# viswavi/speech-anonymization

Hardware: AMD Instinct MI355X
Metric: audio frames/sec (node), ConvAE+gender-adv train step (higher is better)
Workload: dtype bf16x3; 1 GPU; ConvAE recon0.1+sex0.9 adversarial train step (L1 recon + NLL), shape M: 32 utt/GPU x 161120 samples (T=1008 frames), Fbank x2 + norm + fwd + bwd + clip + Adam + Noam; batch_per_gpu=32, frames_per_utt=1008, parallelism=dp1

## Files before the change

### include/sa_hip.h

```cpp
#ifndef SA_HIP_H
#define SA_HIP_H
#ifdef __cplusplus
extern "C" {
#endif

#define SA_F32 0
#define SA_BF16 1
#define SA_BF16X3 2
#define SA_BF16X1F 3
#define SA_FP8 4
#define SA_F64 5
#define SA_MAX_TAPS 5
#define SA_COMM_ID_BYTES 128

typedef struct SaTaps {
  int ntaps[2];
  int off[2][SA_MAX_TAPS];
  int widx[2][SA_MAX_TAPS];
} SaTaps;

typedef struct SaConvArgs {
  const void* x;
  const void* wp;
  const float* bias;
  void* y;
  const float* s1; const float* t1;
  const float* s2; const float* t2;
  int swish;
  int relu;
  float* stats;
  int B, Lin, Lout, ntiles;
  int rowmin, nrows, wlo_off;
  SaTaps taps;
  int ep_mode, ep_xp_is_act, ep_bstride;
  const void* ep_x; const void* ep_g2;
  const float* ep_s1; const float* ep_t1; const float* ep_mean; const float* ep_rstd;
  void* a_out;
  const void* nb_x; const float* nb_c1; const float* nb_c2; const float* nb_c3;
  int nb_bstride, nb_relu_mask; float* nb_colsum;
  const float* ep_g2k1; const float* ep_g2k2; const float* ep_g2k3;
  float* pro_stats;
  const float* wscale;
  int tile_rows; int pad2_;
} SaConvArgs;

int sa_conv_gemm(int dtype, int cin, int cout, int sa, int u, const SaConvArgs* a, void* stream);
int sa_abi_sizeof(int which);
int sa_conv_gemm_ntiles(int cin, int cout, int u, int Lout);
int sa_conv_gemm_ntiles_tm(int tile_rows, int u, int Lout);
int sa_conv_gemm_set_tile_rows(int rows);
int sa_conv_gemm_set_impl(int impl);
int sa_conv_gemm_route(int dtype, int cin, int cout, int sa, int u, const SaConvArgs* a);

int sa_pack_weights(int dtype, const float* src, void* dst, int ntaps, int K, int N, int sk, int sn,
                    int st, void* stream);

typedef struct SaPackDesc {
  const float* src; void* dst;
  int dtype, ntaps, K, N, sk, sn, st, pad_;
  float* scale;
} SaPackDesc;
int sa_pack_weights_multi(const SaPackDesc* descs, int n, int blocks_per_image, void* stream);
int sa_pack_scales_multi(const SaPackDesc* descs, int n, void* stream);

typedef struct SaWgradArgs {
  const void* x;
  const void* dy;
  float* slabs;
  const float* s1; const float* t1; const float* s2; const float* t2; int swish;
  int B, Lin, Ldy, Mrows, chunk, nchunk;
  int ntaps; int off[SA_MAX_TAPS]; int ph[SA_MAX_TAPS];
  int x_pre;
  int dy_pre;
} SaWgradArgs;

int sa_wgrad(int dtype, int cin, int cout, int sa, int u, const SaWgradArgs* a, void* stream);
int sa_wgrad_kw(int cin, int cout);
int sa_wgrad_reduce(const float* slabs, float* dst, int nslab, int ntaps, int cin, int cout, int sk,
                    int sn, int st, int accumulate, void* stream);
#define SA_WRED_MAX 8
typedef struct SaWredDesc {
  const float* slabs; float* dst;
  int nslab, ntaps, cin, cout, sk, sn, st, accumulate, vec, pad_;
} SaWredDesc;
typedef struct SaWredMulti { int n, pad_; SaWredDesc d[SA_WRED_MAX]; } SaWredMulti;
int sa_wgrad_reduce_multi(const SaWredMulti* m, void* stream);

int sa_conv1toC(int dtype, const float* x, const float* w, const float* bias, void* y, int B, int L,
                int flip, float* stats, const void* ep_x, const float* ep_s1, const float* ep_t1,
                const float* ep_mean, const float* ep_rstd, void* stream);
int sa_conv1toC_ntiles(int L);
int sa_convCto1(int dtype, const void* x, const float* w, const float* bias, float* y, int B, int L,
                const float* s1, const float* t1, int swish, int flip, void* stream);
int sa_wgrad1C(int dtype, const float* u, const void* v, float* slabs, int B, int L, int chunk,
               int flip, const float* s1, const float* t1, int swish, void* stream);
int sa_wgrad1C_nchunk(int L, int chunk);
int sa_bwd1C(int dtype, const float* u, const void* v, const float* w, void* g, float* stats, float* slabs,
             int B, int L, int chunk, int flip, const float* s1, const float* t1, const float* mean,
             const float* rstd, void* stream);
int sa_sum_slabs(const float* slabs, float* dst, int nslab, int n, int accumulate, void* stream);

typedef struct SaEwArgs {
  const void* g; const void* g2; const void* x; void* out;
  const float* s1; const float* t1;
  const float* mean; const float* rstd;
  const float* c1; const float* c2; const float* c3;
  int actbwd, xp_is_act, relu_mask, bstride;
  float* stats;
  int B, L, ntiles;
} SaEwArgs;

int sa_ew_stats(int dtype, int C, const SaEwArgs* a, void* stream);
int sa_ew_apply(int dtype, int C, const SaEwArgs* a, void* stream);
int sa_ew_ntiles(int L);
int sa_sum_partials(const float* slabs, double* dst, int nbatch, int nslab, int n, void* stream);
int sa_sum_rows_d(const double* src, double* dst, int R, int n, void* stream);
int sa_fin_in_fwd(const double* sums, int B, int C, int n, const float* gamma, const float* beta,
                  float eps, float* mean, float* rstd, float* scale, float* shift, void* stream);
int sa_fin_bn_fwd(const double* sums, int R, int C, double count, const float* gamma, const float* beta,
                  float eps, float momentum, float* run_mean, float* run_var, float* mean,
                  float* rstd, float* scale, float* shift, const double* count_dev, void* stream);
int sa_fin_bn_eval(int C, const float* gamma, const float* beta, float eps, const float* run_mean,
                   const float* run_var, float* mean, float* rstd, float* scale, float* shift,
                   void* stream);
int sa_fin_norm_bwd(const double* sums, const double* lsums, int R, int groups, int C, double n,
                    const float* gamma, const float* mean, const float* rstd, float sign, float* c1,
                    float* c2, float* c3, float* dgamma, float* dbeta, const double* n_dev,
                    void* stream);
int sa_fin_bias(const double* sums, int B, int C, int ncomp, float* db, void* stream);

#define SA_FLATS_MAX 4
typedef struct SaFlat { float* p; long long n; } SaFlat;
typedef struct SaFlats { int n, pad_; SaFlat f[SA_FLATS_MAX]; } SaFlats;
int sa_clip_grads(const SaFlats* f, float max_norm, float eps, double* partials, float* total_norm, void* stream);
#define SA_BIAS_MAX 8
typedef struct SaBiasDesc {
  const float* part; double* rows; float* db;
  int nbatch, nslab, C, ncomp;
} SaBiasDesc;
typedef struct SaBiasMulti { int n, pad_; SaBiasDesc d[SA_BIAS_MAX]; } SaBiasMulti;
int sa_bias_multi(const SaBiasMulti* m, void* stream);

int sa_pool_fwd(int dtype, const void* r, const float* scale, const float* shift, float* part, int B,
                int L, int nseg, void* stream);
int sa_pool_nseg(int B);
int sa_pool_gather(const float* part, int B, int nseg, int L, double* sums, void* stream);
int sa_pool_fin(const double* sums, int B, int n, const float* noise, float eps, float* pooled,
                float* mean, float* stdraw, void* stream);
int sa_pool_bwd(int dtype, const void* r, const float* scale, const float* shift,
                const float* dpooled, const float* mean, const float* stdraw, void* g, int B, int L,
                const float* bn_mean, const float* bn_rstd, float* stats, void* stream);
int sa_dense(const float* X, int lda, const float* ps, const float* pt, const float* W, int sbk,
             int sbn, const float* bias, float* Y, int ldy, int M, int N, int K, int relu,
             void* stream);
int sa_colsums(const float* X, const float* H, const float* hmean, const float* hrstd, int M, int N,
               double* sums, float* out0, float* out1, void* stream);
int sa_bn2d_bwd(const float* G, const float* H, const double* sums, double count, const float* gamma,
                const float* mean, const float* rstd, int relu_mask, int M, int N, float* dH,
                const double* count_dev, void* stream);
int sa_dense_wgrad(const float* dY, const float* X, const float* ps, const float* pt, int M, int N,
                   int K, float* dW, void* stream);
int sa_log_softmax(const float* X, float* Y, int M, int N, void* stream);
int sa_log_softmax_bwd(const float* dY, const float* Y, float* dX, int M, int N, void* stream);
int sa_loss_workspace_bytes(void);
int sa_recon_loss(const float* a, const float* b, long long n, int kind, float* grad, float* loss,
                  void* workspace, void* stream);
int sa_cls_losses(const float* logp, const long long* label, int B, int NC, float* out, float* dnll,
                  float* dconf, void* stream);
int sa_cosine_loss(const float* x1, const float* x2, int B, int S, int D, float* rowloss,
                   float* loss, float* dx1, void* stream);

int sa_head_fwd(const float* pooled, const float* w1, const float* b1, const float* g1, const float* be1,
                float* rm1, float* rv1, const float* w2, const float* b2, const float* g2, const float* be2,
                float* rm2, float* rv2, const float* w3, const float* b3, float* h1, float* f1, float* h2,
                float* f2, float* logp, int M, float eps, float momentum, void* stream);
int sa_head_bwd(const float* dlogp, const float* logp, const float* pooled, const float* h1, const float* f1,
                const float* h2, const float* f2, const float* w1, const float* g1, const float* w2,
                const float* g2, const float* w3, float* dw1, float* db1, float* dg1, float* dbe1, float* dw2,
                float* db2, float* dg2, float* dbe2, float* dw3, float* db3, float* dpooled, int M, void* stream);
int sa_head_max_rows(void);

int sa_tdnn_fwd(const float* x, const void* wp, const float* bias, const float* bn_s, const float* bn_t,
                float* y, int B, int T, int Cin, int Cout, int Npad, int K, int dil, float slope,
                unsigned char* mask, void* stream);
int sa_time_pool(const float* x, const float* lens, const float* noise, int B, int T, int C, float eps,
                 float* out, void* stream);
int sa_leaky_affine(const float* x, const float* s, const float* t, float slope, int M, int C, float* y,
                    void* stream);
int sa_tdnn_bwd_input(const float* dy, const unsigned char* mask, const float* bn_s, const void* wp,
                      float* dxe, int B, int T, int Cy, int Cred, int Cin, int Npad, int K, int dil,
                      float slope, void* stream);
int sa_tdnn_fold(const float* dxe, float* dx, int B, int T, int C, int pad, void* stream);
int sa_time_pool_bwd(const float* x, const float* lens, const float* g, const float* pooled, int B,
                     int T, int C, float eps, float* dx, void* stream);
int sa_leaky_affine_bwd(const float* dy, const float* x, const float* s, float slope, int M, int C,
                        float* dx, void* stream);

int sa_xv_tdnn_fwd_train(const float* x, const float* s_in, const float* t_in, const void* wp, const float* bias,
                         float* z, float* part, int B, int T, int Cin, int Cout, int Npad, int K, int dil,
                         float slope, void* stream);
int sa_xv_tdnn_ntiles(int T);
int sa_xv_colsums(const float* G, const float* H, const float* hmean, const float* hrstd, const float* c1,
                  const float* c2, const float* c3, float slope, float* out, int M, int N, int rows_per,
                  double* part, void* stream);
int sa_xv_tdnn_wgrad(const float* dpre, const float* x, const float* s_in, const float* t_in, float* part, int B,
                     int T, int Cin, int Cout, int K, int dil, int nsplit, int rows_per, void* stream);
int sa_xv_wgrad_reduce(const float* part, int nsplit, int K, int Cout, int Cin, float* dW, void* stream);
int sa_xv_tdnn_dgrad(const float* dpre, const void* wp, float* dxe, int B, int T, int Cy, int Cred, int Cin,
                     int Npad, int K, int dil, void* stream);
int sa_xv_pool_affine(const float* pz, const float* s, const float* t, const float* noise, int B, int C,
                      float eps, float* pooled, void* stream);
int sa_xv_pool_affine_bwd(const float* g, const float* s, int B, int C, float* gz, void* stream);

int sa_fc_tiles(int T);
int sa_fc_groups(int B, int T);
int sa_fc_nparam(void);
int sa_fc_nhead(void);
int sa_fc_max_rows(void);
int sa_fc_enc_fwd(const float* feats, const void* const* wb, float* h1, float* h2, float* z, double* bnpart,
                  int B, int T, void* stream);
int sa_fc_bn_fin(const double* bnpart, int npart, const float* gamma, const float* beta, float* run_mean,
                 float* run_var, float* bnf, int B, int T, int train, float eps, float momentum, void* stream);
int sa_fc_mid_fwd(const float* z, const float* bnf, const void* const* wb, float* a1, float* u, float* d1,
                  float* d2, float* recon, double* poolpart, int B, int T, void* stream);
int sa_fc_recon_fwd(const float* feats, const void* const* wb, float* recon, int B, int T, void* stream);
int sa_fc_head_fwd(const double* poolpart, const float* noise, const void* const* hw, float* pooled, float* pst,
                   float* h1, float* f1, float* h2, float* h3, float* f2, float* logp, int B, int T, int train,
                   float eps, float momentum, void* stream);
int sa_fc_head_bwd(const float* dlogp, const float* logp, const float* pooled, const float* h1,
                   const float* h2, const float* h3, const void* const* hw, float* dhead,
                   float* dpooled, int B, int train, float eps, void* stream);
int sa_fc_mid_bwd(const float* d_recon, const float* dpooled, const float* pst, const float* z, const float* bnf,
                  const float* a1, const float* u, const float* d1, const float* d2, const void* const* wb,
                  float* dzn, float* dzdec, float* wpart, double* bnbpart, int B, int T, void* stream);
int sa_fc_bn_bwd_fin(const double* bnbpart, int npart, const float* gamma, const float* bnf, float* coef,
                     float* dgamma, float* dbeta, int B, int T, int train, void* stream);
int sa_fc_enc_bwd(const float* feats, const float* h1, const float* h2, const float* z, const float* dzn,
                  const float* dzdec, const float* coef, const void* const* wb, float* wpart, int B, int T,
                  void* stream);
int sa_fc_wreduce(const float* wpart, int G, float* grads, void* stream);

int sa_cluster_mi(const float* X, const long long* y, const long long* idx, int iters, int n, int D,
                  int ncls, int k, float* mi, void* stream);

int sa_fbank(const float* wav, int B, int N, const float* window, const void* dft,
             const void* mel, float* feats, float* tilemax, void* stream);
int sa_fbank_table_elems(int which);
int sa_fbank_ntiles(int T);
int sa_fbank_scratch_bytes(int B);
int sa_fbank_normalize(const float* feats, const float* tilemax, int B, int T, int Tp,
                       const float* lens, float top_db, int batch_max, int update, int epoch,
                       int update_until_epoch, float* state, float* scratch, float* out,
                       void* stream);
int sa_fbank_normalize_pair(const float* feats, const float* tilemax, int B, int T, int Tp,
                            const float* lens, float top_db, int batch_max, int update, int epoch,
                            int update_until_epoch, float* state, float* scratch, float* snap,
                            float* out1, float* out2, void* stream);

int sa_wav_augment_tile(void);
int sa_wav_augment_max_chunks(void);
int sa_wav_abs_sums(const float* wav, const float* noise, int B, int L, double* sums, void* stream);
int sa_noise_scales(const double* sums, const float* lens, const float* snr, int B, int L, float* scales,
                    void* stream);
int sa_wav_augment(const float* wav, const float* noise, const float* scales, const void* plan, int B, int L, int R,
                   int Lp, int S_in, int S_out, int W, int first_min, int first_max, float* out, void* stream);

int sa_specaug_warp_sums(const float* x, const void* plan, int B, int T, int F, float* out, double* part,
                         void* stream);
int sa_specaug_finalize(const double* part, const void* plan, int B, int T, int F, float* vals, void* stream);
int sa_specaug_fill(const void* plan, const float* vals, int B, int T, int F, float* out, void* stream);

int sa_gl_tile(void);
int sa_mel_to_mag(const float* x, const float* mean, const float* stdv, const float* M, int B, int T, int Tf,
                  float* S, void* stream);
int sa_gl_istft(const void* C, const float* window, const float* twiddle, int B, int T, float* y, void* stream);
int sa_gl_project(const float* y, const float* S, const void* Tprev, float momentum_ratio, const float* window,
                  const float* twiddle, int B, int T, void* C_new, void* R, void* stream);

int sa_yin_dim(int which);
int sa_yin_f0(const float* wav, int B, int N, float threshold, float* f0, float* dprime, void* stream);
int sa_pitch_ratio(const float* f0, const float* lens, int B, int T, int N, float target, float r_min, float r_max,
                   int min_voiced, float* ratio, float* mean, int* voiced, void* stream);
int sa_pitch_stretch_mag(const void* R, const float* ratio, int B, int T, int Tout, float* S, void* stream);
int sa_pitch_resample(const float* y, const float* ratio, const int* n_valid, int B, int Nin, int Nout, float* out,
                      void* stream);

int sa_env_dim(int which);
int sa_env_warp(const float* S, const float* q, int B, int T, int n_c, float floor_rel, float max_gain_ln,
                float* out, float* env, void* stream);

int sa_mcadams_dim(int which);
int sa_mcadams(const float* wav, const float* alpha, const int* n_valid, int B, int N, int level, float* out,
               void* ws, int* status, float* gain, void* stream);

int sa_stoi_dim(int which);
int sa_stoi(const float* ref, const float* deg, const int* n_valid, int B, int N, const double* taps,
            float* stoi, float* estoi, int* frames, int* segments, void* ws, void* stream);

int sa_pv_dim(int which);
long long sa_pv_workspace_bytes(int B, int Tout);
int sa_pv_synth(const void* R, const float* S, const float* ratio, int B, int T, int Tout, void* C, double* phase,
                void* ws, void* stream);

int sa_contour_dim(int which);
int sa_pitch_contour(const float* f0, const float* lens, int B, int T, int N, float target, float gamma, int smooth,
                     float r_min, float r_max, int min_voiced, int* rho_q, long long* Q, int* Tq, float* mean,
                     int* voiced, void* stream);
int sa_pv_synth_map(const void* R, const float* M, const int* rho_q, const long long* Q, int B, int T, int Tout,
                    void* C, double* phase, void* ws, void* stream);
int sa_env_warp_frames(const float* S, const float* q, int B, int T, int n_c, float floor_rel, float max_gain_ln,
                       float* out, float* env, void* stream);
int sa_pitch_resample_map(const float* y, const int* rho_q, const long long* Q, const int* n_valid, int B, int Nin,
                          int Nout, int T, float* out, void* stream);

int sa_f0v_dim(int which);
int sa_f0_candidates(const float* dprime, int B, int T, int* cand_tau, int* cand_q, void* stream);
int sa_f0_viterbi(const float* dprime, const int* cand_tau, const int* cand_q, const float* lens, const int* log_q,
                  int B, int T, int N, float voicing_cost, float switch_cost, float jump_cost, float lag_bias,
                  unsigned char* psi, int* path, float* f0, void* stream);

int sa_f0cmp_dim(int which);
int sa_f0_compare(const float* f0_ref, const float* f0_deg, const int* frames, int B, int T, int max_lag,
                  int min_common, float* rho, int* lag, int* common, float* shift_st, float* dev_st, float* voicing,
                  void* stream);

int sa_mcd_dim(int which);
int sa_mcd(const float* mel_ref, const float* mel_deg, const int* n_ref, const int* n_deg, int B, int T_ref, int T_deg,
           int n_mels, int order, int band, void* ws, float* mcd, float* mcd_sync, int* frames, void* stream);

int sa_psola_dim(int which);
long long sa_psola_workspace_bytes(int B, int N);
int sa_psola_marks(const float* wav, const float* f0, const int* n_valid, int B, int N, int T, int* marks, int* count,
                   void* stream);
int sa_psola_plan(const int* marks, const int* count, const float* f0, const int* rho_q, const int* n_valid, int B,
                  int N, int T, void* ws, int* syn_pos, int* syn_src, int* syn_count, void* stream);
int sa_psola_ola(const float* wav, const int* marks, const int* count, const int* syn_pos, const int* syn_src,
                 const int* syn_count, const int* n_valid, int B, int N, float* out, void* stream);

int sa_formant_dim(int which);
int sa_formant_tracks(const float* wav, const int* n_valid, int B, int N, float* freq, float* bw, int* status,
                      void* stream);
int sa_formant_compare(const float* F_ref, const float* F_deg, const int* st_ref, const int* st_deg,
                       const float* f0_ref, const float* f0_deg, const int* frames, int B, int T, int min_common,
                       float* med, float* ratio, float* shift, int* common, void* stream);

int sa_add_layernorm_fwd(const void* x, const void* r, const void* gamma, const void* beta, void* y, void* s_out,
                         float* stat, int rows, int d, float eps, void* stream);
int sa_layernorm_bwd(const void* dy, const void* s, const float* stat, const void* gamma, void* ds, int rows,
                     int d, void* stream);
int sa_ln_leaky_fwd(const void* x, const void* gamma, const void* beta, void* y, float* stat, int rows, int d,
                    float eps, float slope, void* stream);
int sa_ln_leaky_bwd(const void* dy, const void* x, const float* stat, const void* gamma, const void* beta, void* dx,
                    int rows, int d, float slope, void* stream);
int sa_asr_block0_fwd(const void* x, const void* w, const void* bias, const void* gamma, const void* beta, void* y,
                      float* stat, int B, int T, int F, int C, float eps, float slope, void* stream);
int sa_asr_block0_bwd(const void* dy, const void* x, const void* w, const void* bias, const void* gamma,
                      const void* beta, const float* stat, float* part, void* dx, int B, int T, int F, int C,
                      float slope, void* stream);
int sa_reflect_pad_fwd(const void* x, void* y, int B, int T, int F, int C, void* stream);
int sa_reflect_pad_bwd(const void* dy, void* dx, int B, int T, int F, int C, void* stream);

int sa_comm_unique_id(void* id128);
int sa_comm_init(int rank, int world, const void* id128, int device);
int sa_comm_world(void);
int sa_comm_allreduce(void* buf, long long n, int dtype, int avg, void* producer_stream);
int sa_comm_allreduce_inline(void* buf, long long n, int dtype, int avg, void* stream);
int sa_comm_join(void* consumer_stream);
int sa_comm_ncalls(void);
int sa_comm_destroy(void);

#ifdef __cplusplus
}
#endif
#endif
```

### speech-anonymization_amd/_lib.py

```python
import ctypes as C
import os

import torch

_HERE = os.path.dirname(os.path.abspath(__file__))
LIB_PATH = os.environ.get("SA_HIP_LIB") or os.path.join(_HERE, "libsa_hip.so")

F32, BF16, BF16X3, BF16X1F, FP8, F64 = 0, 1, 2, 3, 4, 5
MAX_TAPS = 5

c_fp = C.POINTER(C.c_float)
vp = C.c_void_p


class SaTaps(C.Structure):
    _fields_ = [("ntaps", C.c_int * 2), ("off", (C.c_int * MAX_TAPS) * 2),
                ("widx", (C.c_int * MAX_TAPS) * 2)]


class SaConvArgs(C.Structure):
    _fields_ = [("x", vp), ("wp", vp), ("bias", vp), ("y", vp),
                ("s1", vp), ("t1", vp), ("s2", vp), ("t2", vp),
                ("swish", C.c_int), ("relu", C.c_int), ("stats", vp),
                ("B", C.c_int), ("Lin", C.c_int), ("Lout", C.c_int), ("ntiles", C.c_int),
                ("rowmin", C.c_int), ("nrows", C.c_int), ("wlo_off", C.c_int), ("taps", SaTaps),
                ("ep_mode", C.c_int), ("ep_xp_is_act", C.c_int), ("ep_bstride", C.c_int),
                ("ep_x", vp), ("ep_g2", vp), ("ep_s1", vp), ("ep_t1", vp), ("ep_mean", vp), ("ep_rstd", vp),
                ("a_out", vp),
                ("nb_x", vp), ("nb_c1", vp), ("nb_c2", vp), ("nb_c3", vp),
                ("nb_bstride", C.c_int), ("nb_relu_mask", C.c_int), ("nb_colsum", vp),
                ("ep_g2k1", vp), ("ep_g2k2", vp), ("ep_g2k3", vp), ("pro_stats", vp), ("wscale", vp),
                ("tile_rows", C.c_int), ("pad2_", C.c_int)]


class SaPackDesc(C.Structure):
    _fields_ = [("src", vp), ("dst", vp), ("dtype", C.c_int), ("ntaps", C.c_int), ("K", C.c_int),
                ("N", C.c_int), ("sk", C.c_int), ("sn", C.c_int), ("st", C.c_int), ("pad_", C.c_int),
                ("scale", vp)]


class SaWgradArgs(C.Structure):
    _fields_ = [("x", vp), ("dy", vp), ("slabs", vp),
                ("s1", vp), ("t1", vp), ("s2", vp), ("t2", vp), ("swish", C.c_int),
                ("B", C.c_int), ("Lin", C.c_int), ("Ldy", C.c_int), ("Mrows", C.c_int),
                ("chunk", C.c_int), ("nchunk", C.c_int),
                ("ntaps", C.c_int), ("off", C.c_int * MAX_TAPS), ("ph", C.c_int * MAX_TAPS),
                ("x_pre", C.c_int), ("dy_pre", C.c_int)]


class SaEwArgs(C.Structure):
    _fields_ = [("g", vp), ("g2", vp), ("x", vp), ("out", vp),
                ("s1", vp), ("t1", vp), ("mean", vp), ("rstd", vp),
                ("c1", vp), ("c2", vp), ("c3", vp),
                ("actbwd", C.c_int), ("xp_is_act", C.c_int), ("relu_mask", C.c_int),
                ("bstride", C.c_int), ("stats", vp),
                ("B", C.c_int), ("L", C.c_int), ("ntiles", C.c_int)]


BIAS_MAX = 8


class SaBiasDesc(C.Structure):
    _fields_ = [("part", vp), ("rows", vp), ("db", vp),
                ("nbatch", C.c_int), ("nslab", C.c_int), ("C", C.c_int), ("ncomp", C.c_int)]


class SaBiasMulti(C.Structure):
    _fields_ = [("n", C.c_int), ("pad_", C.c_int), ("d", SaBiasDesc * BIAS_MAX)]


WRED_MAX = 8
FLATS_MAX = 4


class SaFlat(C.Structure):
    _fields_ = [("p", vp), ("n", C.c_longlong)]


class SaFlats(C.Structure):
    _fields_ = [("n", C.c_int), ("pad_", C.c_int), ("f", SaFlat * FLATS_MAX)]



class SaWredDesc(C.Structure):
    _fields_ = [("slabs", vp), ("dst", vp)] + [(k, C.c_int) for k in ("nslab", "ntaps", "cin", "cout", "sk", "sn", "st",
                                                                      "accumulate", "vec", "pad_")]


class SaWredMulti(C.Structure):
    _fields_ = [("n", C.c_int), ("pad_", C.c_int), ("d", SaWredDesc * WRED_MAX)]


SYMBOLS = [
    "sa_conv_gemm", "sa_abi_sizeof", "sa_conv_gemm_ntiles", "sa_conv_gemm_ntiles_tm", "sa_conv_gemm_set_tile_rows",
    "sa_conv_gemm_set_impl", "sa_conv_gemm_route", "sa_pack_weights", "sa_pack_weights_multi", "sa_pack_scales_multi", "sa_wgrad", "sa_wgrad_kw", "sa_wgrad_reduce",
    "sa_conv1toC", "sa_conv1toC_ntiles", "sa_convCto1", "sa_wgrad1C", "sa_wgrad1C_nchunk", "sa_bwd1C",
    "sa_sum_slabs", "sa_ew_stats", "sa_ew_apply", "sa_ew_ntiles",
    "sa_sum_partials", "sa_sum_rows_d", "sa_fin_in_fwd", "sa_fin_bn_fwd", "sa_fin_bn_eval", "sa_fin_norm_bwd", "sa_fin_bias",
    "sa_pool_fwd", "sa_pool_nseg", "sa_pool_gather", "sa_pool_fin", "sa_pool_bwd", "sa_dense", "sa_colsums",
    "sa_bn2d_bwd", "sa_dense_wgrad", "sa_log_softmax", "sa_log_softmax_bwd",
    "sa_loss_workspace_bytes", "sa_recon_loss", "sa_cls_losses", "sa_cosine_loss",
    "sa_tdnn_fwd", "sa_time_pool", "sa_leaky_affine", "sa_tdnn_bwd_input", "sa_tdnn_fold", "sa_time_pool_bwd",
    "sa_leaky_affine_bwd", "sa_cluster_mi", "sa_fbank", "sa_fbank_table_elems", "sa_fbank_ntiles", "sa_fbank_scratch_bytes", "sa_fbank_normalize", "sa_fbank_normalize_pair",
    "sa_comm_unique_id", "sa_comm_init", "sa_comm_world", "sa_comm_allreduce", "sa_comm_allreduce_inline", "sa_comm_join", "sa_comm_ncalls",
    "sa_comm_destroy", "sa_head_fwd", "sa_head_bwd", "sa_head_max_rows",
    "sa_add_layernorm_fwd", "sa_layernorm_bwd", "sa_reflect_pad_fwd", "sa_reflect_pad_bwd", "sa_ln_leaky_fwd", "sa_ln_leaky_bwd", "sa_bias_multi", "sa_asr_block0_fwd", "sa_asr_block0_bwd", "sa_wgrad_reduce_multi", "sa_clip_grads",
    "sa_xv_tdnn_fwd_train", "sa_xv_tdnn_ntiles", "sa_xv_colsums", "sa_xv_tdnn_wgrad", "sa_xv_wgrad_reduce",
    "sa_xv_tdnn_dgrad", "sa_xv_pool_affine", "sa_xv_pool_affine_bwd",
    "sa_fc_tiles", "sa_fc_groups", "sa_fc_nparam", "sa_fc_nhead", "sa_fc_max_rows", "sa_fc_enc_fwd", "sa_fc_bn_fin",
    "sa_fc_mid_fwd", "sa_fc_head_fwd", "sa_fc_head_bwd", "sa_fc_mid_bwd", "sa_fc_bn_bwd_fin", "sa_fc_enc_bwd",
    "sa_fc_wreduce", "sa_fc_recon_fwd",
    "sa_wav_augment_tile", "sa_wav_augment_max_chunks", "sa_wav_abs_sums", "sa_noise_scales", "sa_wav_augment",
    "sa_specaug_warp_sums", "sa_specaug_finalize", "sa_specaug_fill",
    "sa_gl_tile", "sa_mel_to_mag", "sa_gl_istft", "sa_gl_project",
    "sa_yin_dim", "sa_yin_f0", "sa_pitch_ratio", "sa_pitch_stretch_mag", "sa_pitch_resample",
    "sa_env_dim", "sa_env_warp",
    "sa_mcadams_dim", "sa_mcadams",
    "sa_stoi_dim", "sa_stoi",
    "sa_pv_dim", "sa_pv_synth",
    "sa_contour_dim", "sa_pitch_contour", "sa_pv_synth_map", "sa_env_warp_frames", "sa_pitch_resample_map",
    "sa_f0v_dim", "sa_f0_candidates", "sa_f0_viterbi",
    "sa_f0cmp_dim", "sa_f0_compare",
    "sa_mcd_dim", "sa_mcd",
    "sa_psola_dim", "sa_psola_marks", "sa_psola_plan", "sa_psola_ola",
    "sa_formant_dim", "sa_formant_tracks", "sa_formant_compare",
]

_lib = None


class SaHipError(RuntimeError):
    pass


def load():
    global _lib
    if _lib is None:
        if not os.path.exists(LIB_PATH):
            raise SaHipError(
                f"{LIB_PATH} not found: build it with `python -c 'import __graft_entry__ as g; "
                "g.build()'` (hipcc --offload-arch=gfx950). There is no CPU fallback.")
        _lib = C.CDLL(LIB_PATH)
        for s in SYMBOLS:
            getattr(_lib, s).restype = C.c_int
        _lib.sa_pv_workspace_bytes.restype = C.c_longlong
        _lib.sa_psola_workspace_bytes.restype = C.c_longlong
        for i, rec in enumerate((SaConvArgs, SaWgradArgs, SaEwArgs, SaPackDesc, SaTaps, SaBiasMulti, SaWredMulti, SaFlats)):
            if _lib.sa_abi_sizeof(i) != C.sizeof(rec):
                raise SaHipError(f"{rec.__name__}: binding has {C.sizeof(rec)} bytes, {LIB_PATH} "
                                 f"{_lib.sa_abi_sizeof(i)} -- rebuild the library (stale build?)")
    return _lib


def stream():
    return C.c_void_p(torch._C._cuda_getCurrentRawStream(torch._C._cuda_getDevice()))


def ptr(t):
    if t is None:
        return None
    assert t.is_cuda and t.is_contiguous(), "HIP kernels take contiguous device tensors"
    return C.c_void_p(t.data_ptr())


def check(rc, what):
    if rc != 0:
        raise SaHipError(f"{what} failed with code {rc}")


def dt_code(dtype):
    if dtype == torch.float32:
        return F32
    if dtype == torch.bfloat16:
        return BF16
    raise SaHipError(f"unsupported activation dtype {dtype}")


_taps_cache = {}


def make_taps(phases):
    key = tuple(tuple(p) for p in phases)
    t = _taps_cache.get(key)
    if t is not None:
        return t
    t = _taps_cache[key] = SaTaps()
    for ph, lst in enumerate(phases):
        t.ntaps[ph] = len(lst)
        for i, (off, wi) in enumerate(lst):
            t.off[ph][i] = off
            t.widx[ph][i] = wi
    return t
```

### speech-anonymization_amd/brain.py

```python
import enum
import os
import types

import torch

from . import distributed as sdist


class Stage(enum.Enum):
    TRAIN = 1
    VALID = 2
    TEST = 3


class EpochCounter:

    def __init__(self, limit):
        self.current, self.limit = 0, int(limit)

    def __iter__(self):
        return self

    def __next__(self):
        if self.current < self.limit:
            self.current += 1
            return self.current
        raise StopIteration


class NoamScheduler:

    def __init__(self, lr_initial, n_warmup_steps, model_size=None):
        self.lr_initial, self.n_warmup_steps = lr_initial, n_warmup_steps
        self.current_lr, self.n_steps = lr_initial, 0
        self.normalize = n_warmup_steps ** 0.5 if model_size is None else model_size ** (-0.5)

    def __call__(self, opt):
        self.n_steps += 1
        current_lr = getattr(opt, "_sa_host_lr", None)
        if current_lr is None:
            current_lr = opt.param_groups[0]["lr"]
        lr = self.lr_initial * self.normalize * min(self.n_steps ** (-0.5),
                                                    self.n_steps * self.n_warmup_steps ** (-1.5))
        for g in opt.param_groups:
            if torch.is_tensor(g["lr"]):
                g["lr"].fill_(lr)
            else:
                g["lr"] = lr
        opt._sa_host_lr = lr
        self.current_lr = current_lr
        return current_lr, lr

    def state_dict(self):
        return {"losses": [], "n_steps": self.n_steps}

    def load_state_dict(self, sd):
        self.n_steps = sd["n_steps"]


class Batch:

    def __init__(self, wavs, lens, gender, tokens_bos=None, ids=None):
        self.sig = (wavs, lens)
        self.gender = gender
        self.tokens_bos = (tokens_bos if tokens_bos is not None
                           else torch.ones(wavs.shape[0], 1, dtype=torch.long), lens)
        self.id = ids

    def to(self, device):
        w, l = self.sig
        tb, tl = self.tokens_bos
        out = Batch.__new__(Batch)
        out.sig = (w.to(device, non_blocking=True), l.to(device, non_blocking=True))
        out.gender = self.gender.to(device, non_blocking=True)
        out.tokens_bos = (tb.to(device, non_blocking=True), tl.to(device, non_blocking=True))
        out.id = self.id
        return out


def settle_python_heap():
    import gc
    gc.collect()
    gc.freeze()


class Brain:
    GC_FREEZE_STEP = 8

    def __init__(self, modules=None, opt_class=None, hparams=None, run_opts=None, checkpointer=None):
        run_opts = dict(run_opts or {})
        self.device = torch.device(run_opts.get("device", "cuda:0" if torch.cuda.is_available() else "cpu"))
        if self.device.type == "cuda":
            torch.cuda.set_device(self.device)
        self.max_grad_norm = float(run_opts.get("max_grad_norm", 5.0))
        self.nonfinite_patience = int(run_opts.get("nonfinite_patience", 3))
        self.lazy_finite_check = bool(run_opts.get("lazy_finite_check", True))
        self.hip_graph = bool(run_opts.get("hip_graph", False)) and self.device.type == "cuda"
        self.gc_freeze = bool(run_opts.get("gc_freeze", True))
        self.fused_clip = bool(run_opts.get("fused_clip", os.environ.get("SA_FUSED_CLIP", "1") == "1"))
        self.front_end_once = bool(run_opts.get("front_end_once", os.environ.get("SA_FRONT_END_ONCE", "1") == "1"))
        self.distributed_launch = bool(run_opts.get("distributed_launch", sdist.is_distributed()))
        self.modules = torch.nn.ModuleDict(modules or {})
        self.dp_batch_sizes = run_opts.get("dp_batch_sizes", "equal")
        self.opt_class = opt_class
        self.hparams = types.SimpleNamespace(**(hparams or {}))
        self.checkpointer = checkpointer
        self.step, self.nonfinite_count, self.optimizer = 0, 0, None
        self.avg_train_loss = 0.0

    def compute_forward(self, batch, stage):
        raise NotImplementedError

    def compute_objectives(self, predictions, batch, stage):
        raise NotImplementedError

    def on_stage_start(self, stage, epoch=None):
        pass

    def on_stage_end(self, stage, stage_loss, epoch=None):
        pass

    def on_fit_start(self):
        self.modules.to(self.device)
        for m in self.modules.values():
            if hasattr(m, "dp_batch_sizes"):
                m.dp_batch_sizes = self.dp_batch_sizes
        self.init_optimizers()
        if self.checkpointer is not None:
            if self.optimizer is not None:
                self.checkpointer.add_recoverable("optimizer", self.optimizer)
            self.resumed_from = self.checkpointer.recover_if_possible(device=self.device, brain=self)

    def init_optimizers(self):
        if self.opt_class is not None and self.optimizer is None:
            params = list(self.modules.parameters())
            base = getattr(self.opt_class, "func", self.opt_class)
            given = getattr(self.opt_class, "keywords", None) or {}
            if base is torch.optim.Adam and "fused" not in given and params and all(p.is_cuda for p in params):
                try:
                    if self.hip_graph:
                        self.optimizer = self.opt_class(params, fused=True, capturable=True)
                        for g in self.optimizer.param_groups:
                            self.optimizer._sa_host_lr = float(g["lr"])
                            g["lr"] = torch.tensor(float(g["lr"]), dtype=torch.float32, device=self.device)
                    else:
                        self.optimizer = self.opt_class(params, fused=True)
                    return
                except (TypeError, RuntimeError):
                    self.hip_graph = False
            self.optimizer = self.opt_class(params)

    def check_gradients(self, loss):
        bad = self._count_nonfinite(loss)
        if bad:
            self.nonfinite_count += bad
            if self.nonfinite_count > self.nonfinite_patience:
                raise ValueError("Loss is not finite and patience is exhausted.")
            if not (self.lazy_finite_check and loss.is_cuda):
                return False
        params = getattr(self, "_clip_params", None)
        if params is None:
            params = self._clip_params = list(self.modules.parameters())
        flats = self._grad_flats(params) if self.fused_clip else None
        if flats:
            from . import ops
            ops.clip_flats(flats, self.max_grad_norm)
        else:
            torch.nn.utils.clip_grad_norm_(params, self.max_grad_norm)
        return True

    def _grad_flats(self, params):
        model = self.modules["ConvAE"] if "ConvAE" in self.modules else None
        flats = getattr(model, "_last_flats", None) if model is not None else None
        if not flats:
            return None
        spans = [(f.data_ptr(), f.data_ptr() + 4 * f.numel(), f.numel()) for f in flats]
        seen = [0] * len(flats)
        for p in params:
            g = p.grad
            if g is None:
                continue
            if g.dtype != torch.float32 or not g.is_contiguous():
                return None
            a = g.data_ptr()
            for i, (lo, hi, _) in enumerate(spans):
                if lo <= a < hi:
                    seen[i] += g.numel()
                    break
            else:
                return None
        if any(n != span[2] for n, span in zip(seen, spans)):
            return None
        return flats

    def _count_nonfinite(self, loss):
        if not (self.lazy_finite_check and loss.is_cuda):
            return 0 if bool(torch.isfinite(loss)) else 1
        st = getattr(self, "_finite_state", None)
        if st is None:
            st = self._finite_state = dict(dev=torch.zeros((), dtype=torch.int32, device=loss.device),
                                           host=torch.zeros((), dtype=torch.int32).pin_memory(),
                                           event=torch.cuda.Event(), seen=0, pending=False)
        new = self._poll_nonfinite()
        st["dev"].add_((~torch.isfinite(loss.detach())).to(torch.int32))
        st["host"].copy_(st["dev"], non_blocking=True)
        if not torch.cuda.is_current_stream_capturing():
            st["event"].record()
            st["pending"] = True
        return new

    def _poll_nonfinite(self, wait=False):
        st = getattr(self, "_finite_state", None)
        if st is None or not st["pending"]:
            return 0
        if wait:
            st["event"].synchronize()
        elif not st["event"].query():
            return 0
        st["pending"] = False
        total = int(st["host"])
        new, st["seen"] = total - st["seen"], total
        return max(new, 0)

    def fit_batch(self, batch):
        outputs = self.compute_forward(batch, Stage.TRAIN)
        loss = self.compute_objectives(outputs, batch, Stage.TRAIN)
        loss.backward()
        if self.check_gradients(loss):
            self.optimizer.step()
        self.optimizer.zero_grad()
        return loss.detach()

    def evaluate_batch(self, batch, stage):
        out = self.compute_forward(batch, stage=stage)
        return self.compute_objectives(out, batch, stage=stage).detach()

    def update_average(self, loss, avg_loss):
        if not loss.is_cuda:
            if torch.isfinite(loss):
                avg_loss -= avg_loss / self.step
                avg_loss += float(loss) / self.step
            return avg_loss
        if not torch.is_tensor(avg_loss):
            avg_loss = torch.full((), float(avg_loss), device=loss.device, dtype=torch.float32)
        new = avg_loss + (loss.detach().float() - avg_loss) / self.step
        return torch.where(torch.isfinite(loss), new, avg_loss)

    def fit(self, epoch_counter, train_set, valid_set=None, progressbar=False, **_):
        self.on_fit_start()
        for epoch in epoch_counter:
            self.on_stage_start(Stage.TRAIN, epoch)
            self.modules.train()
            self.nonfinite_count = 0
            self.avg_train_loss = 0.0
            self.step = 0
            for batch in train_set:
                self.step += 1
                loss = self.fit_batch(batch)
                self.avg_train_loss = self.update_average(loss, self.avg_train_loss)
                if self.gc_freeze and self.step == self.GC_FREEZE_STEP and not self.__dict__.get("_gc_frozen"):
                    settle_python_heap()
                    self._gc_frozen = True
            self.nonfinite_count += self._poll_nonfinite(wait=True)
            if self.nonfinite_count > self.nonfinite_patience:
                raise ValueError("Loss is not finite and patience is exhausted.")
            self.avg_train_loss = float(self.avg_train_loss)
            self.on_stage_end(Stage.TRAIN, self.avg_train_loss, epoch)
            if valid_set is not None:
                self.on_stage_start(Stage.VALID, epoch)
                self.modules.eval()
                avg, n = 0.0, 0
                with torch.no_grad():
                    for batch in valid_set:
                        n += 1
                        avg += (float(self.evaluate_batch(batch, Stage.VALID)) - avg) / n
                self.on_stage_end(Stage.VALID, avg, epoch)

    def on_evaluate_start(self, max_key=None, min_key=None):
        pass

    def evaluate(self, test_set, max_key=None, min_key=None, **_):
        self.on_evaluate_start(max_key=max_key, min_key=min_key)
        self.on_stage_start(Stage.TEST, None)
        self.modules.eval()
        avg, n = 0.0, 0
        with torch.no_grad():
            for batch in test_set:
                n += 1
                avg += (float(self.evaluate_batch(batch, Stage.TEST)) - avg) / n
        self.on_stage_end(Stage.TEST, avg, None)
        return avg


class SexAnonymizationTraining(Brain):

    @staticmethod
    def _sig_key(wavs, wav_lens):
        return tuple((t.data_ptr(), tuple(t.shape), t.dtype, t._version) for t in (wavs, wav_lens))

    def features(self, wavs, wav_lens):
        stash, self._target_stash = self.__dict__.get("_target_stash"), None
        if stash is not None and stash[0] == self._sig_key(wavs, wav_lens):
            return stash[1]
        feats = self.hparams.compute_features(wavs)
        current_epoch = self.hparams.epoch_counter.current
        pad = 36 if self.hparams.model_type != "fcae" else None
        return self.modules.normalize(feats, wav_lens, epoch=current_epoch, pad_multiple=pad)

    def _features_pair(self, wavs, wav_lens):
        feats = self.hparams.compute_features(wavs)
        pad = 36 if self.hparams.model_type != "fcae" else None
        inp, target = self.modules.normalize.forward_pair(feats, wav_lens, epoch=self.hparams.epoch_counter.current,
                                                          pad_multiple=pad)
        self._target_stash = (self._sig_key(wavs, wav_lens), target)
        return inp

    def compute_forward(self, batch, stage):
        batch = batch.to(self.device)
        wavs, wav_lens = batch.sig
        if (stage == Stage.TRAIN and self.__dict__.get("_in_fit_batch") and self.front_end_once
                and hasattr(self.modules.normalize, "forward_pair")):
            feats = self._features_pair(wavs, wav_lens)
        else:
            feats = self.features(wavs, wav_lens)
        aug = self.__dict__.get("_specaug")
        if aug is not None and stage == Stage.TRAIN:
            self._specaug_shapes[tuple(wavs.shape)] = tuple(feats.shape)
            feats = aug.apply(feats) if self.__dict__.get("_specaug_drawn") else aug(feats)
        return self.modules.ConvAE(feats)

    def spec_augment(self):
        if not getattr(self.hparams, "spec_augment", False):
            return None
        from . import specaug
        aug = getattr(self.hparams, "augmentation", None)
        return aug if isinstance(aug, specaug.SpecAugment) else None

    def compute_objectives(self, predictions, batch, stage):
        reconstructed_speech, sex_logits = predictions
        batch = batch.to(self.device)
        sex_label = batch.gender
        wavs, wav_lens = batch.sig
        feats = self.features(wavs, wav_lens)
        hp = self.hparams
        utility_loss = 0.0
        asr_brain = getattr(self, "asr_brain", None)
        if stage == Stage.TRAIN and hp.utility_loss_weight > 0 and asr_brain is not None:
            from . import asr
            tokens_bos, _ = batch.tokens_bos
            utility_loss = asr.utility_loss(asr_brain, hp.loss_utility, feats, reconstructed_speech,
                                            wav_lens, tokens_bos, batch)
        B = reconstructed_speech.shape[0]
        recon_loss = hp.loss_reconstruction(reconstructed_speech.view(B, -1), feats.view(B, -1))
        sex_loss = hp.loss_sex_classification(sex_logits, sex_label)
        if hp.model_type == "endtoend":
            if hp.recon_loss_weight == 0.0 and hp.utility_loss_weight == 0.0:
                loss = hp.sex_loss_weight * sex_loss
            else:
                confusion_loss = hp.loss_confusion(sex_logits, None)
                loss = (hp.recon_loss_weight * recon_loss - hp.sex_loss_weight * sex_loss
                        + hp.utility_loss_weight * utility_loss
                        - hp.confusion_loss_weight * confusion_loss)
        else:
            loss = (hp.recon_loss_weight * recon_loss + hp.sex_loss_weight * sex_loss
                    + hp.utility_loss_weight * utility_loss)
        self.last_losses = dict(recon=recon_loss.detach(), sex=sex_loss.detach())
        if stage != Stage.TRAIN:
            n = torch.tensor(sex_label.shape[0], device=sex_logits.device).unsqueeze(0)
            self.sex_classification_acc.append(sex_logits.unsqueeze(0), sex_label.unsqueeze(0), n)
            ext = getattr(self, "external_classifier", None)
            if ext is not None:
                with torch.no_grad():
                    lo, _, _ = ext.classify_batch_feats(feats)
                    lr, _, _ = ext.classify_batch_feats(reconstructed_speech.detach())
                self.sex_classification_acc_extern_orig.append(lo.unsqueeze(0), sex_label.unsqueeze(0), n)
                self.sex_classification_acc_extern.append(lr.unsqueeze(0), sex_label.unsqueeze(0), n)
            if asr_brain is not None:
                from . import ops
                tokens_bos, _ = batch.tokens_bos
                with torch.no_grad():
                    recon_enc, _ = asr_brain.get_predictions(reconstructed_speech.detach(), wav_lens, tokens_bos,
                                                             batch, eval=True, do_ctc=False)
                    orig_enc, _ = asr_brain.get_predictions(feats, wav_lens, tokens_bos, batch, eval=True,
                                                            do_ctc=False)
                    nb = recon_enc.shape[0]
                    self.utility_similarity_aggregator.append(
                        ops.cosine_rows(recon_enc.reshape(nb, -1), orig_enc.reshape(nb, -1)))
        return loss

    def apply_epoch_schedule(self):
        hp = self.hparams
        if not getattr(hp, "epoch_parity_schedule", False):
            return
        joint = hp.epoch_counter.current % 2 == 0
        if joint:
            hp.recon_loss_weight, hp.sex_loss_weight = 0.0, 0.8
            hp.utility_loss_weight, hp.confusion_loss_weight = 0.2, 0.0
        else:
            hp.recon_loss_weight, hp.sex_loss_weight, hp.utility_loss_weight = 0.0, 0.5, 0.0
        for name, param in self.modules.ConvAE.named_parameters():
            param.requires_grad = ("sex_classifier" not in name) if joint else ("sex_classifier" in name)

    def _zero_grads_of_frozen(self):
        st = self.optimizer.state
        for group in self.optimizer.param_groups:
            for p in group["params"]:
                if p.grad is None and not p.requires_grad and p in st and len(st[p]):
                    z = getattr(self, "_zero_grad_cache", None)
                    if z is None:
                        z = self._zero_grad_cache = {}
                    g = z.get(p)
                    if g is None:
                        g = z[p] = torch.zeros_like(p)
                    p.grad = g

    GRAPH_WARMUP = 3

    def _graph_key(self, batch):
        hp = self.hparams
        wavs, lens = batch.sig
        nrm = self.modules["normalize"] if "normalize" in self.modules else None
        upd = nrm is not None and hp.epoch_counter.current < getattr(nrm, "update_until_epoch", 0)
        st = self.optimizer.state if self.optimizer is not None else {}
        params = list(self.modules.ConvAE.parameters())
        tok = batch.tokens_bos[0]
        return (tuple(wavs.shape), str(wavs.dtype), hp.model_type, float(hp.recon_loss_weight),
                float(hp.sex_loss_weight), float(hp.utility_loss_weight),
                float(getattr(hp, "confusion_loss_weight", 0.0)), bool(upd),
                tuple(p.requires_grad for p in params),
                tuple(bool(st.get(p)) for p in params if not p.requires_grad),
                tuple(tok.shape), getattr(self, "asr_brain", None) is not None,
                self.front_end_once, bool(not upd and getattr(nrm, "_count_positive", False)),
                self.__dict__.get("_specaug") is not None)

    def _step_core(self, batch):
        predictions = self.compute_forward(batch, Stage.TRAIN)
        loss = self.compute_objectives(predictions, batch, Stage.TRAIN)
        loss.backward()
        if getattr(self.hparams, "epoch_parity_schedule", False):
            self._zero_grads_of_frozen()
        self.check_gradients(loss)
        self.optimizer.step()
        return loss.detach()

    def _fit_batch_graph(self, batch):
        batch = batch.to(self.device)
        key = self._graph_key(batch)
        graphs = self.__dict__.setdefault("_graphs", {})
        ent = graphs.get(key)
        if ent is None:
            ent = graphs[key] = {"seen": 0}
        if "graph" not in ent:
            ent["seen"] += 1
            if ent["seen"] <= self.GRAPH_WARMUP:
                self.optimizer.zero_grad(set_to_none=True)
                loss = self._step_core(batch)
                self.optimizer.zero_grad()
                self.hparams.noam_annealing(self.optimizer)
                return loss
            wavs, lens = batch.sig
            ent["wav"], ent["lens"] = wavs.clone(), lens.clone()
            ent["gender"] = batch.gender.clone()
            tok, tok_lens = batch.tokens_bos
            ent["tok"], ent["tok_lens"] = tok.clone(), tok_lens.clone()
            ent["batch"] = Batch(ent["wav"], ent["lens"], ent["gender"], tokens_bos=ent["tok"], ids=batch.id)
            ent["batch"].tokens_bos = (ent["tok"], ent["tok_lens"])
            torch.cuda.synchronize()
            self.nonfinite_count += self._poll_nonfinite(wait=True)
            g = torch.cuda.CUDAGraph()
            self.optimizer.zero_grad(set_to_none=True)
            aug = self.__dict__.get("_specaug")
            if aug is not None:
                ent["specaug"] = self._specaug_shapes[tuple(wavs.shape)]
                aug.draw(*ent["specaug"], device=self.device)
                self._specaug_drawn = True
            try:
                with torch.cuda.graph(g):
                    ent["loss"] = self._step_core(ent["batch"])
            finally:
                self._specaug_drawn = False
            ent["graph"] = g
        elif "specaug" in ent:
            self._specaug.draw(*ent["specaug"], device=self.device)
        wavs, lens = batch.sig
        ent["wav"].copy_(wavs, non_blocking=True)
        ent["lens"].copy_(lens, non_blocking=True)
        ent["gender"].copy_(batch.gender, non_blocking=True)
        ent["tok"].copy_(batch.tokens_bos[0], non_blocking=True)
        ent["tok_lens"].copy_(batch.tokens_bos[1], non_blocking=True)
        ent["batch"].id = batch.id
        bad = self._poll_nonfinite()
        if bad:
            self.nonfinite_count += bad
            if self.nonfinite_count > self.nonfinite_patience:
                raise ValueError("Loss is not finite and patience is exhausted.")
        ent["graph"].replay()
        st = getattr(self, "_finite_state", None)
        if st is not None:
            st["event"].record()
            st["pending"] = True
        self.hparams.noam_annealing(self.optimizer)
        return ent["loss"]

    def fit_batch(self, batch):
        self._target_stash, self._in_fit_batch = None, True
        try:
            return self._fit_batch(batch)
        finally:
            self._target_stash, self._in_fit_batch = None, False

    def _fit_batch(self, batch):
        self.apply_epoch_schedule()
        if (self.hip_graph and self.hparams.gradient_accumulation == 1 and sdist.capturable()
                and self.optimizer is not None):
            return self._fit_batch_graph(batch)
        if self.front_end_once:
            batch = batch.to(self.device)
        predictions = self.compute_forward(batch, Stage.TRAIN)
        loss = self.compute_objectives(predictions, batch, Stage.TRAIN)
        (loss / self.hparams.gradient_accumulation).backward()
        if self.step % self.hparams.gradient_accumulation == 0:
            if getattr(self.hparams, "epoch_parity_schedule", False):
                self._zero_grads_of_frozen()
            self.check_gradients(loss)
            self.optimizer.step()
            self.optimizer.zero_grad()
            self.hparams.noam_annealing(self.optimizer)
        return loss.detach()

    def evaluate_batch(self, batch, stage):
        with torch.no_grad():
            predictions = self.compute_forward(batch, stage=stage)
            loss = self.compute_objectives(predictions, batch, stage=stage)
        return loss.detach()

    def load_external_classifier(self):
        ext = getattr(self.hparams, "external_classifier", None)
        if ext is not None:
            ext.eval()
            ext.to(self.device)
        return ext

    def on_stage_start(self, stage, epoch=None):
        from .metrics import AccuracyStats, SimilarityMetricsStats
        self.external_classifier = self.load_external_classifier()
        if stage == Stage.TRAIN:
            self._specaug = self.spec_augment()
            if self._specaug is not None:
                self.__dict__.setdefault("_specaug_shapes", {})
                self._specaug.reseed(epoch, sdist.rank())
        if stage != Stage.TRAIN:
            self.sex_classification_acc = AccuracyStats()
            self.sex_classification_acc_extern = AccuracyStats()
            self.sex_classification_acc_extern_orig = AccuracyStats()
            self.utility_similarity_aggregator = SimilarityMetricsStats()

    def on_evaluate_start(self, max_key=None, min_key=None):
        if self.checkpointer is None:
            return
        ckpts = self.checkpointer.find_checkpoints(max_key=max_key, min_key=min_key)
        if not ckpts:
            return
        sd = self.checkpointer.average_checkpoints(ckpts, recoverable_name="model", device=self.device)
        model = getattr(self.hparams, "model", None)
        if model is not None:
            model.load_state_dict(sd, strict=False)
            model.eval()

    def on_stage_end(self, stage, stage_loss, epoch=None):
        stats = {"loss": stage_loss}
        if stage == Stage.TRAIN:
            self.train_stats = stats
            return
        stats["ACC"] = self.sex_classification_acc.summarize()
        if self.external_classifier is not None:
            stats["ACC_external"] = self.sex_classification_acc_extern.summarize()
            stats["ACC_external_orig"] = self.sex_classification_acc_extern_orig.summarize()
        if self.utility_similarity_aggregator.denom:
            stats["Utility_Retention"] = float(self.utility_similarity_aggregator.summarize())
        self.valid_stats = stats
        logger = getattr(self.hparams, "train_logger", None)
        if stage == Stage.VALID and sdist.if_main_process() and logger is not None:
            na = self.hparams.noam_annealing
            logger.log_stats(stats_meta={"epoch": epoch, "lr": na.current_lr, "steps": na.n_steps,
                                         "optimizer": self.optimizer.__class__.__name__},
                             train_stats=self.train_stats, valid_stats=stats)
        if stage == Stage.VALID and sdist.if_main_process() and self.checkpointer is not None:
            keys = {k: stats[k] for k in ("ACC_external", "Utility_Retention") if k in stats}
            self.checkpointer.save_and_keep_only(self, epoch, dict(stats, **keys),
                                                 max_keys=[k for k in ("Utility_Retention",) if k in stats],
                                                 min_keys=[k for k in ("ACC_external",) if k in stats],
                                                 num_to_keep=5)


class FileTrainLogger:

    def __init__(self, save_file):
        self.save_file = save_file

    @staticmethod
    def _fmt(d):
        out = []
        for k, v in d.items():
            if isinstance(v, float) and 1.0 < v < 100.0:
                v = f"{v:.2f}"
            elif isinstance(v, float):
                v = f"{v:.2e}"
            out.append(f"{k}: {v}")
        return ", ".join(out)

    def log_stats(self, stats_meta, train_stats=None, valid_stats=None, test_stats=None):
        s = self._fmt(stats_meta)
        for name, st in (("train", train_stats), ("valid", valid_stats), ("test", test_stats)):
            if st is not None:
                s += " - " + self._fmt({f"{name} {k}": v for k, v in st.items()})
        os.makedirs(os.path.dirname(os.path.abspath(self.save_file)), exist_ok=True)
        with open(self.save_file, "a") as f:
            f.write(s + "\n")
```

### speech-anonymization_amd/convae.py

```python
import functools
import os

import torch
import torch.nn as nn

from . import distributed as sdist
from . import ops
from . import _lib as L
from ._lib import SaHipError


class _ParamOnly(nn.Module):

    def forward(self, x):
        raise SaHipError("parameter container only; use ConvAutoencoder.forward")


class GLU(_ParamOnly):
    pass


class StatisticsPooling(_ParamOnly):
    pass


class TDNNSexClassifier(nn.Module):
    def __init__(self, num_classes=2):
        super().__init__()
        self.tdnn = nn.Sequential(
            nn.Conv1d(128, 128, kernel_size=5, dilation=1), nn.ReLU(), nn.BatchNorm1d(128),
            nn.Conv1d(128, 128, kernel_size=3, dilation=2), nn.ReLU(), nn.BatchNorm1d(128),
            nn.Conv1d(128, 128, kernel_size=3, dilation=3), nn.ReLU(), nn.BatchNorm1d(128),
        )
        self.norm = nn.BatchNorm1d(128)
        self.stats_pooling = StatisticsPooling()
        self.classify = nn.Sequential(
            nn.Linear(256, 128), nn.ReLU(), nn.BatchNorm1d(128),
            nn.Linear(128, 64), nn.ReLU(), nn.BatchNorm1d(64),
            nn.Linear(64, num_classes),
        )

    def forward(self, x):
        raise SaHipError("parameter container only; use ConvAutoencoder.forward")


class ConvAutoencoder(nn.Module):
    def __init__(self, precision="bf16x3", pooling_noise=True, sync_bn=True, dtype=None,
                 cache_wgrad_operand=True):
        super().__init__()
        if dtype is not None:
            precision = {torch.float32: "f32", torch.bfloat16: "bf16"}[dtype]
        if precision not in ops.PRECISIONS:
            raise SaHipError(f"unknown precision {precision!r}")
        self.precision = precision
        self.encoder = nn.Sequential(
            nn.Conv1d(1, 32, 15, 1, 7), GLU(),
            nn.Conv1d(32, 64, 5, 2, 2), nn.InstanceNorm1d(64, affine=True), GLU(),
            nn.Conv1d(64, 64, 5, 1, 2), nn.InstanceNorm1d(64, affine=True), GLU(),
            nn.Conv1d(64, 128, 5, 2, 2), nn.InstanceNorm1d(128, affine=True), GLU(),
            nn.Conv1d(128, 128, 5, 1, 2), nn.InstanceNorm1d(128, affine=True), GLU(),
        )
        self.decoder = nn.Sequential(
            nn.Conv1d(128, 128, 5, 1, 2),
            nn.ConvTranspose1d(128, 64, 5, 2, 2, output_padding=1),
            nn.InstanceNorm1d(64, affine=True), GLU(),
            nn.Conv1d(64, 64, 5, 1, 2),
            nn.ConvTranspose1d(64, 32, 5, 2, 2, output_padding=1),
            nn.InstanceNorm1d(32, affine=True), GLU(),
            nn.Conv1d(32, 1, 15, 1, 7),
        )
        self.sex_classifier = TDNNSexClassifier(2)
        self.lay = ops.conv_layers(self, ("encoder", "sex_classifier.tdnn", "decoder"))
        self.pack_plan = [(ly.key, ly.kinds[i]) for i in (0, 1)
                          for ly in sorted(self.lay.values(), key=lambda ly: ly.transposed)]
        self.act_dtype, self.kcode = ops.PRECISIONS[precision]
        self.dgrad_kcode = ops.DGRAD_CODE[precision]
        self.cache_wgrad_operand = cache_wgrad_operand
        self.pooling_noise = pooling_noise
        self.sync_bn = sync_bn
        self.fused_head = os.environ.get("SA_FUSED_HEAD", "1") == "1"
        self.fused_bwd1c = os.environ.get("SA_FUSED_BWD1C", "1") == "1"
        self.dp_batch_sizes = None

    def forward(self, feats):
        names, params = self._named_params()
        return _ConvAEFn.apply(self, names, feats, *params)

    def _named_params(self):
        c = self.__dict__.get("_np_cache")
        if c is None or any(o[n] is not p for o, n, p in c[2]):
            names, params, owners = [], [], []
            for mname, mod in self.named_modules():
                for pname, p in mod._parameters.items():
                    if p is not None:
                        names.append(f"{mname}.{pname}" if mname else pname)
                        params.append(p)
                        owners.append((mod._parameters, pname, p))
            c = self.__dict__["_np_cache"] = (tuple(names), tuple(params), owners)
        return c[0], c[1]

    @torch.no_grad()
    def reconstruct(self, feats):
        if not torch.is_tensor(feats) or feats.dim() != 3:
            raise SaHipError("ConvAutoencoder expects feats [B, T, 80]")
        x0, B, T, Ltot = _input_rows(feats)
        P = dict(zip(*self._named_params()))
        cg, inorm = _launchers(self, P, _packed(self, P), B)
        y, _, _ = _encoder_launches(self, P, cg, inorm, x0, Ltot, False)
        return _decoder_launches(self, P, cg, inorm, y[5], Ltot)[-1].view(B, T, 80)

    def _side_stream(self, device):
        if getattr(self, "_side", None) is None and device.type == "cuda":
            self._side = torch.cuda.Stream(device=device)
        return getattr(self, "_side", None)

    def _bn_syncs(self):
        return self.sync_bn and sdist.dp_active()

    def _bn_allreduce(self, sums):
        if self._bn_syncs():
            sdist.all_reduce_now(sums)
            return sdist.world_size()
        return 1

    def _bn_global_counts(self, counts, device):
        if not self._bn_syncs():
            return None
        key = (tuple(counts), str(device))
        cache = self.__dict__.setdefault("_count_cache", {})
        local = cache.get(key)
        if local is None:
            if len(cache) > 64:
                cache.clear()
            local = cache[key] = torch.tensor(counts, dtype=torch.float64).to(device)
        g = local.clone()
        sdist.all_reduce_now(g)
        return g

    def _bn_rows(self):
        return not self._bn_syncs()

    def _bn_global(self, local_sums):
        if not self._bn_syncs():
            return local_sums, 1
        g = local_sums.clone()
        return g, self._bn_allreduce(g)

    def _head_plan(self, B):
        if not self._bn_syncs() or self.dp_batch_sizes is None:
            return None
        W, r = sdist.world_size(), sdist.rank()
        sizes = [B] * W if isinstance(self.dp_batch_sizes, str) else [int(b) for b in self.dp_batch_sizes]
        if self.dp_batch_sizes != "equal" and isinstance(self.dp_batch_sizes, str):
            raise SaHipError(f"dp_batch_sizes: 'equal', a list of per-rank batch sizes or None, not {self.dp_batch_sizes!r}")
        if len(sizes) != W or sizes[r] != B:
            raise SaHipError(f"dp_batch_sizes {sizes} does not describe rank {r} of {W} holding {B} utterances")
        return sum(sizes[:r]), sum(sizes), W

    @staticmethod
    def _gather_rows(x, plan):
        off, Bg, _ = plan
        g = torch.zeros(Bg, x.shape[1], device=x.device, dtype=x.dtype)
        g[off:off + x.shape[0]].copy_(x)
        sdist.all_reduce_now(g)
        return g


class _W:
    __slots__ = ("img", "code")

    def __init__(self, img, code):
        self.img, self.code = img, code


def _kcode(model, kind):
    return model.dgrad_kcode if kind.endswith("dgrad") else model.kcode


def _packed(model, P):
    items = [((k, kind), P[k], kind, _kcode(model, kind)) for k, kind in model.pack_plan]
    key = tuple(w.data_ptr() for _, w, _, _ in items) + tuple(c for _, _, _, c in items)
    pk = getattr(model, "_pack_cache", None)
    if pk is None or pk[0] != key:
        pk = (key, ops.PackedWeights(items, model.act_dtype))
        model._pack_cache = pk
    pk[1].refresh()
    return {tag: _W(img, code) for tag, (img, code) in pk[1].images.items()}


def _conv(x, w, *args, **kw):
    return ops.conv_gemm(x, w.img, *args, code=w.code, **kw)


class _PendingApply:
    __slots__ = ("g", "y", "c", "per_c", "relu", "bias_key", "wgrads")

    def __init__(self, g, y, c, per_c, relu, bias_key):
        self.g, self.y, self.c, self.per_c, self.relu, self.bias_key = g, y, c, per_c, relu, bias_key
        self.wgrads = []


def _noise(model, B, device):
    return ops.pooling_noise(model.pooling_noise, B, 128, device)


def _input_rows(feats):
    B, T, Fd = feats.shape
    Ltot = T * Fd
    if Fd != 80 or Ltot % 4:
        raise SaHipError("ConvAutoencoder expects feats [B, T, 80] with T*80 divisible by 4")
    if not feats.is_cuda:
        raise SaHipError("ConvAutoencoder runs on the GPU only (no CPU fallback)")
    return feats.detach().reshape(B, Ltot).contiguous().float(), B, T, Ltot


def _in_ep(y, nrm, g2=None):
    mean, rstd, scale, shift = nrm
    d = dict(mode=1, x=y, g2=g2, s1=scale, t1=shift, mean=mean, rstd=rstd)
    if isinstance(g2, _PendingApply):
        d.update(g2=g2.g, g2k=g2.c)
    return d


def _launchers(model, P, W, B, A=None):
    def cg(ly, x, **kw):
        if A is not None and P[ly.key].requires_grad:
            A[ly.key] = kw["a_out"] = torch.empty(x.shape, dtype=torch.bfloat16, device=x.device)
        return _conv(x, W[ly.key, ly.kinds[0]], P[ly.bias], *ly.fwd(x.shape[1]), **kw)

    def inorm(stats, n, prefix, C):
        sums = ops.sum_partials(stats, B)
        return ops.fin_in_fwd(sums, B, C, n, P[prefix + ".weight"], P[prefix + ".bias"])
    return cg, inorm


def _encoder_launches(model, P, cg, inorm, x0, Ltot, want_pro_stats):
    L2, L4, lay = Ltot // 2, Ltot // 4, model.lay
    y0 = ops.conv1toC(x0, P["encoder.0.weight"], P["encoder.0.bias"], model.act_dtype)
    y1, st = cg(lay["encoder.2"], y0, swish=True, want_stats=True)
    n1 = inorm(st, L2, "encoder.3", 64)
    y2, st = cg(lay["encoder.5"], y1, s1=n1[2], t1=n1[3], swish=True, want_stats=True)
    n2 = inorm(st, L2, "encoder.6", 64)
    y3, st = cg(lay["encoder.8"], y2, s1=n2[2], t1=n2[3], swish=True, want_stats=True)
    n3 = inorm(st, L4, "encoder.9", 128)
    y4, st = cg(lay["encoder.11"], y3, s1=n3[2], t1=n3[3], swish=True, want_stats=True)
    n4 = inorm(st, L4, "encoder.12", 128)
    y5 = cg(lay["decoder.0"], y4, s1=n4[2], t1=n4[3], swish=True, want_pro_stats=want_pro_stats)
    a4_stats = None
    if want_pro_stats:
        y5, a4_stats = y5
    return [y0, y1, y2, y3, y4, y5], [n1, n2, n3, n4], a4_stats


def _decoder_launches(model, P, cg, inorm, y5, Ltot):
    L2, lay = Ltot // 2, model.lay
    y6, st = cg(lay["decoder.1"], y5, want_stats=True)
    n6 = inorm(st, L2, "decoder.2", 64)
    y7 = cg(lay["decoder.4"], y6, s1=n6[2], t1=n6[3], swish=True)
    y8, st = cg(lay["decoder.5"], y7, want_stats=True)
    n8 = inorm(st, Ltot, "decoder.6", 32)
    recon = ops.convCto1(y8, P["decoder.8.weight"], P["decoder.8.bias"], n8[2], n8[3], True)
    return y6, n6, y7, y8, n8, recon


class _ConvAEFn(torch.autograd.Function):
    @staticmethod
    def forward(ctx, model, names, feats, *params):
        ctx.set_materialize_grads(False)
        P = dict(zip(names, params))
        train = model.training
        x0, B, T, Ltot = _input_rows(feats)
        L2, L4 = Ltot // 2, Ltot // 4
        S = {}
        W, lay = _packed(model, P), model.lay
        A = {}
        cache_a = (train and model.cache_wgrad_operand and any(ctx.needs_input_grad)
                   and ops.WGRAD_CODE[model.precision] in (L.BF16X1F, L.BF16) and model.kcode != L.FP8)

        cg, inorm = _launchers(model, P, W, B, A if cache_a else None)

        def bn_stats(stats, count, mod, prefix, C, ci):
            sums = ops.sum_partials(stats, 1, rows=model._bn_rows()) if train else None
            return bnorm(sums, count, mod, prefix, C, ci)

        def bnorm(sums, count, mod, prefix, C, ci, local=False):
            if not train:
                return ops.fin_bn_eval(C, P[prefix + ".weight"], P[prefix + ".bias"],
                                       mod.running_mean, mod.running_var)
            if not local:
                model._bn_allreduce(sums)
            out = ops.fin_bn_fwd(sums, C, count, P[prefix + ".weight"], P[prefix + ".bias"],
                                 mod.running_mean, mod.running_var, count_dev=None if local else cdev(ci))
            tracked.append(mod.num_batches_tracked)
            return out

        tracked = []
        enc, dec, cls = model.encoder, model.decoder, model.sex_classifier
        La, Lb, Lc = L4 - 4, L4 - 8, L4 - 14
        gc = model._bn_global_counts([B * L4, B * La, B * Lb, B * Lc, B, B], feats.device) if train else None
        cdev = lambda i: None if gc is None else gc[i:i + 1]
        (y0, y1, y2, y3, y4, y5), (n1, n2, n3, n4), a4_stats = _encoder_launches(model, P, cg, inorm, x0, Ltot, train)
        bn_n = bn_stats(a4_stats if train else None, B * L4, cls.norm, "sex_classifier.norm", 128, 0)
        r0, st = cg(lay["sex_classifier.tdnn.0"], y4, s1=n4[2], t1=n4[3], swish=True, s2=bn_n[2], t2=bn_n[3],
                    relu=True, want_stats=True)
        bn0 = bn_stats(st, B * La, cls.tdnn[2], "sex_classifier.tdnn.2", 128, 1)
        r1, st = cg(lay["sex_classifier.tdnn.3"], r0, s2=bn0[2], t2=bn0[3], relu=True, want_stats=True)
        bn1 = bn_stats(st, B * Lb, cls.tdnn[5], "sex_classifier.tdnn.5", 128, 2)
        r2, st = cg(lay["sex_classifier.tdnn.6"], r1, s2=bn1[2], t2=bn1[3], relu=True, want_stats=True)
        bn2 = bn_stats(st, B * Lc, cls.tdnn[8], "sex_classifier.tdnn.8", 128, 3)
        pooled, pmean, psd = ops.pool_fwd(r2, bn2[2], bn2[3], noise=_noise(model, B, feats.device))
        def head_fwd(X, n, local=False):
            H1 = ops.dense(X, P["sex_classifier.classify.0.weight"], P["sex_classifier.classify.0.bias"],
                           128, 256, relu=True)
            f1 = bnorm(ops.colsums(H1) if train else None, n, cls.classify[2], "sex_classifier.classify.2", 128, 4, local)
            H2 = ops.dense(H1, P["sex_classifier.classify.3.weight"], P["sex_classifier.classify.3.bias"],
                           64, 128, ps=f1[2], pt=f1[3], relu=True)
            f2 = bnorm(ops.colsums(H2) if train else None, n, cls.classify[5], "sex_classifier.classify.5", 64, 5, local)
            logits = ops.dense(H2, P["sex_classifier.classify.6.weight"], P["sex_classifier.classify.6.bias"],
                               2, 64, ps=f2[2], pt=f2[3])
            return H1, f1, H2, f2, ops.log_softmax(logits)

        plan = model._head_plan(B) if train else None
        head_in, Bh = (model._gather_rows(pooled, plan), plan[1]) if plan else (pooled, B)
        fused_head = (train and model.fused_head and (plan is not None or not model._bn_syncs())
                      and Bh <= ops.head_max_rows())
        clsP = {k[len("sex_classifier.classify."):]: v for k, v in P.items() if k.startswith("sex_classifier.classify.")}
        if fused_head:
            H1, f1, H2, f2, logp = ops.head_fwd(head_in, clsP, cls.classify[2], cls.classify[5])
            tracked += [cls.classify[2].num_batches_tracked, cls.classify[5].num_batches_tracked]
        else:
            H1, f1, H2, f2, logp = head_fwd(head_in, Bh, plan is not None)
        logp_all = logp
        if plan:
            logp = logp_all[plan[0]:plan[0] + B]
        y6, n6, y7, y8, n8, recon = _decoder_launches(model, P, cg, inorm, y5, Ltot)

        if tracked:
            torch._foreach_add_(tracked, 1)
        S.update(x0=x0, y=[y0, y1, y2, y3, y4, y5, y6, y7, y8], r=[r0, r1, r2],
                 n=[None, n1, n2, n3, n4, None, n6, None, n8], bn=[bn_n, bn0, bn1, bn2], f=[f1, f2],
                 pooled=head_in, pmean=pmean, psd=psd, H1=H1, H2=H2, logp=logp_all, head_plan=plan,
                 dims=(B, T, Ltot, L2, L4, La, Lb, Lc), train=train, W=W, A=A, gc=gc, fused_head=fused_head)
        ctx.S, ctx.model, ctx.names, ctx.params = S, model, names, params
        ctx.need_input_grad = feats.requires_grad
        return recon.view(B, T, 80), logp

    @staticmethod
    def backward(ctx, d_recon, d_logp):
        S, model, names = ctx.S, ctx.model, ctx.names
        if S is None:
            raise SaHipError("ConvAutoencoder backward called twice (saved tensors were released)")
        P = dict(zip(names, ctx.params))
        dt = model.act_dtype
        B, T, Ltot, L2, L4, La, Lb, Lc = S["dims"]
        if not S["train"]:
            raise SaHipError("backward through eval-mode BatchNorm is not implemented")
        y0, y1, y2, y3, y4, y5, y6, y7, y8 = S["y"]
        r0, r1, r2 = S["r"]
        n1, n2, n3, n4, n6, n8 = S["n"][1], S["n"][2], S["n"][3], S["n"][4], S["n"][6], S["n"][8]
        bn_n, bn0, bn1, bn2 = S["bn"]
        f1, f2 = S["f"]
        dev = y0.device
        G = {k: None for k in names}
        need = {k: p.requires_grad for k, p in P.items()}
        need_stage = {st: any(v for k, v in need.items() if k.startswith(st))
                      for st in sdist.StageBuckets.STAGES}
        run_encoder = need_stage["encoder"] or ctx.need_input_grad
        run_decoder = need_stage["decoder"] or run_encoder
        model._last_flats = None
        buckets = sdist.StageBuckets(list(P.items()), dev, model._side_stream(dev))
        newg = buckets.view

        def setg(key, val):
            G[key] = newg(key).copy_(val.reshape(P[key].shape))
        W, A, lay = S["W"], S["A"], model.lay
        gc = S["gc"]
        cdev = lambda i: None if gc is None else gc[i:i + 1]
        pending_wred = []
        wg = functools.partial(ops.wgrad, code=ops.WGRAD_CODE[model.precision], defer=pending_wred)
        fuse = bool(A) and model.dgrad_kcode in (L.BF16X3, L.BF16)

        def cg(ly, gin, **kw):
            p, dy = gin, gin.g if isinstance(gin, _PendingApply) else gin
            w, args = W[ly.key, ly.kinds[1]], (None,) + ly.dgrad(ly.lin(dy.shape[1]))
            if dy is gin:
                return _conv(dy, w, *args, **kw)
            dyc = torch.empty(p.g.shape, dtype=torch.bfloat16, device=p.g.device) if p.wgrads else None
            want_cs = p.bias_key is not None and need[p.bias_key]
            out = _conv(p.g, w, *args, a_out=dyc, nb=dict(x=p.y, c1=p.c[0], c2=p.c[1], c3=p.c[2],
                                                           per_c=p.per_c, relu_mask=p.relu,
                                                           want_colsum=want_cs), **kw)
            if want_cs:
                cs = out[-1]
                out = out[:-1] if len(out) > 2 else out[0]
                nb_, _, cc_ = cs.shape
                G[p.bias_key] = newg(p.bias_key)
                pending_bias.append((cs, nb_, cc_, 1, G[p.bias_key]))
            for f in p.wgrads:
                f(dyc)
            p.wgrads = []
            return out

        def bias_from(stats, key, C):
            if need[key]:
                G[key] = newg(key)
                pending_bias.append((stats, B, C, 2, G[key]))

        pending_bias = []

        def flush_pending():
            if pending_bias:
                ops.bias_multi(pending_bias)
                pending_bias.clear()
            if pending_wred:
                ops.wgrad_reduce_multi(pending_wred)
                pending_wred.clear()

        def in_finish(g, st, y, nrm, C, Ln, prefix, bias_key):
            mean, rstd = nrm[0], nrm[1]
            dg, db = newg(prefix + ".weight"), newg(prefix + ".bias")
            sums = ops.sum_partials(st, B)
            c1, c2, c3 = ops.fin_norm_bwd(sums, sums, B * C, C, Ln, P[prefix + ".weight"], mean, rstd,
                                          dgamma=dg, dbeta=db)
            G[prefix + ".weight"], G[prefix + ".bias"] = dg, db
            if fuse:
                return _PendingApply(g, y, (c1, c2, c3), False, False, bias_key)
            st2 = ops.ew("apply", g, y, C, out=g, c1=c1, c2=c2, c3=c3)
            bias_from(st2, bias_key, C)
            return g

        def bn_ep(r, bn, xp=None):
            d = dict(mode=2, x=r, mean=bn[0], rstd=bn[1], per_c=True)
            if xp:
                d.update(s1=xp[0], t1=xp[1], xp_is_act=True)
            return d

        def bn_finish(g, st, r, bn, Ln, prefix, bias_key, ci, xp=None):
            mean, rstd = bn[0], bn[1]
            kw = dict(s1=xp[0], t1=xp[1], xp_is_act=True) if xp else {}
            dg, db = newg(prefix + ".weight"), newg(prefix + ".bias")
            lsums = ops.sum_partials(st, 1, rows=model._bn_rows())
            gsums, _ = model._bn_global(lsums)
            c1, c2, c3 = ops.fin_norm_bwd(gsums, lsums, 128, 128, float(B * Ln), P[prefix + ".weight"],
                                          mean, rstd, sign=-1.0 if xp else 1.0, dgamma=dg, dbeta=db,
                                          n_dev=cdev(ci))
            G[prefix + ".weight"], G[prefix + ".bias"] = dg, db
            if fuse:
                return _PendingApply(g, r, (c1, c2, c3), True, not xp, bias_key)
            st2 = ops.ew("apply", g, r, 128, out=g, c1=c1, c2=c2, c3=c3, relu_mask=not xp, per_c=True,
                         want_stats=bias_key is not None, **kw)
            if bias_key:
                bias_from(st2, bias_key, 128)
            return g

        def conv_wgrad(ly, x, dy, **pro):
            key = ly.key
            if not need[key]:
                return
            if isinstance(dy, _PendingApply):
                dy.wgrads.append(lambda dyc: conv_wgrad(ly, x, dyc, dy_pre=True))
                return
            if key in A:
                x, pro = A[key], dict(x_pre=True, dy_pre=bool(pro.get("dy_pre")))
            *geo, strides = ly.wgrad(x.shape[1])
            G[key] = wg(x, dy, *geo, newg(key), strides, **pro)

        recon_unused = d_recon is None
        if recon_unused:
            for k in need:
                if k.startswith("decoder"):
                    need[k] = False
            need_stage["decoder"] = False
        if d_logp is None:
            d_logp = torch.zeros(B, 2, device=dev)

        def finish(d_feats=None):
            flush_pending()
            buckets.join()
            ctx.S = None
            model._last_flats = [buckets.flat[st] for st in sdist.StageBuckets.STAGES if need_stage[st]]
            grads = tuple(G[k] if need[k] else None for k in names)
            G.clear()
            buckets.views.clear()
            return (None, None, d_feats) + grads

        def head_bwd():
            c = "sex_classifier.classify."
            plan = S.get("head_plan")
            dlp, Bh = d_logp.contiguous().float(), B
            if plan:
                dlp, Bh = model._gather_rows(dlp, plan), plan[1]
            dP = head_bwd_rows(c, dlp, Bh, plan is not None)
            if plan:
                hg = [G[k] for k in names if k.startswith(c) and k in G]
                if plan[2] > 1 and hg:
                    torch._foreach_mul_(hg, 1.0 / plan[2])
                dP = dP[plan[0]:plan[0] + B]
            return dP

        def head_bwd_rows(c, dlp, n, local):
            if S.get("fused_head"):
                short = ("0.weight", "0.bias", "2.weight", "2.bias", "3.weight", "3.bias", "5.weight", "5.bias",
                         "6.weight", "6.bias")
                views = {}
                for k in short:
                    if need[c + k]:
                        views[k] = G[c + k] = newg(c + k)
                clsP = {k: P[c + k] for k in short}
                return ops.head_bwd(dlp, S["logp"], S["pooled"], S["H1"], f1, S["H2"], f2, clsP, views)
            glob = (lambda l: l) if local else (lambda l: model._bn_global(l)[0])
            cd = (lambda i: None) if local else cdev
            dLG = ops.log_softmax_bwd(dlp, S["logp"])
            H1, H2 = S["H1"], S["H2"]
            G[c + "6.weight"] = ops.dense_wgrad(dLG, H2, newg(c + "6.weight"), ps=f2[2], pt=f2[3])
            G[c + "6.bias"] = newg(c + "6.bias"); ops.colsums(dLG, out0=G[c + "6.bias"])
            dN2 = ops.dense(dLG, P[c + "6.weight"], None, 64, 2, transpose_w=True)
            G[c + "5.weight"], G[c + "5.bias"] = newg(c + "5.weight"), newg(c + "5.bias")
            l2 = ops.colsums(dN2, H2, f2[0], f2[1], out0=G[c + "5.bias"], out1=G[c + "5.weight"])
            dH2 = ops.bn2d_bwd(dN2, H2, glob(l2), n, P[c + "5.weight"], f2[0], f2[1], True, count_dev=cd(5))
            G[c + "3.weight"] = ops.dense_wgrad(dH2, H1, newg(c + "3.weight"), ps=f1[2], pt=f1[3])
            G[c + "3.bias"] = newg(c + "3.bias"); ops.colsums(dH2, out0=G[c + "3.bias"])
            dN1 = ops.dense(dH2, P[c + "3.weight"], None, 128, 64, transpose_w=True)
            G[c + "2.weight"], G[c + "2.bias"] = newg(c + "2.weight"), newg(c + "2.bias")
            l1 = ops.colsums(dN1, H1, f1[0], f1[1], out0=G[c + "2.bias"], out1=G[c + "2.weight"])
            dH1 = ops.bn2d_bwd(dN1, H1, glob(l1), n, P[c + "2.weight"], f1[0], f1[1], True, count_dev=cd(4))
            G[c + "0.weight"] = ops.dense_wgrad(dH1, S["pooled"], newg(c + "0.weight"))
            G[c + "0.bias"] = newg(c + "0.bias"); ops.colsums(dH1, out0=G[c + "0.bias"])
            return ops.dense(dH1, P[c + "0.weight"], None, 256, 128, transpose_w=True)

        def tdnn_bwd(dP):
            t = "sex_classifier.tdnn."
            g, st = ops.pool_bwd(r2, bn2[2], bn2[3], dP, S["pmean"], S["psd"], bn=(bn2[0], bn2[1]))
            g = bn_finish(g, st, r2, bn2, Lc, t + "8", t + "6.bias", 3)
            conv_wgrad(lay[t + "6"], r1, g, s2=bn1[2], t2=bn1[3])
            g, st = cg(lay[t + "6"], g, want_stats=True, ep=bn_ep(r1, bn1))
            g = bn_finish(g, st, r1, bn1, Lb, t + "5", t + "3.bias", 2)
            conv_wgrad(lay[t + "3"], r0, g, s2=bn0[2], t2=bn0[3])
            g, st = cg(lay[t + "3"], g, want_stats=True, ep=bn_ep(r0, bn0))
            g = bn_finish(g, st, r0, bn0, La, t + "2", t + "0.bias", 1)
            conv_wgrad(lay[t + "0"], y4, g, s1=n4[2], t1=n4[3], swish=True, s2=bn_n[2], t2=bn_n[3])
            xp4 = (n4[2], n4[3])
            g, st = cg(lay[t + "0"], g, want_stats=True, ep=bn_ep(y4, bn_n, xp4))
            da = bn_finish(g, st, y4, bn_n, L4, "sex_classifier.norm", None, 0, xp=xp4)
            flush_pending()
            if need_stage["sex_classifier"]:
                buckets.reduce_stage("sex_classifier")
            return da

        def decoder_bwd():
            d_rec = torch.zeros(B, T, 80, device=dev) if recon_unused else d_recon
            g_rec = d_rec.reshape(B, Ltot).contiguous().float()
            if need["decoder.8.bias"]:
                setg("decoder.8.bias", ops.sum_partials(g_rec.view(4 * B, Ltot // 4), 1, n=Ltot // 4).sum())
            if need["decoder.8.weight"] and model.fused_bwd1c:
                g, st, G["decoder.8.weight"] = ops.bwd1C(g_rec, y8, P["decoder.8.weight"], newg("decoder.8.weight"),
                                                         n8[2], n8[3], n8[0], n8[1])
            else:
                if need["decoder.8.weight"]:
                    G["decoder.8.weight"] = ops.wgrad1C(g_rec, y8, newg("decoder.8.weight"), flip=True,
                                                        s1=n8[2], t1=n8[3], swish=True)
                g, st = ops.conv1toC(g_rec, P["decoder.8.weight"], None, dt, flip=True, want_stats=True,
                                     ep=dict(x=y8, s1=n8[2], t1=n8[3], mean=n8[0], rstd=n8[1]))
            g = in_finish(g, st, y8, n8, 32, Ltot, "decoder.6", "decoder.5.bias")
            conv_wgrad(lay["decoder.5"], y7, g)
            g, st = cg(lay["decoder.5"], g, want_stats=True)
            bias_from(st, "decoder.4.bias", 64)
            conv_wgrad(lay["decoder.4"], y6, g, s1=n6[2], t1=n6[3], swish=True)
            g, st = cg(lay["decoder.4"], g, want_stats=True, ep=_in_ep(y6, n6))
            g = in_finish(g, st, y6, n6, 64, L2, "decoder.2", "decoder.1.bias")
            conv_wgrad(lay["decoder.1"], y5, g)
            g, st = cg(lay["decoder.1"], g, want_stats=True)
            bias_from(st, "decoder.0.bias", 128)
            conv_wgrad(lay["decoder.0"], y4, g, s1=n4[2], t1=n4[3], swish=True)
            flush_pending()
            if need_stage["decoder"]:
                buckets.reduce_stage("decoder")
            return g

        da4_cls = tdnn_bwd(head_bwd())
        if not run_decoder:
            return finish()
        g = decoder_bwd()
        if not run_encoder:
            return finish()

        g, st = cg(lay["decoder.0"], g, want_stats=True, ep=_in_ep(y4, n4, g2=da4_cls))
        for conv, norm, y, nrm, x, nx in (("encoder.11", "encoder.12", y4, n4, y3, n3),
                                          ("encoder.8", "encoder.9", y3, n3, y2, n2),
                                          ("encoder.5", "encoder.6", y2, n2, y1, n1),
                                          ("encoder.2", "encoder.3", y1, n1, y0, None)):
            ly = lay[conv]
            g = in_finish(g, st, y, nrm, ly.cout, y.shape[1], norm, ly.bias)
            conv_wgrad(ly, x, g, swish=True, **(dict(s1=nx[2], t1=nx[3]) if nx else {}))
            g, st = cg(ly, g, want_stats=True, ep=_in_ep(x, nx) if nx else dict(mode=1, x=x))
        bias_from(st, "encoder.0.bias", 32)
        if need["encoder.0.weight"]:
            G["encoder.0.weight"] = ops.wgrad1C(S["x0"], g, newg("encoder.0.weight"))
        d_feats = None
        if ctx.need_input_grad:
            d_feats = ops.convCto1(g, P["encoder.0.weight"], None, flip=True).view(B, T, 80)
        flush_pending()
        if need_stage["encoder"]:
            buckets.reduce_stage("encoder")
        return finish(d_feats)
```

### speech-anonymization_amd/csrc/sa_head.hip

```cpp
#include "sa_common.h"

template <typename T>
__global__ __launch_bounds__(256) void sa_pool_fwd_kernel(const T* __restrict__ r,
                                                          const float* __restrict__ sc,
                                                          const float* __restrict__ sh,
                                                          float* __restrict__ part, int L,
                                                          int nseg) {
  constexpr int C = 128, VEC = Tr<T>::VEC, CH = C / VEC, RPB = 256 / CH, NG = 128 / RPB;
  __shared__ float tile[RPB][C][2];
  const int tid = threadIdx.x, b = blockIdx.y, grp = blockIdx.x % NG, seg = blockIdx.x / NG;
  const int c = tid % CH, rl = tid / CH, lm = grp * RPB + rl;
  float s[VEC], t[VEC], sum[VEC], sq[VEC];
#pragma unroll
  for (int j = 0; j < VEC; ++j) { s[j] = sc[c * VEC + j]; t[j] = sh[c * VEC + j]; sum[j] = 0.f; sq[j] = 0.f; }
  const int nk = (L + 127) / 128, per = (nk + nseg - 1) / nseg;
  const int kbeg = seg * per, kend = (kbeg + per < nk) ? kbeg + per : nk;
  const T* rb = r + (size_t)b * L * C + c * VEC;
  for (int k0 = kbeg; k0 < kend; k0 += 4) {
    uint4 raw[4];
#pragma unroll
    for (int i = 0; i < 4; ++i) {
      const int l = lm + 128 * (k0 + i);
      raw[i] = make_uint4(0, 0, 0, 0);
      if (k0 + i < kend && l < L) raw[i] = *reinterpret_cast<const uint4*>(rb + (size_t)l * C);
    }
#pragma unroll
    for (int i = 0; i < 4; ++i) {
      const int l = lm + 128 * (k0 + i);
      if (k0 + i < kend && l < L) {
        float f[VEC];
        Tr<T>::unpack(raw[i], f);
#pragma unroll
        for (int j = 0; j < VEC; ++j) {
          const float v = fmaf(f[j], s[j], t[j]);
          sum[j] += v; sq[j] = fmaf(v, v, sq[j]);
        }
      }
    }
  }
#pragma unroll
  for (int j = 0; j < VEC; ++j) { tile[rl][c * VEC + j][0] = sum[j]; tile[rl][c * VEC + j][1] = sq[j]; }
  __syncthreads();
  float* dst = part + ((size_t)b * nseg + seg) * C * 128 * 2;
  for (int e = tid; e < RPB * C * 2; e += 256) {
    const int cc = e / (RPB * 2), w = e % (RPB * 2);
    dst[((size_t)cc * 128 + grp * RPB) * 2 + w] = tile[w >> 1][cc][w & 1];
  }
}

__global__ __launch_bounds__(1024) void sa_pool_gather_kernel(const float* __restrict__ part, int nseg,
                                                              int L, double* __restrict__ sums) {
  __shared__ double grp[7][128][2];
  const int tid = threadIdx.x, b = blockIdx.x, j = tid & 127, h = tid >> 7, Lm = L % 128;
  double s = 0.0, q = 0.0;
  for (int seg = 0; seg < nseg; ++seg) {
    const float2* p = reinterpret_cast<const float2*>(part) + ((size_t)b * nseg + seg) * 128 * 128;
#pragma unroll 16
    for (int c = h * 16; c < h * 16 + 16; ++c) {
      const float2 v = p[(size_t)c * 128 + ((j - c * Lm) & 127)];
      s += v.x; q += v.y;
    }
  }
  if (h > 0) { grp[h - 1][j][0] = s; grp[h - 1][j][1] = q; }
  __syncthreads();
  if (h == 0) {
#pragma unroll
    for (int g = 0; g < 7; ++g) { s += grp[g][j][0]; q += grp[g][j][1]; }
    sums[((size_t)b * 128 + j) * 2 + 0] = s;
    sums[((size_t)b * 128 + j) * 2 + 1] = q;
  }
}

extern "C" int sa_pool_nseg(int B) {
  int n = 2048 / (B * 16);
  return n < 1 ? 1 : (n > 8 ? 8 : n);
}

extern "C" int sa_pool_fwd(int dtype, const void* r, const float* scale, const float* shift,
                           float* part, int B, int L, int nseg, void* stream) {
  if (!r || !scale || !shift || !part || B <= 0 || L <= 1 || nseg < 1) return -22;
  hipStream_t st = reinterpret_cast<hipStream_t>(stream);
  if (dtype == SA_BF16)
    hipLaunchKernelGGL(sa_pool_fwd_kernel<bf16_t>, dim3(8 * nseg, B), dim3(256), 0, st,
                       reinterpret_cast<const bf16_t*>(r), scale, shift, part, L, nseg);
  else
    hipLaunchKernelGGL(sa_pool_fwd_kernel<float>, dim3(16 * nseg, B), dim3(256), 0, st,
                       reinterpret_cast<const float*>(r), scale, shift, part, L, nseg);
  hipError_t e = hipGetLastError();
  return e == hipSuccess ? 0 : -(int)e;
}

extern "C" int sa_pool_gather(const float* part, int B, int nseg, int L, double* sums, void* stream) {
  if (!part || !sums || B <= 0 || nseg < 1) return -22;
  hipLaunchKernelGGL(sa_pool_gather_kernel, dim3(B), dim3(1024), 0,
                     reinterpret_cast<hipStream_t>(stream), part, nseg, L, sums);
  hipError_t e = hipGetLastError();
  return e == hipSuccess ? 0 : -(int)e;
}

__global__ void sa_pool_fin_kernel(const double* __restrict__ sums, int B, int n,
                                   const float* __restrict__ noise, float eps, float* pooled,
                                   float* mean, float* stdraw) {
  const int i = blockIdx.x * blockDim.x + threadIdx.x;
  if (i >= B * 128) return;
  const int b = i / 128, j = i % 128;
  const double S = sums[2 * i], Q = sums[2 * i + 1];
  const double m = S / n;
  double var = (Q - S * m) / (n - 1);
  if (var < 0.0) var = 0.0;
  const float sd = (float)sqrt(var);
  mean[i] = (float)m; stdraw[i] = sd;
  float mo = (float)m;
  if (noise) mo += eps * ((1.0f - 9.0f) * noise[i] + 9.0f);
  pooled[(size_t)b * 256 + j] = mo;
  pooled[(size_t)b * 256 + 128 + j] = sd + eps;
}

extern "C" int sa_pool_fin(const double* sums, int B, int n, const float* noise, float eps,
                           float* pooled, float* mean, float* stdraw, void* stream) {
  if (!sums || !pooled || !mean || !stdraw || n < 2) return -22;
  hipLaunchKernelGGL(sa_pool_fin_kernel, dim3(sa_div_up(B * 128, 256)), dim3(256), 0,
                     reinterpret_cast<hipStream_t>(stream), sums, B, n, noise, eps, pooled, mean,
                     stdraw);
  hipError_t e = hipGetLastError();
  return e == hipSuccess ? 0 : -(int)e;
}

template <typename T>
__global__ __launch_bounds__(256) void sa_pool_bwd_kernel(const T* __restrict__ r,
                                                          const float* __restrict__ sc,
                                                          const float* __restrict__ sh,
                                                          const float* __restrict__ dpooled,
                                                          const float* __restrict__ mean,
                                                          const float* __restrict__ stdraw,
                                                          T* __restrict__ g, int L,
                                                          const float* __restrict__ bn_mean,
                                                          const float* __restrict__ bn_rstd,
                                                          float* __restrict__ stats) {
  constexpr int C = 128, VEC = Tr<T>::VEC, CH = C / VEC, RPP = 256 / CH;
  __shared__ float ka[128], kb[128];
  __shared__ float red[RPP][C][2];
  const int tid = threadIdx.x, b = blockIdx.y, l0 = blockIdx.x * SA_WAVE * 4;
  if (tid < 128) {
    const float dm = dpooled[(size_t)b * 256 + tid], ds = dpooled[(size_t)b * 256 + 128 + tid];
    const float sd = stdraw[(size_t)b * 128 + tid], m = mean[(size_t)b * 128 + tid];
    const float inv = sd > 0.0f ? 1.0f / ((float)(L - 1) * sd) : 0.0f;
    kb[tid] = ds * inv;
    ka[tid] = dm / (float)L - ds * inv * m;
  }
  __syncthreads();
  const int c = tid % CH, r0 = tid / CH;
  float s[VEC], t[VEC];
  int jb[VEC];
#pragma unroll
  for (int j = 0; j < VEC; ++j) {
    s[j] = sc[c * VEC + j]; t[j] = sh[c * VEC + j];
    jb[j] = (int)(((long long)(c * VEC + j) * L) % 128);
  }
  float bm[VEC], br[VEC], s1[VEC], s2[VEC];
#pragma unroll
  for (int j = 0; j < VEC; ++j) {
    bm[j] = stats ? bn_mean[c * VEC + j] : 0.0f;
    br[j] = stats ? bn_rstd[c * VEC + j] : 0.0f;
    s1[j] = 0.0f; s2[j] = 0.0f;
  }
  for (int rr = r0; rr < 256; rr += RPP) {
    const int l = l0 + rr;
    if (l >= L) break;
    float f[VEC], x[VEC];
    Tr<T>::unpack(*reinterpret_cast<const uint4*>(r + ((size_t)b * L + l) * C + c * VEC), x);
#pragma unroll
    for (int j = 0; j < VEC; ++j) {
      const int col = (jb[j] + l) % 128;
      f[j] = fmaf(kb[col], fmaf(x[j], s[j], t[j]), ka[col]);
    }
    const uint4 u = Tr<T>::pack(f);
    *reinterpret_cast<uint4*>(g + ((size_t)b * L + l) * C + c * VEC) = u;
    if (stats) {
      Tr<T>::unpack(u, f);
#pragma unroll
      for (int j = 0; j < VEC; ++j) {
        s1[j] += f[j];
        s2[j] = fmaf(f[j], (x[j] - bm[j]) * br[j], s2[j]);
      }
    }
  }
  if (stats) {
#pragma unroll
    for (int j = 0; j < VEC; ++j) { red[r0][c * VEC + j][0] = s1[j]; red[r0][c * VEC + j][1] = s2[j]; }
    __syncthreads();
    if (tid < C) {
      float a0 = 0.0f, a1 = 0.0f;
#pragma unroll
      for (int q = 0; q < RPP; ++q) { a0 += red[q][tid][0]; a1 += red[q][tid][1]; }
      float* dst = stats + (((size_t)b * gridDim.x + blockIdx.x) * C + tid) * 2;
      dst[0] = a0; dst[1] = a1;
    }
  }
}

extern "C" int sa_pool_bwd(int dtype, const void* r, const float* scale, const float* shift,
                           const float* dpooled, const float* mean, const float* stdraw, void* g,
                           int B, int L, const float* bn_mean, const float* bn_rstd, float* stats,
                           void* stream) {
  if (!r || !scale || !shift || !dpooled || !mean || !stdraw || !g || L < 2) return -22;
  if (stats && (!bn_mean || !bn_rstd)) return -22;
  hipStream_t st = reinterpret_cast<hipStream_t>(stream);
  dim3 grid(sa_div_up(L, 256), B);
  if (dtype == SA_BF16)
    hipLaunchKernelGGL(sa_pool_bwd_kernel<bf16_t>, grid, dim3(256), 0, st,
                       reinterpret_cast<const bf16_t*>(r), scale, shift, dpooled, mean, stdraw,
                       reinterpret_cast<bf16_t*>(g), L, bn_mean, bn_rstd, stats);
  else
    hipLaunchKernelGGL(sa_pool_bwd_kernel<float>, grid, dim3(256), 0, st,
                       reinterpret_cast<const float*>(r), scale, shift, dpooled, mean, stdraw,
                       reinterpret_cast<float*>(g), L, bn_mean, bn_rstd, stats);
  hipError_t e = hipGetLastError();
  return e == hipSuccess ? 0 : -(int)e;
}

__global__ __launch_bounds__(256) void sa_dense_kernel(const float* __restrict__ X, int lda,
                                                       const float* __restrict__ ps,
                                                       const float* __restrict__ pt,
                                                       const float* __restrict__ W, int sbk, int sbn,
                                                       const float* __restrict__ bias, float* __restrict__ Y,
                                                       int ldy, int M, int N, int K, int relu) {
  __shared__ float part[4][16][64];
  const int lane = threadIdx.x & 63, wave = threadIdx.x >> 6, n0 = blockIdx.x * 32, m0 = blockIdx.y * 32;
  const int m = m0 + (lane & 31), n = n0 + (lane & 31), kh = lane >> 5;
  f32x16 acc;
#pragma unroll
  for (int i = 0; i < 16; ++i) acc[i] = 0.0f;
  for (int k0 = wave * 16; k0 < K; k0 += 64) {
    float av[8], bv[8];
#pragma unroll
    for (int u = 0; u < 8; ++u) {
      const int k = k0 + 2 * u + kh;
      av[u] = 0.0f; bv[u] = 0.0f;
      if (k < K) {
        if (m < M) {
          av[u] = X[(size_t)m * lda + k];
          if (ps) av[u] = fmaf(av[u], ps[k], pt[k]);
        }
        if (n < N) bv[u] = W[(size_t)k * sbk + (size_t)n * sbn];
      }
    }
#pragma unroll
    for (int u = 0; u < 8; ++u)
      if (k0 + 2 * u < K) acc = __builtin_amdgcn_mfma_f32_32x32x2f32(av[u], bv[u], acc, 0, 0, 0);
  }
#pragma unroll
  for (int i = 0; i < 16; ++i) part[wave][i][lane] = acc[i];
  __syncthreads();
  if (wave == 0 && n < N) {
    const float bb = bias ? bias[n] : 0.0f;
#pragma unroll
    for (int i = 0; i < 16; ++i) {
      const int mr = m0 + sa_acc_row(i, lane);
      if (mr < M) {
        float v = ((part[0][i][lane] + part[1][i][lane]) + part[2][i][lane]) + part[3][i][lane] + bb;
        if (relu) v = fmaxf(v, 0.0f);
        Y[(size_t)mr * ldy + n] = v;
      }
    }
  }
}

extern "C" int sa_dense(const float* X, int lda, const float* ps, const float* pt, const float* W,
                        int sbk, int sbn, const float* bias, float* Y, int ldy, int M, int N, int K,
                        int relu, void* stream) {
  if (!X || !W || !Y || M <= 0 || N <= 0 || K <= 0) return -22;
  dim3 grid(sa_div_up(N, 32), sa_div_up(M, 32));
  hipLaunchKernelGGL(sa_dense_kernel, grid, dim3(256), 0, reinterpret_cast<hipStream_t>(stream), X,
                     lda, ps, pt, W, sbk, sbn, bias, Y, ldy, M, N, K, relu);
  hipError_t e = hipGetLastError();
  return e == hipSuccess ? 0 : -(int)e;
}

__global__ void sa_colsums_kernel(const float* __restrict__ X, const float* __restrict__ H,
                                  const float* __restrict__ hm, const float* __restrict__ hr,
                                  int M, int N, double* sums, float* __restrict__ out0,
                                  float* __restrict__ out1) {
  const int n = blockIdx.x * blockDim.x + threadIdx.x;
  if (n >= N) return;
  double s = 0.0, q = 0.0;
#pragma unroll 8
  for (int m = 0; m < M; ++m) {
    const float x = X[(size_t)m * N + n];
    float h = H ? H[(size_t)m * N + n] : x;
    if (hm) h = (h - hm[n]) * hr[n];
    s += x; q += (double)x * h;
  }
  sums[2 * n] = s; sums[2 * n + 1] = q;
  if (out0) out0[n] = (float)s;
  if (out1) out1[n] = (float)q;
}

extern "C" int sa_colsums(const float* X, const float* H, const float* hmean, const float* hrstd,
                          int M, int N, double* sums, float* out0, float* out1, void* stream) {
  if (!X || !sums) return -22;
  hipLaunchKernelGGL(sa_colsums_kernel, dim3(sa_div_up(N, 64)), dim3(64), 0,
                     reinterpret_cast<hipStream_t>(stream), X, H, hmean, hrstd, M, N, sums, out0,
                     out1);
  hipError_t e = hipGetLastError();
  return e == hipSuccess ? 0 : -(int)e;
}

__global__ void sa_bn2d_bwd_kernel(const float* __restrict__ G, const float* __restrict__ H,
                                   const double* __restrict__ sums, double count,
                                   const float* __restrict__ gamma, const float* __restrict__ mean,
                                   const float* __restrict__ rstd, int relu_mask, int M, int N,
                                   float* dH, const double* __restrict__ count_dev) {
  const int i = blockIdx.x * blockDim.x + threadIdx.x;
  if (i >= M * N) return;
  if (count_dev) count = *count_dev;
  const int n = i % N;
  const float hh = (H[i] - mean[n]) * rstd[n];
  float v = gamma[n] * rstd[n] * (G[i] - (float)(sums[2 * n] / count) - hh * (float)(sums[2 * n + 1] / count));
  if (relu_mask && !(H[i] > 0.0f)) v = 0.0f;
  dH[i] = v;
}

extern "C" int sa_bn2d_bwd(const float* G, const float* H, const double* sums, double count,
                           const float* gamma, const float* mean, const float* rstd, int relu_mask,
                           int M, int N, float* dH, const double* count_dev, void* stream) {
  if (!G || !H || !sums || !gamma || !mean || !rstd || !dH) return -22;
  hipLaunchKernelGGL(sa_bn2d_bwd_kernel, dim3(sa_div_up(M * N, 256)), dim3(256), 0,
                     reinterpret_cast<hipStream_t>(stream), G, H, sums, count, gamma, mean, rstd,
                     relu_mask, M, N, dH, count_dev);
  hipError_t e = hipGetLastError();
  return e == hipSuccess ? 0 : -(int)e;
}

__global__ void sa_dense_wgrad_kernel(const float* __restrict__ dY, const float* __restrict__ X,
                                      const float* __restrict__ ps, const float* __restrict__ pt,
                                      int M, int N, int K, float* dW) {
  const int i = blockIdx.x * blockDim.x + threadIdx.x;
  if (i >= N * K) return;
  const int n = i / K, k = i % K;
  float s = 0.0f;
#pragma unroll 8
  for (int m = 0; m < M; ++m) {
    float x = X[(size_t)m * K + k];
    if (ps) x = fmaf(x, ps[k], pt[k]);
    s = fmaf(dY[(size_t)m * N + n], x, s);
  }
  dW[i] = s;
}

extern "C" int sa_dense_wgrad(const float* dY, const float* X, const float* ps, const float* pt,
                              int M, int N, int K, float* dW, void* stream) {
  if (!dY || !X || !dW) return -22;
  hipLaunchKernelGGL(sa_dense_wgrad_kernel, dim3(sa_div_up(N * K, 256)), dim3(256), 0,
                     reinterpret_cast<hipStream_t>(stream), dY, X, ps, pt, M, N, K, dW);
  hipError_t e = hipGetLastError();
  return e == hipSuccess ? 0 : -(int)e;
}

__global__ void sa_log_softmax_kernel(const float* __restrict__ X, float* __restrict__ Y, int M, int N) {
  const int m = blockIdx.x * blockDim.x + threadIdx.x;
  if (m >= M) return;
  float mx = -INFINITY;
  for (int n = 0; n < N; ++n) mx = fmaxf(mx, X[(size_t)m * N + n]);
  float s = 0.0f;
  for (int n = 0; n < N; ++n) s += expf(X[(size_t)m * N + n] - mx);
  const float lse = mx + logf(s);
  for (int n = 0; n < N; ++n) Y[(size_t)m * N + n] = X[(size_t)m * N + n] - lse;
}
__global__ void sa_log_softmax_bwd_kernel(const float* __restrict__ dY, const float* __restrict__ Y,
                                          float* __restrict__ dX, int M, int N) {
  const int m = blockIdx.x * blockDim.x + threadIdx.x;
  if (m >= M) return;
  float s = 0.0f;
  for (int n = 0; n < N; ++n) s += dY[(size_t)m * N + n];
  for (int n = 0; n < N; ++n) dX[(size_t)m * N + n] = dY[(size_t)m * N + n] - expf(Y[(size_t)m * N + n]) * s;
}
extern "C" int sa_log_softmax(const float* X, float* Y, int M, int N, void* stream) {
  if (!X || !Y) return -22;
  hipLaunchKernelGGL(sa_log_softmax_kernel, dim3(sa_div_up(M, 64)), dim3(64), 0,
                     reinterpret_cast<hipStream_t>(stream), X, Y, M, N);
  hipError_t e = hipGetLastError();
  return e == hipSuccess ? 0 : -(int)e;
}
extern "C" int sa_log_softmax_bwd(const float* dY, const float* Y, float* dX, int M, int N, void* stream) {
  if (!dY || !Y || !dX) return -22;
  hipLaunchKernelGGL(sa_log_softmax_bwd_kernel, dim3(sa_div_up(M, 64)), dim3(64), 0,
                     reinterpret_cast<hipStream_t>(stream), dY, Y, dX, M, N);
  hipError_t e = hipGetLastError();
  return e == hipSuccess ? 0 : -(int)e;
}

__global__ __launch_bounds__(256) void sa_recon_loss_kernel(const float* __restrict__ a,
                                                            const float* __restrict__ b, size_t n,
                                                            int kind, float* __restrict__ grad,
                                                            double* __restrict__ part) {
  __shared__ double wsum[4];
  const float inv = 1.0f / (float)n;
  double s = 0.0;
  const size_t n4 = n / 4;
  for (size_t i = (size_t)blockIdx.x * blockDim.x + threadIdx.x; i < n4; i += (size_t)gridDim.x * blockDim.x) {
    const float4 x = reinterpret_cast<const float4*>(a)[i], y = reinterpret_cast<const float4*>(b)[i];
    float d[4] = {x.x - y.x, x.y - y.y, x.z - y.z, x.w - y.w}, g[4];
#pragma unroll
    for (int j = 0; j < 4; ++j) {
      if (kind == 0) { s += fabsf(d[j]); g[j] = d[j] > 0.f ? inv : (d[j] < 0.f ? -inv : 0.f); }
      else { s += (double)d[j] * d[j]; g[j] = 2.0f * d[j] * inv; }
    }
    if (grad) reinterpret_cast<float4*>(grad)[i] = make_float4(g[0], g[1], g[2], g[3]);
  }
  if (blockIdx.x == 0 && threadIdx.x == 0)
    for (size_t i = n4 * 4; i < n; ++i) {
      const float d = a[i] - b[i];
      if (kind == 0) { s += fabsf(d); if (grad) grad[i] = d > 0.f ? inv : (d < 0.f ? -inv : 0.f); }
      else { s += (double)d * d; if (grad) grad[i] = 2.0f * d * inv; }
    }
  s = sa_wave_sum_d(s);
  if ((threadIdx.x & 63) == 0) wsum[threadIdx.x >> 6] = s;
  __syncthreads();
  if (threadIdx.x == 0) part[blockIdx.x] = wsum[0] + wsum[1] + wsum[2] + wsum[3];
}
__global__ void sa_recon_loss_fin_kernel(const double* part, int nb, double n, float* loss) {
  __shared__ double lane_sum[64];
  double s = 0.0;
#pragma unroll 8
  for (int i = threadIdx.x; i < nb; i += 64) s += part[i];
  lane_sum[threadIdx.x] = s;
  __syncthreads();
  if (threadIdx.x == 0) {
    double t = 0.0;
    for (int i = 0; i < 64; ++i) t += lane_sum[i];
    loss[0] = (float)(t / n);
  }
}
#define SA_LOSS_BLOCKS 512
extern "C" int sa_loss_workspace_bytes() { return SA_LOSS_BLOCKS * (int)sizeof(double); }
extern "C" int sa_recon_loss(const float* a, const float* b, long long n, int kind, float* grad,
                             float* loss, void* workspace, void* stream) {
  if (!a || !b || !loss || !workspace || n <= 0) return -22;
  if ((reinterpret_cast<uintptr_t>(a) | reinterpret_cast<uintptr_t>(b) |
       reinterpret_cast<uintptr_t>(grad)) & 15) return -22;
  hipStream_t st = reinterpret_cast<hipStream_t>(stream);
  int nb = (int)((n / 4 + 255) / 256);
  if (nb < 1) nb = 1;
  if (nb > SA_LOSS_BLOCKS) nb = SA_LOSS_BLOCKS;
  hipLaunchKernelGGL(sa_recon_loss_kernel, dim3(nb), dim3(256), 0, st, a, b, (size_t)n, kind, grad,
                     reinterpret_cast<double*>(workspace));
  hipLaunchKernelGGL(sa_recon_loss_fin_kernel, dim3(1), dim3(64), 0, st,
                     reinterpret_cast<const double*>(workspace), nb, (double)n, loss);
  hipError_t e = hipGetLastError();
  return e == hipSuccess ? 0 : -(int)e;
}

__global__ __launch_bounds__(64) void sa_cls_losses_kernel(const float* __restrict__ logp,
                                                           const long long* __restrict__ label, int B, int NC,
                                                           float* out, float* dnll, float* dconf) {
  __shared__ double pn[64], pc[64];
  const int t = threadIdx.x;
  double nll = 0.0, conf = 0.0;
  for (int e = t; e < B * NC; e += 64) {
    const int b = e / NC, c = e % NC;
    const float lp = logp[e];
    const float d = lp - (-0.6931f);
    conf += (double)d * d;
    if (dconf) dconf[e] = 2.0f * d / (float)(B * NC);
    const bool hit = (long long)c == label[b];
    if (hit) nll -= lp;
    if (dnll) dnll[e] = hit ? -1.0f / (float)B : 0.0f;
  }
  pn[t] = nll; pc[t] = conf;
  __syncthreads();
  if (t == 0) {
    double a = 0.0, q = 0.0;
    for (int i = 0; i < 64; ++i) { a += pn[i]; q += pc[i]; }
    out[0] = (float)(a / B);
    out[1] = (float)(q / (B * NC));
  }
}
extern "C" int sa_cls_losses(const float* logp, const long long* label, int B, int NC, float* out,
                             float* dnll, float* dconf, void* stream) {
  if (!logp || !label || !out) return -22;
  hipLaunchKernelGGL(sa_cls_losses_kernel, dim3(1), dim3(64), 0,
                     reinterpret_cast<hipStream_t>(stream), logp, label, B, NC, out, dnll, dconf);
  hipError_t e = hipGetLastError();
  return e == hipSuccess ? 0 : -(int)e;
}

__global__ __launch_bounds__(256) void sa_cosine_rows_kernel(const float* __restrict__ x1,
                                                             const float* __restrict__ x2,
                                                             int rows, int D, int S, float eps,
                                                             float* __restrict__ rowloss,
                                                             float* __restrict__ dx1) {
  const int row = blockIdx.x * 4 + (threadIdx.x >> 6), lane = threadIdx.x & 63;
  if (row >= rows) return;
  const float* a = x1 + (size_t)row * D;
  const float* b = x2 + (size_t)row * D;
  float dot = 0.f, na = 0.f, nb = 0.f;
  for (int i = lane; i < D; i += 64) { dot = fmaf(a[i], b[i], dot); na = fmaf(a[i], a[i], na); nb = fmaf(b[i], b[i], nb); }
  dot = sa_wave_sum(dot); na = sa_wave_sum(na); nb = sa_wave_sum(nb);
  const float den2 = fmaxf(na * nb, eps * eps);
  const float cs = dot / sqrtf(den2);
  if (lane == 0) rowloss[row] = 1.0f - cs;
  if (dx1) {
    const bool clamped = na * nb < eps * eps;
    const float inv = 1.0f / sqrtf(den2), k = -1.0f / (float)S;
    for (int i = lane; i < D; i += 64) {
      float g = b[i] * inv;
      if (!clamped) g -= cs * a[i] / na;
      dx1[(size_t)row * D + i] = k * g;
    }
  }
}
__global__ void sa_cosine_fin_kernel(const float* rowloss, int rows, int S, float* loss) {
  double s = 0.0;
  for (int i = 0; i < rows; ++i) s += rowloss[i];
  loss[0] = (float)(s / S);
}
extern "C" int sa_cosine_loss(const float* x1, const float* x2, int B, int S, int D, float* rowloss,
                              float* loss, float* dx1, void* stream) {
  if (!x1 || !x2 || !rowloss || !loss || B <= 0 || S <= 0 || D <= 0) return -22;
  hipStream_t st = reinterpret_cast<hipStream_t>(stream);
  const int rows = B * S;
  hipLaunchKernelGGL(sa_cosine_rows_kernel, dim3(sa_div_up(rows, 4)), dim3(256), 0, st, x1, x2, rows,
                     D, S, 1e-6f, rowloss, dx1);
  hipLaunchKernelGGL(sa_cosine_fin_kernel, dim3(1), dim3(1), 0, st, rowloss, rows, S, loss);
  hipError_t e = hipGetLastError();
  return e == hipSuccess ? 0 : -(int)e;
}
```

### speech-anonymization_amd/csrc/sa_head_fused.hip

```cpp
#include "sa_common.h"

#define SA_HEAD_MAXB 64

namespace {

constexpr int K0 = 256, N1 = 128, N2 = 64, NC = 2;

__device__ __forceinline__ void head_bn_fwd(const float* H, int M, int N, int n, const float* gamma, const float* beta,
                                            float eps, float momentum, float* run_mean, float* run_var,
                                            float* f , float* s_lds, float* t_lds) {
  double S = 0.0, Q = 0.0;
  for (int m = 0; m < M; ++m) { const float x = H[m * N + n]; S += x; Q += (double)x * x; }
  const double cnt = (double)M, mu = S / cnt;
  double var = Q / cnt - mu * mu;
  if (var < 0.0) var = 0.0;
  const float r = (float)(1.0 / sqrt(var + (double)eps));
  const float sc = gamma[n] * r, sh = beta[n] - (float)mu * sc;
  f[n] = (float)mu; f[N + n] = r; f[2 * N + n] = sc; f[3 * N + n] = sh;
  s_lds[n] = sc; t_lds[n] = sh;
  if (run_mean) {
    const double unb = cnt > 1.0 ? var * cnt / (cnt - 1.0) : var;
    run_mean[n] = (1.0f - momentum) * run_mean[n] + momentum * (float)mu;
    run_var[n] = (1.0f - momentum) * run_var[n] + momentum * (float)unb;
  }
}

}

struct SaHeadFwdArgs {
  const float* pooled;
  const float *w1, *b1, *g1, *be1; float *rm1, *rv1;
  const float *w2, *b2, *g2, *be2; float *rm2, *rv2;
  const float *w3, *b3;
  float *h1, *f1, *h2, *f2, *logp;
  int M; float eps, momentum;
};

constexpr int PITCH = 132;
template <int KC>
__device__ __forceinline__ void head_mfma_tile(f32x16& acc, const float* At, const float* Wt, int lane) {
  const float* ap = At + (lane & 31) * PITCH + (lane >> 5) * (KC / 2);
  const float* wp = Wt + (lane & 31) * PITCH + (lane >> 5) * (KC / 2);
#pragma unroll 4
  for (int j = 0; j < KC / 8; ++j) {
    const float4 av = *reinterpret_cast<const float4*>(ap + 4 * j), bv = *reinterpret_cast<const float4*>(wp + 4 * j);
    acc = __builtin_amdgcn_mfma_f32_32x32x2f32(av.x, bv.x, acc, 0, 0, 0);
    acc = __builtin_amdgcn_mfma_f32_32x32x2f32(av.y, bv.y, acc, 0, 0, 0);
    acc = __builtin_amdgcn_mfma_f32_32x32x2f32(av.z, bv.z, acc, 0, 0, 0);
    acc = __builtin_amdgcn_mfma_f32_32x32x2f32(av.w, bv.w, acc, 0, 0, 0);
  }
}

template <int KC, class XF>
__device__ __forceinline__ void head_stage(float* tile, const float* src, int ld, int k0, int rows, int nvalid, int tid,
                                           XF xf) {
  for (int i = tid; i < rows * (KC / 4); i += 256) {
    const int r = i / (KC / 4), q = i % (KC / 4);
    float4 v = make_float4(0.0f, 0.0f, 0.0f, 0.0f);
    if (r < nvalid) v = xf(*reinterpret_cast<const float4*>(src + (size_t)r * ld + k0 + 4 * q), k0 + 4 * q);
    *reinterpret_cast<float4*>(tile + r * PITCH + 4 * q) = v;
  }
}

__global__ __launch_bounds__(256) void sa_head_fwd_kernel(SaHeadFwdArgs a) {
  extern __shared__ __attribute__((aligned(16))) unsigned char smem[];
  const int M = a.M, tid = threadIdx.x, lane = tid & 63, wave = tid >> 6;
  const int MT = (M + 31) / 32;
  float* At = reinterpret_cast<float*>(smem);
  float* Wt = At + 64 * PITCH;
  float* H1 = Wt + 128 * PITCH;
  float* H2 = H1 + M * N1;
  float* s1 = H2 + M * N2; float* t1 = s1 + N1; float* s2 = t1 + N1; float* t2 = s2 + N2;
  float* lg = t2 + N2;
  auto ident = [](float4 v, int) { return v; };
  {
    f32x16 acc[2];
#pragma unroll
    for (int mt = 0; mt < 2; ++mt)
#pragma unroll
      for (int i = 0; i < 16; ++i) acc[mt][i] = 0.0f;
    for (int c = 0; c < 2; ++c) {
      head_stage<128>(At, a.pooled, K0, c * 128, 32 * MT, M, tid, ident);
      head_stage<128>(Wt, a.w1, K0, c * 128, N1, N1, tid, ident);
      __syncthreads();
      head_mfma_tile<128>(acc[0], At, Wt + wave * 32 * PITCH, lane);
      if (MT > 1) head_mfma_tile<128>(acc[1], At + 32 * PITCH, Wt + wave * 32 * PITCH, lane);
      __syncthreads();
    }
    const int n = wave * 32 + (lane & 31);
    const float bb = a.b1[n];
    for (int mt = 0; mt < MT; ++mt)
#pragma unroll
      for (int i = 0; i < 16; ++i) {
        const int m = mt * 32 + sa_acc_row(i, lane);
        if (m < M) { const float v = fmaxf(acc[mt][i] + bb, 0.0f); H1[m * N1 + n] = v; a.h1[(size_t)m * N1 + n] = v; }
      }
  }
  __syncthreads();
  if (tid < N1) head_bn_fwd(H1, M, N1, tid, a.g1, a.be1, a.eps, a.momentum, a.rm1, a.rv1, a.f1, s1, t1);
  __syncthreads();
  {
    head_stage<128>(At, H1, N1, 0, 32 * MT, M, tid, [&](float4 v, int k) {
      return make_float4(fmaf(v.x, s1[k], t1[k]), fmaf(v.y, s1[k + 1], t1[k + 1]), fmaf(v.z, s1[k + 2], t1[k + 2]),
                         fmaf(v.w, s1[k + 3], t1[k + 3]));
    });
    head_stage<128>(Wt, a.w2, N1, 0, N2, N2, tid, ident);
    __syncthreads();
    const int nt = wave & 1, mt = wave >> 1;
    if (mt < MT) {
      f32x16 acc;
#pragma unroll
      for (int i = 0; i < 16; ++i) acc[i] = 0.0f;
      head_mfma_tile<128>(acc, At + mt * 32 * PITCH, Wt + nt * 32 * PITCH, lane);
      const int n = nt * 32 + (lane & 31);
      const float bb = a.b2[n];
#pragma unroll
      for (int i = 0; i < 16; ++i) {
        const int m = mt * 32 + sa_acc_row(i, lane);
        if (m < M) { const float v = fmaxf(acc[i] + bb, 0.0f); H2[m * N2 + n] = v; a.h2[(size_t)m * N2 + n] = v; }
      }
    }
  }
  __syncthreads();
  if (tid < N2) head_bn_fwd(H2, M, N2, tid, a.g2, a.be2, a.eps, a.momentum, a.rm2, a.rv2, a.f2, s2, t2);
  __syncthreads();
  if (tid < M * NC) {
    const int m = tid / NC, c = tid % NC;
    float acc = 0.0f;
    for (int k = 0; k < N2; ++k) acc = fmaf(fmaf(H2[m * N2 + k], s2[k], t2[k]), a.w3[c * N2 + k], acc);
    lg[tid] = acc + a.b3[c];
  }
  __syncthreads();
  if (tid < M * NC) {
    const int m = tid / NC;
    const float x0 = lg[m * NC], x1 = lg[m * NC + 1], mx = fmaxf(x0, x1);
    const float lse = mx + logf(expf(x0 - mx) + expf(x1 - mx));
    a.logp[tid] = lg[tid] - lse;
  }
}

extern "C" int sa_head_fwd(const float* pooled, const float* w1, const float* b1, const float* g1, const float* be1,
                           float* rm1, float* rv1, const float* w2, const float* b2, const float* g2,
                           const float* be2, float* rm2, float* rv2, const float* w3, const float* b3,
                           float* h1, float* f1, float* h2, float* f2, float* logp, int M, float eps,
                           float momentum, void* stream) {
  if (!pooled || !w1 || !b1 || !g1 || !be1 || !w2 || !b2 || !g2 || !be2 || !w3 || !b3 || !h1 || !f1 || !h2 || !f2 ||
      !logp || M < 1 || M > SA_HEAD_MAXB)
    return -22;
  SaHeadFwdArgs a{pooled, w1, b1, g1, be1, rm1, rv1, w2, b2, g2, be2, rm2, rv2, w3, b3, h1, f1, h2, f2, logp, M, eps, momentum};
  const size_t lds = ((size_t)(64 + 128) * PITCH + (size_t)M * (N1 + N2 + NC) + 2 * (N1 + N2)) * sizeof(float);
  static bool attr_set = false;
  if (!attr_set) {
    hipError_t e = hipFuncSetAttribute(reinterpret_cast<const void*>(sa_head_fwd_kernel),
                                       hipFuncAttributeMaxDynamicSharedMemorySize, 160 * 1024);
    if (e != hipSuccess) return -(int)e;
    attr_set = true;
  }
  hipLaunchKernelGGL(sa_head_fwd_kernel, dim3(1), dim3(256), lds, reinterpret_cast<hipStream_t>(stream), a);
  hipError_t e = hipGetLastError();
  return e == hipSuccess ? 0 : -(int)e;
}

struct SaHeadBwdArgs {
  const float *dlogp, *logp, *pooled, *h1, *f1, *h2, *f2;
  const float *w1, *g1, *w2, *g2, *w3;
  float *dw1, *db1, *dg1, *dbe1, *dw2, *db2, *dg2, *dbe2, *dw3, *db3, *dpooled;
  int M;
};

__device__ __forceinline__ void head_bn_bwd(float* dN, const float* H, int M, int N, int n, const float* f,
                                            const float* gamma, float* dgamma, float* dbeta) {
  const float mean = f[n], rstd = f[N + n];
  double S1 = 0.0, S2 = 0.0;
  for (int m = 0; m < M; ++m) {
    const float g = dN[m * N + n], hh = (H[m * N + n] - mean) * rstd;
    S1 += g; S2 += (double)g * hh;
  }
  if (dbeta) dbeta[n] = (float)S1;
  if (dgamma) dgamma[n] = (float)S2;
  const float a1 = (float)(S1 / (double)M), a2 = (float)(S2 / (double)M), c = gamma[n] * rstd;
  for (int m = 0; m < M; ++m) {
    const float h = H[m * N + n], hh = (h - mean) * rstd;
    float v = c * (dN[m * N + n] - a1 - hh * a2);
    if (!(h > 0.0f)) v = 0.0f;
    dN[m * N + n] = v;
  }
}

__global__ __launch_bounds__(1024) void sa_head_bwd_kernel(SaHeadBwdArgs a) {
  extern __shared__ __attribute__((aligned(16))) unsigned char smem[];
  const int M = a.M, tid = threadIdx.x;
  const float* X = a.pooled;
  float* H1 = reinterpret_cast<float*>(smem);
  float* H2 = H1 + M * N1;
  float* D1 = H2 + M * N2;
  float* D2 = D1 + M * N1;
  float* DL = D2 + M * N2;
  for (int i = tid; i < M * N1 / 4; i += 1024) reinterpret_cast<float4*>(H1)[i] = reinterpret_cast<const float4*>(a.h1)[i];
  for (int i = tid; i < M * N2 / 4; i += 1024) reinterpret_cast<float4*>(H2)[i] = reinterpret_cast<const float4*>(a.h2)[i];
  if (tid < M) {
    const float d0 = a.dlogp[tid * NC], d1 = a.dlogp[tid * NC + 1], s = d0 + d1;
    DL[tid * NC] = d0 - expf(a.logp[tid * NC]) * s;
    DL[tid * NC + 1] = d1 - expf(a.logp[tid * NC + 1]) * s;
  }
  __syncthreads();
  const float* s2 = a.f2 + 2 * N2; const float* t2 = a.f2 + 3 * N2;
  const float* s1 = a.f1 + 2 * N1; const float* t1 = a.f1 + 3 * N1;
  if (tid < NC * N2) {
    const int c = tid / N2, k = tid % N2;
    float acc = 0.0f;
    for (int m = 0; m < M; ++m) acc = fmaf(DL[m * NC + c], fmaf(H2[m * N2 + k], s2[k], t2[k]), acc);
    if (a.dw3) a.dw3[tid] = acc;
  } else if (tid < NC * N2 + NC) {
    const int c = tid - NC * N2;
    float acc = 0.0f;
    for (int m = 0; m < M; ++m) acc += DL[m * NC + c];
    if (a.db3) a.db3[c] = acc;
  }
  for (int i = tid; i < M * N2; i += 1024) {
    const int m = i / N2, k = i % N2;
    D2[i] = fmaf(DL[m * NC], a.w3[k], DL[m * NC + 1] * a.w3[N2 + k]);
  }
  __syncthreads();
  if (tid < N2) head_bn_bwd(D2, H2, M, N2, tid, a.f2, a.g2, a.dg2, a.dbe2);
  __syncthreads();
  for (int i = tid; i < N2 * N1; i += 1024) {
    const int n = i / N1, k = i % N1;
    float acc = 0.0f;
    const float sk = s1[k], tk = t1[k];
    for (int m = 0; m < M; ++m) acc = fmaf(D2[m * N2 + n], fmaf(H1[m * N1 + k], sk, tk), acc);
    if (a.dw2) a.dw2[i] = acc;
  }
  if (tid < N2 && a.db2) {
    float acc = 0.0f;
    for (int m = 0; m < M; ++m) acc += D2[m * N2 + tid];
    a.db2[tid] = acc;
  }
  for (int i = tid; i < M * N1; i += 1024) {
    const int m = i / N1, k = i % N1;
    float acc = 0.0f;
#pragma unroll 8
    for (int n = 0; n < N2; ++n) acc = fmaf(D2[m * N2 + n], a.w2[n * N1 + k], acc);
    D1[i] = acc;
  }
  __syncthreads();
  if (tid < N1) head_bn_bwd(D1, H1, M, N1, tid, a.f1, a.g1, a.dg1, a.dbe1);
  __syncthreads();
  {
    const int kq = tid & 63, ng = tid >> 6;
    float acc[8][4];
#pragma unroll
    for (int r = 0; r < 8; ++r) { acc[r][0] = acc[r][1] = acc[r][2] = acc[r][3] = 0.0f; }
    for (int m = 0; m < M; ++m) {
      const float4 x = *reinterpret_cast<const float4*>(X + m * K0 + 4 * kq);
      const float4 d0 = *reinterpret_cast<const float4*>(D1 + m * N1 + 8 * ng);
      const float4 d1 = *reinterpret_cast<const float4*>(D1 + m * N1 + 8 * ng + 4);
      const float dv[8] = {d0.x, d0.y, d0.z, d0.w, d1.x, d1.y, d1.z, d1.w};
#pragma unroll
      for (int r = 0; r < 8; ++r) {
        acc[r][0] = fmaf(dv[r], x.x, acc[r][0]); acc[r][1] = fmaf(dv[r], x.y, acc[r][1]);
        acc[r][2] = fmaf(dv[r], x.z, acc[r][2]); acc[r][3] = fmaf(dv[r], x.w, acc[r][3]);
      }
    }
    if (a.dw1) {
#pragma unroll
      for (int r = 0; r < 8; ++r)
        *reinterpret_cast<float4*>(a.dw1 + (size_t)(8 * ng + r) * K0 + 4 * kq) = make_float4(acc[r][0], acc[r][1], acc[r][2], acc[r][3]);
    }
  }
  if (tid < N1 && a.db1) {
    float acc = 0.0f;
    for (int m = 0; m < M; ++m) acc += D1[m * N1 + tid];
    a.db1[tid] = acc;
  }
  if (a.dpooled) {
    const int kq = tid & 63, m0 = tid >> 6;
    float acc[4][4];
#pragma unroll
    for (int r = 0; r < 4; ++r) { acc[r][0] = acc[r][1] = acc[r][2] = acc[r][3] = 0.0f; }
#pragma unroll 2
    for (int n = 0; n < N1; ++n) {
      const float4 w = *reinterpret_cast<const float4*>(a.w1 + (size_t)n * K0 + 4 * kq);
#pragma unroll
      for (int r = 0; r < 4; ++r) {
        const int m = m0 + 16 * r;
        const float d = m < M ? D1[m * N1 + n] : 0.0f;
        acc[r][0] = fmaf(d, w.x, acc[r][0]); acc[r][1] = fmaf(d, w.y, acc[r][1]);
        acc[r][2] = fmaf(d, w.z, acc[r][2]); acc[r][3] = fmaf(d, w.w, acc[r][3]);
      }
    }
#pragma unroll
    for (int r = 0; r < 4; ++r) {
      const int m = m0 + 16 * r;
      if (m < M) *reinterpret_cast<float4*>(a.dpooled + (size_t)m * K0 + 4 * kq) = make_float4(acc[r][0], acc[r][1], acc[r][2], acc[r][3]);
    }
  }
}

extern "C" int sa_head_bwd(const float* dlogp, const float* logp, const float* pooled, const float* h1,
                           const float* f1, const float* h2, const float* f2, const float* w1, const float* g1,
                           const float* w2, const float* g2, const float* w3, float* dw1, float* db1, float* dg1,
                           float* dbe1, float* dw2, float* db2, float* dg2, float* dbe2, float* dw3, float* db3,
                           float* dpooled, int M, void* stream) {
  if (!dlogp || !logp || !pooled || !h1 || !f1 || !h2 || !f2 || !w1 || !g1 || !w2 || !g2 || !w3 || M < 1 ||
      M > SA_HEAD_MAXB)
    return -22;
  SaHeadBwdArgs a{dlogp, logp, pooled, h1, f1, h2, f2, w1, g1, w2, g2, w3,
                  dw1, db1, dg1, dbe1, dw2, db2, dg2, dbe2, dw3, db3, dpooled, M};
  const size_t lds = (size_t)M * (2 * N1 + 2 * N2 + NC) * sizeof(float);
  static bool attr_set = false;
  if (!attr_set) {
    hipError_t e = hipFuncSetAttribute(reinterpret_cast<const void*>(sa_head_bwd_kernel),
                                       hipFuncAttributeMaxDynamicSharedMemorySize, 160 * 1024);
    if (e != hipSuccess) return -(int)e;
    attr_set = true;
  }
  hipLaunchKernelGGL(sa_head_bwd_kernel, dim3(1), dim3(1024), lds, reinterpret_cast<hipStream_t>(stream), a);
  hipError_t e = hipGetLastError();
  return e == hipSuccess ? 0 : -(int)e;
}

extern "C" int sa_head_max_rows(void) { return SA_HEAD_MAXB; }
```

### speech-anonymization_amd/ops.py

```python
import collections
import ctypes as C
import functools
import sys

import torch

from . import _lib as L

UP2 = [[(1, 0), (0, 2), (-1, 4)], [(1, 1), (0, 3)]]


def taps_conv(K, dil, pad):
    return [[(k * dil - pad, k) for k in range(K)]]


def taps_conv_dgrad_s1(K, dil, pad):
    return [[(pad - k * dil, k) for k in range(K)]]


def taps_convT_dgrad(K=5, pad=2):
    return [[(k - pad, k) for k in range(K)]]


CONVT_WG_TAPS = [(1, 0), (1, 1), (0, 0), (0, 1), (-1, 0)]
# ... 148 lines not shown
        self.table = raw.to(dev)
        self.n = len(items)
        self.key = tuple(w.data_ptr() for _, w, _, _ in items)

    def refresh(self):
        if getattr(self, "fp8", False):
            L.check(L.load().sa_pack_scales_multi(_f(self.table), self.n, L.stream()), "sa_pack_scales_multi")
        L.check(L.load().sa_pack_weights_multi(_f(self.table), self.n, 64, L.stream()),
                "sa_pack_weights_multi")


@functools.lru_cache(maxsize=None)
def _conv_geometry(cin, cout, u, Lout):
    return L.load().sa_conv_gemm_ntiles(cin, cout, u, Lout)


def conv_impl(pingpong=False, tile_rows=0, ws=True):
    if pingpong:
        raise L.SaHipError("the ping-pong conv kernel was removed (it tied the one-tile kernel forward and lost "
                           "on the fused data gradients: DESIGN.md section 4); use ws=True or ws=False")
    lib = L.load()
    L.check(lib.sa_conv_gemm_set_impl(2 if ws else 0), "sa_conv_gemm_set_impl")
    L.check(lib.sa_conv_gemm_set_tile_rows(int(tile_rows)), "sa_conv_gemm_set_tile_rows")
    _conv_geometry.cache_clear()


def conv_gemm(x, wp, bias, cin, cout, sa, u, phases, Lout, s1=None, t1=None, s2=None, t2=None,
              swish=False, relu=False, want_stats=False, out=None, code=None, ep=None, a_out=None,
              nb=None, want_pro_stats=False):
    lib = L.load()
    B, Lin, _ = x.shape
    assert x.shape[2] == cin
    y = out if out is not None else torch.empty(B, Lout, cout, dtype=x.dtype, device=x.device)
    kc = L.dt_code(x.dtype) if code is None else code
    nt = _conv_geometry(cin, cout, u, Lout)
    stats = torch.empty(B, nt, cout, 2, dtype=torch.float32, device=x.device) if want_stats else None
    a = L.SaConvArgs()
    a.x, a.wp, a.bias, a.y = _f(x), _f(wp), _f(bias), _f(y)
    a.s1, a.t1, a.s2, a.t2 = _f(s1), _f(t1), _f(s2), _f(t2)
    a.swish, a.relu, a.stats = int(swish), int(relu), _f(stats)
    a.B, a.Lin, a.Lout = B, Lin, Lout
    a.taps = L.make_taps(phases)
    if kc == L.FP8:
        a.wscale = C.c_void_p(wp.data_ptr() + wp.numel() - 4)
    if a_out is not None:
        assert a_out.dtype == torch.bfloat16 and a_out.shape == x.shape
        a.a_out = _f(a_out)
    pro_stats = None
    if want_pro_stats:
        pro_stats = torch.empty(B, nt, cin, 2, dtype=torch.float32, device=x.device)
        a.pro_stats = _f(pro_stats)
    colsum = None
    if nb:
        assert nb["x"].shape == x.shape and nb["x"].dtype == x.dtype
        a.nb_x, a.nb_c1, a.nb_c2, a.nb_c3 = _f(nb["x"]), _f(nb["c1"]), _f(nb["c2"]), _f(nb["c3"])
        a.nb_bstride, a.nb_relu_mask = (0 if nb.get("per_c") else cin), int(bool(nb.get("relu_mask")))
        if nb.get("want_colsum"):
            colsum = torch.empty(B, nt, cin, dtype=torch.float32, device=x.device)
            a.nb_colsum = _f(colsum)
    if ep:
        a.ep_mode, a.ep_xp_is_act = int(ep["mode"]), int(bool(ep.get("xp_is_act")))
        a.ep_bstride = 0 if ep.get("per_c") else cout
        a.ep_x, a.ep_g2 = _f(ep["x"]), _f(ep.get("g2"))
        a.ep_s1, a.ep_t1 = _f(ep.get("s1")), _f(ep.get("t1"))
        a.ep_mean, a.ep_rstd = _f(ep.get("mean")), _f(ep.get("rstd"))
        if ep.get("g2k") is not None:
            a.ep_g2k1, a.ep_g2k2, a.ep_g2k3 = (_f(t) for t in ep["g2k"])
    e0 = PROFILE.start(f"conv_gemm({cin},{cout},{sa},{u})") if PROFILE.key else None
    L.check(lib.sa_conv_gemm(kc, cin, cout, sa, u, C.byref(a), L.stream()),
            f"sa_conv_gemm({cin},{cout},{sa},{u})")
    if e0 is not None:
        ntap = sum(len(p) for p in phases)
        esz = x.element_size()
        extra = (a_out.numel() * 2 if a_out is not None else 0)
        if ep:
            extra += y.numel() * esz * (2 if ep.get("g2") is not None else 1)
        if nb:
            extra += x.numel() * esz
        io = (x.numel() + y.numel()) * esz
        route = lib.sa_conv_gemm_route(kc, cin, cout, sa, u, C.byref(a))
        tname = {L.F32: "float", L.BF16: "bf16_t", L.BF16X3: "bf16x3_t", L.BF16X1F: "bf16x1f_t", L.FP8: "fp8_t"}[kc]
        ws_mode = (5 if s2 is not None else 0) if s1 is None else 3 if want_pro_stats else 4 if s2 is not None else 1
        kind = (f"sa_conv_wsd_kernel ({tname}, {cin}->{cout}; 5 instances)" if route == 3 else
                f"sa_conv_ws_kernel<{ws_mode},{ntap}> ({tname}, {cin}->{cout})" if route == 2 else
                f"sa_conv_gemm_kernel<{tname},{cin},{cout},{sa},{u}{',nb prologue' if nb else ''}>")
        PROFILE.stop(e0, io + ntap * cin * cout * esz + extra,
                     2 * B * (-(-Lout // u)) * ntap * cin * cout,
                     alg_bytes=io + (y.numel() * esz if ep else 0), kind=kind)
    out_t = (y, stats) if want_stats else (y,)
    if nb and nb.get("want_colsum"):
        out_t = out_t + (colsum,)
    if want_pro_stats:
        out_t = out_t + (pro_stats,)
    return out_t if len(out_t) > 1 else y


WGRAD_TARGET_WGS = {True: 256, False: 512}


def wgrad(x, dy, cin, cout, sa, u, taps, Mrows, dst, dst_strides, s1=None, t1=None, s2=None,
          t2=None, swish=False, accumulate=False, target_wgs=None, code=None, x_pre=False,
          dy_pre=False, defer=None):
    lib = L.load()
    B, Lin, _ = x.shape
    Ldy = dy.shape[1]
    if x_pre:
        assert x.dtype == torch.bfloat16 and code in (L.BF16X1F, L.BF16)
    nt = len(taps)
    kw = lib.sa_wgrad_kw(cin, cout)
    if target_wgs is None:
        target_wgs = WGRAD_TARGET_WGS[(cin // 32) * (cout // 32) >= 8]
    chunk = max(64, -(-Mrows * B // target_wgs))
    chunk = -(-chunk // 64) * 64
    nchunk = -(-Mrows // chunk)
    slabs = torch.empty(B * nchunk * kw * nt * cin * cout, dtype=torch.float32, device=x.device)
    a = L.SaWgradArgs()
    a.x, a.dy, a.slabs = _f(x), _f(dy), _f(slabs)
    a.s1, a.t1, a.s2, a.t2, a.swish = _f(s1), _f(t1), _f(s2), _f(t2), int(swish)
    a.B, a.Lin, a.Ldy, a.Mrows, a.chunk, a.nchunk, a.ntaps = B, Lin, Ldy, Mrows, chunk, nchunk, nt
    for i, (off, ph) in enumerate(taps):
        a.off[i], a.ph[i] = off, ph
    a.x_pre, a.dy_pre = int(x_pre), int(dy_pre)
    if dy_pre:
        assert x_pre and dy.dtype == torch.bfloat16
    L.check(lib.sa_wgrad((L.BF16X1F if dy_pre else L.dt_code(dy.dtype)) if code is None else code, cin, cout, sa, u,
                         C.byref(a), L.stream()),
            f"sa_wgrad({cin},{cout},{sa},{u})")
    sk, sn, st = dst_strides
    if defer is not None:
        defer.append((slabs, dst, B * nchunk * kw, nt, cin, cout, sk, sn, st, int(accumulate)))
        return dst
    L.check(lib.sa_wgrad_reduce(_f(slabs), _f(dst), B * nchunk * kw, nt, cin, cout, sk, sn, st,
                                int(accumulate), L.stream()), "sa_wgrad_reduce")
    return dst


def wgrad_reduce_multi(items):
    lib = L.load()
    for i0 in range(0, len(items), L.WRED_MAX):
        m = L.SaWredMulti()
        chunk = items[i0:i0 + L.WRED_MAX]
        m.n = len(chunk)
        for d, (slabs, dst, nslab, nt, cin, cout, sk, sn, st, acc) in zip(m.d, chunk):
            d.slabs, d.dst = slabs.data_ptr(), dst.data_ptr()
            d.nslab, d.ntaps, d.cin, d.cout, d.sk, d.sn, d.st, d.accumulate = nslab, nt, cin, cout, sk, sn, st, acc
        L.check(lib.sa_wgrad_reduce_multi(C.byref(m), L.stream()), "sa_wgrad_reduce_multi")


def conv1toC(x, w, bias, dtype, flip=False, want_stats=False, ep=None):
    lib = L.load()
    B, Ln = x.shape
    y = torch.empty(B, Ln, 32, dtype=dtype, device=x.device)
    nt = lib.sa_conv1toC_ntiles(Ln)
    stats = torch.empty(B, nt, 32, 2, dtype=torch.float32, device=x.device) if want_stats else None
    e = ep or {}
    L.check(lib.sa_conv1toC(L.dt_code(dtype), _f(x), _f(w), _f(bias), _f(y), B, Ln, int(flip),
                            _f(stats), _f(e.get("x")), _f(e.get("s1")), _f(e.get("t1")),
                            _f(e.get("mean")), _f(e.get("rstd")), L.stream()), "sa_conv1toC")
    return (y, stats) if want_stats else y


def convCto1(x, w, bias, s1=None, t1=None, swish=False, flip=False):
    lib = L.load()
    B, Ln, _ = x.shape
    y = torch.empty(B, Ln, dtype=torch.float32, device=x.device)
    L.check(lib.sa_convCto1(L.dt_code(x.dtype), _f(x), _f(w), _f(bias), _f(y), B, Ln, _f(s1), _f(t1),
                            int(swish), int(flip), L.stream()), "sa_convCto1")
    return y


def wgrad1C(u, v, dst, flip=False, s1=None, t1=None, swish=False, accumulate=False, chunk=2048):
    lib = L.load()
    B, Ln = u.shape
    nch = lib.sa_wgrad1C_nchunk(Ln, chunk)
    slabs = torch.empty(B * nch, 32 * 15, dtype=torch.float32, device=u.device)
    L.check(lib.sa_wgrad1C(L.dt_code(v.dtype), _f(u), _f(v), _f(slabs), B, Ln, chunk, int(flip),
                           _f(s1), _f(t1), int(swish), L.stream()), "sa_wgrad1C")
    L.check(lib.sa_sum_slabs(_f(slabs), _f(dst), B * nch, 32 * 15, int(accumulate), L.stream()),
            "sa_sum_slabs")
    return dst


def bwd1C(u, v, w, dst, s1, t1, mean, rstd, flip=True, accumulate=False, chunk=2048):
    lib = L.load()
    B, Ln = u.shape
    nch = lib.sa_wgrad1C_nchunk(Ln, chunk)
    g = torch.empty(B, Ln, 32, dtype=v.dtype, device=u.device)
    stats = torch.empty(B, lib.sa_conv1toC_ntiles(Ln), 32, 2, dtype=torch.float32, device=u.device)
    slabs = torch.empty(B * nch, 32 * 15, dtype=torch.float32, device=u.device)
    L.check(lib.sa_bwd1C(L.dt_code(v.dtype), _f(u), _f(v), _f(w), _f(g), _f(stats), _f(slabs), B, Ln, chunk,
                         int(flip), _f(s1), _f(t1), _f(mean), _f(rstd), L.stream()), "sa_bwd1C")
    L.check(lib.sa_sum_slabs(_f(slabs), _f(dst), B * nch, 32 * 15, int(accumulate), L.stream()),
            "sa_sum_slabs")
    return g, stats, dst


def sum_partials(part, nbatch, n=None, rows=False):
    lib = L.load()
    if n is None:
        n = part.shape[-2] * part.shape[-1]
    total = part.numel()
    nslab = total // (nbatch * n)
    if nbatch == 1 and nslab >= 512 and part.dim() == 4 and part.shape[0] > 1:
        R = part.shape[0]
        mid = torch.empty(R, n, dtype=torch.float64, device=part.device)
        L.check(lib.sa_sum_partials(_f(part), _f(mid), R, nslab // R, n, L.stream()), "sa_sum_partials")
        if rows:
            return mid
        out = torch.empty(1, n, dtype=torch.float64, device=part.device)
        L.check(lib.sa_sum_rows_d(_f(mid), _f(out), R, n, L.stream()), "sa_sum_rows_d")
        return out
    out = torch.empty(nbatch, n, dtype=torch.float64, device=part.device)
    L.check(lib.sa_sum_partials(_f(part), _f(out), nbatch, nslab, n, L.stream()), "sa_sum_partials")
    return out


def fin_in_fwd(sums, B, Cc, n, gamma, beta, eps=1e-5):
    lib = L.load()
    o = torch.empty(4, B, Cc, dtype=torch.float32, device=sums.device)
    L.check(lib.sa_fin_in_fwd(_f(sums), B, Cc, n, _f(gamma), _f(beta), C.c_float(eps), _f(o[0]),
                              _f(o[1]), _f(o[2]), _f(o[3]), L.stream()), "sa_fin_in_fwd")
    return o[0], o[1], o[2], o[3]


def fin_bn_fwd(sums, Cc, count, gamma, beta, run_mean=None, run_var=None, eps=1e-5, momentum=0.1,
               count_dev=None):
    lib = L.load()
    o = torch.empty(4, Cc, dtype=torch.float32, device=sums.device)
    L.check(lib.sa_fin_bn_fwd(_f(sums), sums.numel() // (2 * Cc), Cc, C.c_double(count), _f(gamma), _f(beta), C.c_float(eps),
                              C.c_float(momentum), _f(run_mean), _f(run_var), _f(o[0]), _f(o[1]),
                              _f(o[2]), _f(o[3]), _f(count_dev), L.stream()), "sa_fin_bn_fwd")
    return o[0], o[1], o[2], o[3]


def fin_bn_eval(Cc, gamma, beta, run_mean, run_var, eps=1e-5):
    lib = L.load()
    o = torch.empty(4, Cc, dtype=torch.float32, device=gamma.device)
    L.check(lib.sa_fin_bn_eval(Cc, _f(gamma), _f(beta), C.c_float(eps), _f(run_mean), _f(run_var),
                               _f(o[0]), _f(o[1]), _f(o[2]), _f(o[3]), L.stream()), "sa_fin_bn_eval")
    return o[0], o[1], o[2], o[3]


def fin_norm_bwd(sums, lsums, groups, Cc, n, gamma, mean, rstd, sign=1.0, dgamma=None, dbeta=None,
                 n_dev=None):
    lib = L.load()
    o = torch.empty(3, groups, dtype=torch.float32, device=sums.device)
    R = sums.numel() // (2 * groups)
    assert lsums is None or lsums.numel() == sums.numel()
    L.check(lib.sa_fin_norm_bwd(_f(sums), _f(lsums), R, groups, Cc, C.c_double(n), _f(gamma), _f(mean),
                                _f(rstd), C.c_float(sign), _f(o[0]), _f(o[1]), _f(o[2]), _f(dgamma),
                                _f(dbeta), _f(n_dev), L.stream()), "sa_fin_norm_bwd")
    return o[0], o[1], o[2]


def bias_multi(items):
    lib = L.load()
    dev = items[0][0].device
    rows = torch.empty(sum(nb * cc for _, nb, cc, _, _ in items), dtype=torch.float64, device=dev)
    rp, esz = rows.data_ptr(), 8
    for i0 in range(0, len(items), L.BIAS_MAX):
        m = L.SaBiasMulti()
        chunk = items[i0:i0 + L.BIAS_MAX]
        m.n = len(chunk)
        for d, (part, nb, cc, ncomp, db) in zip(m.d, chunk):
            d.part, d.rows, d.db = part.data_ptr(), rp, db.data_ptr()
            d.nbatch, d.nslab, d.C, d.ncomp = nb, part.numel() // (nb * cc * ncomp), cc, ncomp
            rp += nb * cc * esz
        L.check(lib.sa_bias_multi(C.byref(m), L.stream()), "sa_bias_multi")


def fin_bias(sums, B, Cc, db, ncomp=2):
    L.check(L.load().sa_fin_bias(_f(sums), B, Cc, ncomp, _f(db), L.stream()), "sa_fin_bias")
    return db


def ew(kind, g, x, Cc, out=None, g2=None, s1=None, t1=None, mean=None, rstd=None, c1=None, c2=None,
       c3=None, actbwd=False, xp_is_act=False, relu_mask=False, per_c=False, want_stats=True):
    lib = L.load()
    B, Ln, _ = x.shape
    nt = lib.sa_ew_ntiles(Ln)
    stats = torch.empty(B, nt, Cc, 2, dtype=torch.float32, device=x.device) if want_stats else None
    a = L.SaEwArgs()
    a.g, a.g2, a.x, a.out = _f(g), _f(g2), _f(x), _f(out)
    a.s1, a.t1, a.mean, a.rstd = _f(s1), _f(t1), _f(mean), _f(rstd)
    a.c1, a.c2, a.c3 = _f(c1), _f(c2), _f(c3)
    a.actbwd, a.xp_is_act, a.relu_mask = int(actbwd), int(xp_is_act), int(relu_mask)
    a.bstride = 0 if per_c else Cc
    a.stats, a.B, a.L = _f(stats), B, Ln
    fn = lib.sa_ew_stats if kind == "stats" else lib.sa_ew_apply
    L.check(fn(L.dt_code(x.dtype), Cc, C.byref(a), L.stream()), f"sa_ew_{kind}")
    return stats


def pooling_noise(setting, B, Cc, device):
    if setting is None or setting is False:
        return None
    if torch.is_tensor(setting):
        return setting.to(device=device, dtype=torch.float32).contiguous()
    g = torch.randn(B, Cc, device=device)
    g = g - g.min()
    return (g / g.max()).contiguous()


def pool_fwd(r, scale, shift, noise=None, eps=1e-5):
    lib = L.load()
    B, Ln, _ = r.shape
    nseg = lib.sa_pool_nseg(B)
    part = torch.empty(B, nseg, 128, 128, 2, dtype=torch.float32, device=r.device)
    L.check(lib.sa_pool_fwd(L.dt_code(r.dtype), _f(r), _f(scale), _f(shift), _f(part), B, Ln, nseg,
                            L.stream()), "sa_pool_fwd")
    sums = torch.empty(B, 128, 2, dtype=torch.float64, device=r.device)
    L.check(lib.sa_pool_gather(_f(part), B, nseg, Ln, _f(sums), L.stream()), "sa_pool_gather")
    pooled = torch.empty(B, 256, dtype=torch.float32, device=r.device)
    mean = torch.empty(B, 128, dtype=torch.float32, device=r.device)
    sd = torch.empty(B, 128, dtype=torch.float32, device=r.device)
    L.check(lib.sa_pool_fin(_f(sums), B, Ln, _f(noise), C.c_float(eps), _f(pooled), _f(mean), _f(sd),
                            L.stream()), "sa_pool_fin")
    return pooled, mean, sd


def pool_bwd(r, scale, shift, dpooled, mean, sd, bn=None):
    lib = L.load()
    B, Ln, _ = r.shape
    g = torch.empty_like(r)
    st = torch.empty(B, -(-Ln // 256), 128, 2, dtype=torch.float32, device=r.device) if bn else None
    L.check(lib.sa_pool_bwd(L.dt_code(r.dtype), _f(r), _f(scale), _f(shift), _f(dpooled), _f(mean),
                            _f(sd), _f(g), B, Ln, _f(bn[0]) if bn else None, _f(bn[1]) if bn else None,
                            _f(st), L.stream()), "sa_pool_bwd")
    return (g, st) if bn else g


def dense(X, W, bias, N, K, ps=None, pt=None, relu=False, transpose_w=False):
    lib = L.load()
    M = X.shape[0]
    Y = torch.empty(M, N, dtype=torch.float32, device=X.device)
    sbk, sbn = (W.shape[1], 1) if transpose_w else (1, W.shape[1])
    L.check(lib.sa_dense(_f(X), X.shape[1], _f(ps), _f(pt), _f(W), sbk, sbn, _f(bias), _f(Y), N, M, N,
                         K, int(relu), L.stream()), "sa_dense")
    return Y


def colsums(X, H=None, hmean=None, hrstd=None, out0=None, out1=None):
    lib = L.load()
    M, N = X.shape
    s = torch.empty(N, 2, dtype=torch.float64, device=X.device)
    for o in (out0, out1):
        assert o is None or (o.dtype == torch.float32 and o.numel() == N and o.is_contiguous())
    L.check(lib.sa_colsums(_f(X), _f(H), _f(hmean), _f(hrstd), M, N, _f(s), _f(out0), _f(out1), L.stream()),
            "sa_colsums")
    return s


def bn2d_bwd(G, H, sums, count, gamma, mean, rstd, relu_mask, count_dev=None):
    lib = L.load()
    M, N = G.shape
    dH = torch.empty_like(G)
    L.check(lib.sa_bn2d_bwd(_f(G), _f(H), _f(sums), C.c_double(count), _f(gamma), _f(mean), _f(rstd),
                            int(relu_mask), M, N, _f(dH), _f(count_dev), L.stream()), "sa_bn2d_bwd")
    return dH


def dense_wgrad(dY, X, dW, ps=None, pt=None):
    lib = L.load()
    M, N = dY.shape
    K = X.shape[1]
    L.check(lib.sa_dense_wgrad(_f(dY), _f(X), _f(ps), _f(pt), M, N, K, _f(dW), L.stream()),
            "sa_dense_wgrad")
    return dW


def head_max_rows():
    return L.load().sa_head_max_rows()


def head_fwd(pooled, P, bn1, bn2, eps=1e-5, momentum=0.1):
    M = pooled.shape[0]
    dev = pooled.device
    H1 = torch.empty(M, 128, dtype=torch.float32, device=dev)
    H2 = torch.empty(M, 64, dtype=torch.float32, device=dev)
    f1 = torch.empty(4, 128, dtype=torch.float32, device=dev)
    f2 = torch.empty(4, 64, dtype=torch.float32, device=dev)
    logp = torch.empty(M, 2, dtype=torch.float32, device=dev)
    L.check(L.load().sa_head_fwd(_f(pooled), _f(P["0.weight"]), _f(P["0.bias"]), _f(P["2.weight"]), _f(P["2.bias"]),
                                 _f(bn1.running_mean), _f(bn1.running_var), _f(P["3.weight"]), _f(P["3.bias"]),
                                 _f(P["5.weight"]), _f(P["5.bias"]), _f(bn2.running_mean), _f(bn2.running_var),
                                 _f(P["6.weight"]), _f(P["6.bias"]), _f(H1), _f(f1), _f(H2), _f(f2), _f(logp), M,
                                 C.c_float(eps), C.c_float(momentum), L.stream()), "sa_head_fwd")
    return H1, tuple(f1[i] for i in range(4)), H2, tuple(f2[i] for i in range(4)), logp


def head_bwd(dlogp, logp, pooled, H1, f1, H2, f2, P, grads):
    M = pooled.shape[0]
    dpooled = torch.empty(M, 256, dtype=torch.float32, device=pooled.device)
    g = lambda k: _f(grads.get(k))
    L.check(L.load().sa_head_bwd(_f(dlogp), _f(logp), _f(pooled), _f(H1), _f(f1[0]), _f(H2), _f(f2[0]),
                                 _f(P["0.weight"]), _f(P["2.weight"]), _f(P["3.weight"]), _f(P["5.weight"]),
                                 _f(P["6.weight"]), g("0.weight"), g("0.bias"), g("2.weight"), g("2.bias"),
                                 g("3.weight"), g("3.bias"), g("5.weight"), g("5.bias"), g("6.weight"), g("6.bias"),
                                 _f(dpooled), M, L.stream()), "sa_head_bwd")
    return dpooled


def log_softmax(X):
    Y = torch.empty_like(X)
    L.check(L.load().sa_log_softmax(_f(X), _f(Y), X.shape[0], X.shape[1], L.stream()), "sa_log_softmax")
    return Y


def log_softmax_bwd(dY, Y):
    dX = torch.empty_like(Y)
    L.check(L.load().sa_log_softmax_bwd(_f(dY), _f(Y), _f(dX), Y.shape[0], Y.shape[1], L.stream()),
            "sa_log_softmax_bwd")
    return dX


def recon_loss(a, b, kind, want_grad=True):
    lib = L.load()
    n = a.numel()
    if a.data_ptr() % 16:
        a = a.clone()
    if b.data_ptr() % 16:
        b = b.clone()
    loss = torch.empty(1, dtype=torch.float32, device=a.device)
    grad = torch.empty_like(a) if want_grad else None
    ws = torch.empty(lib.sa_loss_workspace_bytes() // 8, dtype=torch.float64, device=a.device)
    L.check(lib.sa_recon_loss(_f(a), _f(b), C.c_longlong(n), 0 if kind == "l1" else 1, _f(grad),
                              _f(loss), _f(ws), L.stream()), "sa_recon_loss")
    return loss, grad


def cls_losses(logp, label, want_grad=True):
    lib = L.load()
    B, NC = logp.shape
    out = torch.empty(2, dtype=torch.float32, device=logp.device)
    dn = torch.empty_like(logp) if want_grad else None
    dc = torch.empty_like(logp) if want_grad else None
    L.check(lib.sa_cls_losses(_f(logp), _f(label), B, NC, _f(out), _f(dn), _f(dc), L.stream()),
            "sa_cls_losses")
    return out, dn, dc


def cosine_loss(x1, x2, want_grad=False):
    lib = L.load()
    B, S, D = x1.shape
    rl = torch.empty(B * S, dtype=torch.float32, device=x1.device)
    loss = torch.empty(1, dtype=torch.float32, device=x1.device)
    dx1 = torch.empty_like(x1) if want_grad else None
    L.check(lib.sa_cosine_loss(_f(x1), _f(x2), B, S, D, _f(rl), _f(loss), _f(dx1), L.stream()),
            "sa_cosine_loss")
    return loss, dx1


def cosine_rows(x1, x2):
    lib = L.load()
    B, D = x1.shape
    x1, x2 = x1.contiguous().float(), x2.contiguous().float()
    rl = torch.empty(B, dtype=torch.float32, device=x1.device)
    loss = torch.empty(1, dtype=torch.float32, device=x1.device)
    L.check(lib.sa_cosine_loss(_f(x1), _f(x2), B, 1, D, _f(rl), _f(loss), None, L.stream()),
            "sa_cosine_loss")
    return 1.0 - rl


def cluster_mi(X, y, idx=None, ncls=2, k=3):
    lib = L.load()
    iters, n = (idx.shape if idx is not None else (1, X.shape[0]))
    mi = torch.empty(iters, dtype=torch.float32, device=X.device)
    L.check(lib.sa_cluster_mi(_f(X), _f(y), _f(idx), iters, n, X.shape[1], ncls, k, _f(mi), L.stream()),
            "sa_cluster_mi")
    return mi


def add_layernorm(x, r, gamma, beta, eps, save):
    d = x.shape[-1]
    rows = x.numel() // d
    y = torch.empty_like(x)
    s = torch.empty_like(x) if save else None
    stat = torch.empty(rows, 2, dtype=torch.float32, device=x.device) if save else None
    L.check(L.load().sa_add_layernorm_fwd(_f(x), _f(r), _f(gamma), _f(beta), _f(y), _f(s), _f(stat), rows, d,
                                          C.c_float(eps), L.stream()), "sa_add_layernorm_fwd")
    return y, s, stat


def layernorm_bwd(dy, s, stat, gamma):
    d = s.shape[-1]
    ds = torch.empty_like(s)
    L.check(L.load().sa_layernorm_bwd(_f(dy), _f(s), _f(stat), _f(gamma), _f(ds), s.numel() // d, d, L.stream()),
            "sa_layernorm_bwd")
    return ds


def reflect_pad(x):
    B, T, F_, Cc = x.shape
    y = torch.empty(B, T + 2, F_ + 2, Cc, dtype=x.dtype, device=x.device)
    L.check(L.load().sa_reflect_pad_fwd(_f(x), _f(y), B, T, F_, Cc, L.stream()), "sa_reflect_pad_fwd")
    return y


def reflect_pad_bwd(dy):
    B, T2, F2, Cc = dy.shape
    dx = torch.empty(B, T2 - 2, F2 - 2, Cc, dtype=dy.dtype, device=dy.device)
    L.check(L.load().sa_reflect_pad_bwd(_f(dy), _f(dx), B, T2 - 2, F2 - 2, Cc, L.stream()), "sa_reflect_pad_bwd")
    return dx


def ln_leaky(x, gamma, beta, eps, slope, save):
    d = gamma.numel()
    rows = x.numel() // d
    y = torch.empty_like(x)
    stat = torch.empty(rows, 2, dtype=torch.float32, device=x.device) if save else None
    L.check(L.load().sa_ln_leaky_fwd(_f(x), _f(gamma), _f(beta), _f(y), _f(stat), rows, d, C.c_float(eps),
                                     C.c_float(slope), L.stream()), "sa_ln_leaky_fwd")
    return y, stat


def ln_leaky_bwd(dy, x, stat, gamma, beta, slope):
    d = gamma.numel()
    dx = torch.empty_like(x)
    L.check(L.load().sa_ln_leaky_bwd(_f(dy), _f(x), _f(stat), _f(gamma), _f(beta), _f(dx), x.numel() // d, d,
                                     C.c_float(slope), L.stream()), "sa_ln_leaky_bwd")
    return dx


def asr_block0(x, w, bias, gamma, beta, eps, slope, save):
    B, T, F_ = x.shape
    Cc = w.shape[0]
    To = (T - 1) // 2 + 1
    y = torch.empty(B, To, (F_ - 1) // 2 + 1, Cc, dtype=x.dtype, device=x.device)
    stat = torch.empty(B * To, 2, dtype=torch.float32, device=x.device) if save else None
    L.check(L.load().sa_asr_block0_fwd(_f(x), _f(w), _f(bias), _f(gamma), _f(beta), _f(y), _f(stat), B, T, F_, Cc,
                                       C.c_float(eps), C.c_float(slope), L.stream()), "sa_asr_block0_fwd")
    return y, stat


def asr_block0_bwd(dy, x, w, bias, gamma, beta, stat, slope):
    B, T, F_ = x.shape
    To = (T - 1) // 2 + 1
    part = torch.empty(B * To, 3, F_ + 2, dtype=torch.float32, device=x.device)
    dx = torch.empty_like(x)
    L.check(L.load().sa_asr_block0_bwd(_f(dy), _f(x), _f(w), _f(bias), _f(gamma), _f(beta), _f(stat), _f(part), _f(dx),
                                       B, T, F_, w.shape[0], C.c_float(slope), L.stream()), "sa_asr_block0_bwd")
    return dx


def clip_flats(flats, max_norm, eps=1e-6):
    f = L.SaFlats()
    f.n = len(flats)
    for d, t in zip(f.f, flats):
        d.p, d.n = t.data_ptr(), t.numel()
    dev = flats[0].device
    partials = torch.empty(L.FLATS_MAX * 64, dtype=torch.float64, device=dev)
    total = torch.empty((), dtype=torch.float32, device=dev)
    L.check(L.load().sa_clip_grads(C.byref(f), C.c_float(max_norm), C.c_float(eps), _f(partials), _f(total), L.stream()),
            "sa_clip_grads")
    return total


def _aug_in(t, what, dtype=torch.float32, shape=None, family="augmentation"):
    if not torch.is_tensor(t) or not t.is_cuda:
        raise L.SaHipError(f"{what}: the {family} kernels take GPU tensors (no CPU fallback)")
    if t.dtype != dtype:
        raise L.SaHipError(f"{what}: expected {dtype}, got {t.dtype}")
    if not t.is_contiguous():
        raise L.SaHipError(f"{what}: expected a contiguous tensor")
    if shape is not None and tuple(t.shape) != tuple(shape):
        raise L.SaHipError(f"{what}: expected shape {tuple(shape)}, got {tuple(t.shape)}")
    return t


def wav_abs_sums(wav, noise=None):
    if _aug_in(wav, "wav").dim() != 2 or wav.numel() == 0:
        raise L.SaHipError(f"wav: expected [B, L] with B, L >= 1, got {tuple(wav.shape)}")
    B, Lw = wav.shape
    if noise is not None:
        _aug_in(noise, "noise", shape=(B, Lw))
    sums = torch.empty(2, B, dtype=torch.float64, device=wav.device)
    L.check(L.load().sa_wav_abs_sums(_f(wav), _f(noise), B, Lw, _f(sums), L.stream()), "sa_wav_abs_sums")
    return sums


def noise_scales(sums, lens, snr, Lw):
    B = _aug_in(lens, "lens").numel()
    _aug_in(sums, "sums", torch.float64, (2, B))
    _aug_in(snr, "snr", shape=(B,))
    scales = torch.empty(B, 2, dtype=torch.float32, device=sums.device)
    L.check(L.load().sa_noise_scales(_f(sums), _f(lens), _f(snr), B, int(Lw), _f(scales), L.stream()),
            "sa_noise_scales")
    return scales


def wav_augment(wav, noise, scales, plan_words, R, Lp, S_in, S_out, W, first_min, first_max):
    if _aug_in(wav, "wav").dim() != 2 or wav.numel() == 0:
        raise L.SaHipError(f"wav: expected [B, L] with B, L >= 1, got {tuple(wav.shape)}")
    B, Lw = wav.shape
    if R not in (B, 2 * B):
        raise L.SaHipError(f"R = {R}: the output has B = {B} rows, or 2 B with noise rows")
    if R == 2 * B:
        _aug_in(noise, "noise", shape=(B, Lw))
        _aug_in(scales, "scales", shape=(B, 2))
    else:
        noise = scales = None
    from . import augment
    need = S_out + S_out * W + 101 + R * (1 + 2 * augment.max_chunks())
    if _aug_in(plan_words, "plan", torch.int32).numel() < need:
        raise L.SaHipError(f"plan: {plan_words.numel()} words, the geometry needs {need}")
    out = torch.empty(R, Lp, dtype=torch.float32, device=wav.device)
    L.check(L.load().sa_wav_augment(_f(wav), _f(noise), _f(scales), _f(plan_words), B, Lw, R, int(Lp), int(S_in),
                                    int(S_out), int(W), int(first_min), int(first_max), _f(out), L.stream()),
            "sa_wav_augment")
    return out


SPECAUG_TILE = 32


def _specaug_shape(x, what):
    if _aug_in(x, what).dim() != 3:
        raise L.SaHipError(f"{what}: expected [B, T, F], got {tuple(x.shape)}")
    B, T, F = x.shape
    if B < 1 or B > 65535 or T < 1 or F < 4 or F % 4 or F > 128:
        raise L.SaHipError(f"{what}: [B, T, F] = {tuple(x.shape)} -- B in 1..65535, T >= 1, F a multiple of 4 up to 128")
    if x.data_ptr() % 16:
        raise L.SaHipError(f"{what}: expected 16-byte aligned storage")
    return B, T, F


def _specaug_plan(words, B, T):
    from . import specaug
    need = specaug.plan_words(B, T)
    if _aug_in(words, "plan", torch.int32).numel() < need:
        raise L.SaHipError(f"plan: {words.numel()} words, the geometry needs {need}")


def specaug_warp_sums(x, plan_words):
    B, T, F = _specaug_shape(x, "x")
    _specaug_plan(plan_words, B, T)
    out = torch.empty_like(x)
    part = torch.empty(-(-T // SPECAUG_TILE) * B, 2, dtype=torch.float64, device=x.device)
    L.check(L.load().sa_specaug_warp_sums(_f(x), _f(plan_words), B, T, F, _f(out), _f(part), L.stream()),
            "sa_specaug_warp_sums")
    return out, part


def specaug_finalize(part, plan_words, B, T, F):
    B, T, F = int(B), int(T), int(F)
    _aug_in(part, "part", torch.float64, (-(-T // SPECAUG_TILE) * B, 2))
    _specaug_plan(plan_words, B, T)
    vals = torch.empty(2, dtype=torch.float32, device=part.device)
    L.check(L.load().sa_specaug_finalize(_f(part), _f(plan_words), B, T, F, _f(vals), L.stream()),
            "sa_specaug_finalize")
    return vals


def specaug_fill(out, plan_words, vals):
    B, T, F = _specaug_shape(out, "out")
    _specaug_plan(plan_words, B, T)
    _aug_in(vals, "vals", shape=(2,))
    L.check(L.load().sa_specaug_fill(_f(plan_words), _f(vals), B, T, F, _f(out), L.stream()), "sa_specaug_fill")
    return out


GL_MAX_B, GL_MAX_T = 65535, 1 << 23


_gl_in = functools.partial(_aug_in, family="vocoder")


def _gl_spec(t, what, dtype, family_in=_gl_in, t_min=2):
    if family_in(t, what, dtype).dim() != 3 or t.shape[2] != 201:
        raise L.SaHipError(f"{what}: expected [B, T, 201], got {tuple(t.shape)}")
    B, T, _ = t.shape
    if t_min is not None and (B < 1 or B > GL_MAX_B or T < t_min or T > GL_MAX_T):
        raise L.SaHipError(f"{what}: [B, T] = [{B}, {T}] -- B in 1..{GL_MAX_B} (a grid extent), T in "
                           f"{t_min}..{GL_MAX_T}")
    return B, T


def _gl_tables(window, twiddle):
    _gl_in(window, "window", shape=(400,))
    _gl_in(twiddle, "twiddle", shape=(800,))


def mel_to_mag(x, mean, std, M, frames=None):
    if _gl_in(x, "x").dim() != 3 or x.shape[2] != 80:
        raise L.SaHipError(f"x: expected [B, Tf, 80], got {tuple(x.shape)}")
    B, Tf, _ = x.shape
    T = Tf if frames is None else int(frames)
    if B < 1 or B > GL_MAX_B or T < 1 or T > Tf or T > GL_MAX_T:
        raise L.SaHipError(f"x: [B, Tf] = [{B}, {Tf}], frames = {T} -- B in 1..{GL_MAX_B}, frames in 1..Tf")
    _gl_in(mean, "mean", shape=(80,))
    _gl_in(std, "std", shape=(80,))
    _gl_in(M, "M", shape=(80, 201))
    S = torch.empty(B, T, 201, dtype=torch.float32, device=x.device)
    L.check(L.load().sa_mel_to_mag(_f(x), _f(mean), _f(std), _f(M), B, T, Tf, _f(S), L.stream()), "sa_mel_to_mag")
    return S


def gl_istft(C, window, twiddle):
    B, T = _gl_spec(C, "C", torch.complex64)
    _gl_tables(window, twiddle)
    y = torch.empty(B, (T - 1) * 160, dtype=torch.float32, device=C.device)
    L.check(L.load().sa_gl_istft(_f(C), _f(window), _f(twiddle), B, T, _f(y), L.stream()), "sa_gl_istft")
    return y


def gl_project(y, S, Tprev, m, window, twiddle):
    B, T = _gl_spec(S, "S", torch.float32)
    _gl_in(Tprev, "Tprev", torch.complex64, (B, T, 201))
    _gl_in(y, "y", shape=(B, (T - 1) * 160))
    _gl_tables(window, twiddle)
    Cn, R = torch.empty_like(Tprev), torch.empty_like(Tprev)
    L.check(L.load().sa_gl_project(_f(y), _f(S), _f(Tprev), C.c_float(float(m)), _f(window), _f(twiddle), B, T,
                                   _f(Cn), _f(R), L.stream()), "sa_gl_project")
    return Cn, R


YIN_HOP, YIN_TMAX = 160, 266
PN_MAX_N = 1 << 30

_pn_in = functools.partial(_aug_in, family="pitch")


def _pn_rows(t, what, dtype=torch.float32):
    if _pn_in(t, what, dtype).dim() != 2 or t.numel() == 0:
        raise L.SaHipError(f"{what}: expected [B, N] with B, N >= 1, got {tuple(t.shape)}")
    B, N = t.shape
    if B > GL_MAX_B or N > PN_MAX_N:
        raise L.SaHipError(f"{what}: [B, N] = [{B}, {N}] -- B up to {GL_MAX_B} (a grid extent), N up to {PN_MAX_N}")
    return B, N


def yin_f0(wav, threshold=0.15, return_dprime=False):
    B, N = _pn_rows(wav, "wav")
    T = N // YIN_HOP + 1
    f0 = torch.empty(B, T, dtype=torch.float32, device=wav.device)
    dp = torch.empty(B, T, YIN_TMAX + 1, dtype=torch.float32, device=wav.device) if return_dprime else None
    L.check(L.load().sa_yin_f0(_f(wav), B, N, C.c_float(float(threshold)), _f(f0), _f(dp), L.stream()), "sa_yin_f0")
    return (f0, dp) if return_dprime else f0


def pitch_ratio(f0, lens, N, target_hz=170.0, r_min=0.5, r_max=2.0, min_voiced=5):
    B, T = _pn_rows(f0, "f0")
# ... 506 lines not shown
```

Baseline: 3.995 million frames/s.

## Fuse loss tail, pooling gather/finish, and widen head backward kernel

The recon L1 and sex NLL losses, their weighted sum, the gradients and the non-finite count are now computed in two native kernels. Backward then runs straight from the precomputed gradients, skipping the autograd loss graph. The pooling gather and finish kernels are merged into one launch that also applies raw Gaussian noise inline. The classifier-head backward gets a multi-workgroup variant. The aim is fewer small launches and less Python/autograd overhead in the step tail, at the cost of more code paths and stricter eligibility checks.

```diff
diff --git a/include/sa_hip.h b/include/sa_hip.h
--- a/include/sa_hip.h
+++ b/include/sa_hip.h
@@ -147,6 +147,8 @@
 int sa_pool_gather(const float* part, int B, int nseg, int L, double* sums, void* stream);
 int sa_pool_fin(const double* sums, int B, int n, const float* noise, float eps, float* pooled,
                 float* mean, float* stdraw, void* stream);
+int sa_pool_gather_fin(const float* part, int B, int nseg, int L, const float* noise, int raw, float eps,
+                       float* pooled, float* mean, float* stdraw, void* stream);
 int sa_pool_bwd(int dtype, const void* r, const float* scale, const float* shift,
                 const float* dpooled, const float* mean, const float* stdraw, void* g, int B, int L,
                 const float* bn_mean, const float* bn_rstd, float* stats, void* stream);
@@ -169,6 +171,10 @@
                   float* dconf, void* stream);
 int sa_cosine_loss(const float* x1, const float* x2, int B, int S, int D, float* rowloss,
                    float* loss, float* dx1, void* stream);
+int sa_recon_loss_part(const float* a, const float* b, long long n, int kind, float* grad, float gscale,
+                       void* workspace, void* stream);
+int sa_step_loss(const void* workspace, long long n, const float* logp, const long long* label, int B, int NC,
+                 float w_recon, float w_sex, float* out, float* dlogp, int* nonfinite, void* stream);
 
 int sa_head_fwd(const float* pooled, const float* w1, const float* b1, const float* g1, const float* be1,
                 float* rm1, float* rv1, const float* w2, const float* b2, const float* g2, const float* be2,
@@ -178,6 +184,11 @@
                 const float* h2, const float* f2, const float* w1, const float* g1, const float* w2,
                 const float* g2, const float* w3, float* dw1, float* db1, float* dg1, float* dbe1, float* dw2,
                 float* db2, float* dg2, float* dbe2, float* dw3, float* db3, float* dpooled, int M, void* stream);
+int sa_head_bwd_wide(const float* dlogp, const float* logp, const float* pooled, const float* h1, const float* f1,
+                     const float* h2, const float* f2, const float* w1, const float* g1, const float* w2,
+                     const float* g2, const float* w3, float* dw1, float* db1, float* dg1, float* dbe1, float* dw2,
+                     float* db2, float* dg2, float* dbe2, float* dw3, float* db3, float* dpooled, int M,
+                     void* stream);
 int sa_head_max_rows(void);
 
 int sa_tdnn_fwd(const float* x, const void* wp, const float* bias, const float* bn_s, const float* bn_t,
diff --git a/speech-anonymization_amd/_lib.py b/speech-anonymization_amd/_lib.py
--- a/speech-anonymization_amd/_lib.py
+++ b/speech-anonymization_amd/_lib.py
@@ -97,13 +97,13 @@
     "sa_conv1toC", "sa_conv1toC_ntiles", "sa_convCto1", "sa_wgrad1C", "sa_wgrad1C_nchunk", "sa_bwd1C",
     "sa_sum_slabs", "sa_ew_stats", "sa_ew_apply", "sa_ew_ntiles",
     "sa_sum_partials", "sa_sum_rows_d", "sa_fin_in_fwd", "sa_fin_bn_fwd", "sa_fin_bn_eval", "sa_fin_norm_bwd", "sa_fin_bias",
-    "sa_pool_fwd", "sa_pool_nseg", "sa_pool_gather", "sa_pool_fin", "sa_pool_bwd", "sa_dense", "sa_colsums",
+    "sa_pool_fwd", "sa_pool_nseg", "sa_pool_gather", "sa_pool_fin", "sa_pool_gather_fin", "sa_pool_bwd", "sa_dense", "sa_colsums",
     "sa_bn2d_bwd", "sa_dense_wgrad", "sa_log_softmax", "sa_log_softmax_bwd",
-    "sa_loss_workspace_bytes", "sa_recon_loss", "sa_cls_losses", "sa_cosine_loss",
+    "sa_loss_workspace_bytes", "sa_recon_loss", "sa_cls_losses", "sa_cosine_loss", "sa_recon_loss_part", "sa_step_loss",
     "sa_tdnn_fwd", "sa_time_pool", "sa_leaky_affine", "sa_tdnn_bwd_input", "sa_tdnn_fold", "sa_time_pool_bwd",
     "sa_leaky_affine_bwd", "sa_cluster_mi", "sa_fbank", "sa_fbank_table_elems", "sa_fbank_ntiles", "sa_fbank_scratch_bytes", "sa_fbank_normalize", "sa_fbank_normalize_pair",
     "sa_comm_unique_id", "sa_comm_init", "sa_comm_world", "sa_comm_allreduce", "sa_comm_allreduce_inline", "sa_comm_join", "sa_comm_ncalls",
-    "sa_comm_destroy", "sa_head_fwd", "sa_head_bwd", "sa_head_max_rows",
+    "sa_comm_destroy", "sa_head_fwd", "sa_head_bwd", "sa_head_bwd_wide", "sa_head_max_rows",
     "sa_add_layernorm_fwd", "sa_layernorm_bwd", "sa_reflect_pad_fwd", "sa_reflect_pad_bwd", "sa_ln_leaky_fwd", "sa_ln_leaky_bwd", "sa_bias_multi", "sa_asr_block0_fwd", "sa_asr_block0_bwd", "sa_wgrad_reduce_multi", "sa_clip_grads",
     "sa_xv_tdnn_fwd_train", "sa_xv_tdnn_ntiles", "sa_xv_colsums", "sa_xv_tdnn_wgrad", "sa_xv_wgrad_reduce",
     "sa_xv_tdnn_dgrad", "sa_xv_pool_affine", "sa_xv_pool_affine_bwd",
diff --git a/speech-anonymization_amd/brain.py b/speech-anonymization_amd/brain.py
--- a/speech-anonymization_amd/brain.py
+++ b/speech-anonymization_amd/brain.py
@@ -99,6 +99,7 @@
         self.gc_freeze = bool(run_opts.get("gc_freeze", True))
         self.fused_clip = bool(run_opts.get("fused_clip", os.environ.get("SA_FUSED_CLIP", "1") == "1"))
         self.front_end_once = bool(run_opts.get("front_end_once", os.environ.get("SA_FRONT_END_ONCE", "1") == "1"))
+        self.step_tail = bool(run_opts.get("step_tail", os.environ.get("SA_STEP_TAIL", "1") == "1"))
         self.distributed_launch = bool(run_opts.get("distributed_launch", sdist.is_distributed()))
         self.modules = torch.nn.ModuleDict(modules or {})
         self.dp_batch_sizes = run_opts.get("dp_batch_sizes", "equal")
@@ -196,18 +197,23 @@
     def _count_nonfinite(self, loss):
         if not (self.lazy_finite_check and loss.is_cuda):
             return 0 if bool(torch.isfinite(loss)) else 1
-        st = getattr(self, "_finite_state", None)
-        if st is None:
-            st = self._finite_state = dict(dev=torch.zeros((), dtype=torch.int32, device=loss.device),
-                                           host=torch.zeros((), dtype=torch.int32).pin_memory(),
-                                           event=torch.cuda.Event(), seen=0, pending=False)
+        st = self._finite_counter(loss.device)
         new = self._poll_nonfinite()
-        st["dev"].add_((~torch.isfinite(loss.detach())).to(torch.int32))
+        if st.pop("counted", None) is not loss:
+            st["dev"].add_((~torch.isfinite(loss.detach())).to(torch.int32))
         st["host"].copy_(st["dev"], non_blocking=True)
         if not torch.cuda.is_current_stream_capturing():
             st["event"].record()
             st["pending"] = True
         return new
+
+    def _finite_counter(self, device):
+        st = getattr(self, "_finite_state", None)
+        if st is None:
+            st = self._finite_state = dict(dev=torch.zeros((), dtype=torch.int32, device=device),
+                                           host=torch.zeros((), dtype=torch.int32).pin_memory(),
+                                           event=torch.cuda.Event(), seen=0, pending=False)
+        return st
 
     def _poll_nonfinite(self, wait=False):
         st = getattr(self, "_finite_state", None)
@@ -351,6 +357,8 @@
             utility_loss = asr.utility_loss(asr_brain, hp.loss_utility, feats, reconstructed_speech,
                                             wav_lens, tokens_bos, batch)
         B = reconstructed_speech.shape[0]
+        if self._native_tail(stage, predictions):
+            return self._objectives_native(reconstructed_speech, sex_logits, feats, sex_label)
         recon_loss = hp.loss_reconstruction(reconstructed_speech.view(B, -1), feats.view(B, -1))
         sex_loss = hp.loss_sex_classification(sex_logits, sex_label)
         if hp.model_type == "endtoend":
@@ -388,6 +396,52 @@
                         ops.cosine_rows(recon_enc.reshape(nb, -1), orig_enc.reshape(nb, -1)))
         return loss
 
+    def _native_tail(self, stage=Stage.TRAIN, predictions=None):
+        from . import losses
+        hp = self.hparams
+        if not (self.step_tail and stage == Stage.TRAIN and self.__dict__.get("_in_fit_batch")
+                and self.device.type == "cuda" and hp.model_type == "convae"
+                and getattr(hp, "gradient_accumulation", 1) == 1
+                and isinstance(hp.loss_reconstruction, losses.ReconLoss)
+                and isinstance(hp.loss_sex_classification, losses.NLLLoss)):
+            return False
+        w = (hp.recon_loss_weight, hp.sex_loss_weight, hp.utility_loss_weight)
+        if not all(isinstance(x, (int, float)) and x == x and abs(x) != float("inf") for x in w):
+            return False
+        if not (w[2] == 0 or (w[2] > 0 and getattr(self, "asr_brain", None) is None)):
+            return False
+        if predictions is not None:
+            recon, logp = predictions
+            return bool(recon.is_cuda and recon.requires_grad and logp.requires_grad and logp.dim() == 2
+                        and recon.dtype == logp.dtype == torch.float32)
+        return True
+
+    def _objectives_native(self, recon, logp, feats, label):
+        from . import ops
+        hp = self.hparams
+        B = recon.shape[0]
+        st = self._finite_counter(recon.device) if self.lazy_finite_check else None
+        label = torch.as_tensor(label, device=logp.device).long().contiguous()
+        out, d_recon, d_logp = ops.step_loss(
+            recon.detach().view(B, -1).contiguous(), feats.detach().view(B, -1).contiguous().float(),
+            hp.loss_reconstruction.kind, logp.detach().contiguous(), label,
+            float(hp.recon_loss_weight), float(hp.sex_loss_weight), nonfinite=st["dev"] if st else None)
+        loss = out[2]
+        self.last_losses = dict(recon=out[0], sex=out[1])
+        self._tail = (loss, (recon, logp), (d_recon.view_as(recon), d_logp))
+        if st is not None:
+            st["counted"] = loss
+        return loss
+
+    def _backward(self, loss, accumulate=False):
+        tail, self._tail = self.__dict__.get("_tail"), None
+        if tail is not None and tail[0] is loss:
+            torch.autograd.backward(tail[1], tail[2])
+        elif accumulate:
+            (loss / self.hparams.gradient_accumulation).backward()
+        else:
+            loss.backward()
+
     def apply_epoch_schedule(self):
         hp = self.hparams
         if not getattr(hp, "epoch_parity_schedule", False):
@@ -431,12 +485,13 @@
                 tuple(bool(st.get(p)) for p in params if not p.requires_grad),
                 tuple(tok.shape), getattr(self, "asr_brain", None) is not None,
                 self.front_end_once, bool(not upd and getattr(nrm, "_count_positive", False)),
-                self.__dict__.get("_specaug") is not None)
+                self.__dict__.get("_specaug") is not None,
+                self._native_tail())
 
     def _step_core(self, batch):
         predictions = self.compute_forward(batch, Stage.TRAIN)
         loss = self.compute_objectives(predictions, batch, Stage.TRAIN)
-        loss.backward()
+        self._backward(loss)
         if getattr(self.hparams, "epoch_parity_schedule", False):
             self._zero_grads_of_frozen()
         self.check_gradients(loss)
@@ -503,11 +558,11 @@
         return ent["loss"]
 
     def fit_batch(self, batch):
-        self._target_stash, self._in_fit_batch = None, True
+        self._target_stash, self._in_fit_batch, self._tail = None, True, None
         try:
             return self._fit_batch(batch)
         finally:
-            self._target_stash, self._in_fit_batch = None, False
+            self._target_stash, self._in_fit_batch, self._tail = None, False, None
 
     def _fit_batch(self, batch):
         self.apply_epoch_schedule()
@@ -518,7 +573,7 @@
             batch = batch.to(self.device)
         predictions = self.compute_forward(batch, Stage.TRAIN)
         loss = self.compute_objectives(predictions, batch, Stage.TRAIN)
-        (loss / self.hparams.gradient_accumulation).backward()
+        self._backward(loss, accumulate=True)
         if self.step % self.hparams.gradient_accumulation == 0:
             if getattr(self.hparams, "epoch_parity_schedule", False):
                 self._zero_grads_of_frozen()
diff --git a/speech-anonymization_amd/convae.py b/speech-anonymization_amd/convae.py
--- a/speech-anonymization_amd/convae.py
+++ b/speech-anonymization_amd/convae.py
@@ -80,6 +80,8 @@
         self.sync_bn = sync_bn
         self.fused_head = os.environ.get("SA_FUSED_HEAD", "1") == "1"
         self.fused_bwd1c = os.environ.get("SA_FUSED_BWD1C", "1") == "1"
+        self.fused_pool_fin = os.environ.get("SA_FUSED_POOL_FIN", "1") == "1"
+        self.wide_head_bwd = os.environ.get("SA_WIDE_HEAD_BWD", "1") == "1"
         self.dp_batch_sizes = None
 
     def forward(self, feats):
@@ -308,7 +310,11 @@
         bn1 = bn_stats(st, B * Lb, cls.tdnn[5], "sex_classifier.tdnn.5", 128, 2)
         r2, st = cg(lay["sex_classifier.tdnn.6"], r1, s2=bn1[2], t2=bn1[3], relu=True, want_stats=True)
         bn2 = bn_stats(st, B * Lc, cls.tdnn[8], "sex_classifier.tdnn.8", 128, 3)
-        pooled, pmean, psd = ops.pool_fwd(r2, bn2[2], bn2[3], noise=_noise(model, B, feats.device))
+        if model.fused_pool_fin:
+            nz, raw = ops.pooling_noise_raw(model.pooling_noise, B, 128, feats.device)
+            pooled, pmean, psd = ops.pool_fwd(r2, bn2[2], bn2[3], noise=nz, fused=True, raw=raw)
+        else:
+            pooled, pmean, psd = ops.pool_fwd(r2, bn2[2], bn2[3], noise=_noise(model, B, feats.device))
         def head_fwd(X, n, local=False):
             H1 = ops.dense(X, P["sex_classifier.classify.0.weight"], P["sex_classifier.classify.0.bias"],
                            128, 256, relu=True)
@@ -333,10 +339,10 @@
         logp_all = logp
         if plan:
             logp = logp_all[plan[0]:plan[0] + B]
-        y6, n6, y7, y8, n8, recon = _decoder_launches(model, P, cg, inorm, y5, Ltot)
-
         if tracked:
             torch._foreach_add_(tracked, 1)
+        y6, n6, y7, y8, n8, recon = _decoder_launches(model, P, cg, inorm, y5, Ltot)
+
         S.update(x0=x0, y=[y0, y1, y2, y3, y4, y5, y6, y7, y8], r=[r0, r1, r2],
                  n=[None, n1, n2, n3, n4, None, n6, None, n8], bn=[bn_n, bn0, bn1, bn2], f=[f1, f2],
                  pooled=head_in, pmean=pmean, psd=psd, H1=H1, H2=H2, logp=logp_all, head_plan=plan,
@@ -507,7 +513,8 @@
                     if need[c + k]:
                         views[k] = G[c + k] = newg(c + k)
                 clsP = {k: P[c + k] for k in short}
-                return ops.head_bwd(dlp, S["logp"], S["pooled"], S["H1"], f1, S["H2"], f2, clsP, views)
+                return ops.head_bwd(dlp, S["logp"], S["pooled"], S["H1"], f1, S["H2"], f2, clsP, views,
+                                    wide=model.wide_head_bwd)
             glob = (lambda l: l) if local else (lambda l: model._bn_global(l)[0])
             cd = (lambda i: None) if local else cdev
             dLG = ops.log_softmax_bwd(dlp, S["logp"])
diff --git a/speech-anonymization_amd/csrc/sa_head.hip b/speech-anonymization_amd/csrc/sa_head.hip
--- a/speech-anonymization_amd/csrc/sa_head.hip
+++ b/speech-anonymization_amd/csrc/sa_head.hip
@@ -98,22 +98,70 @@
   return e == hipSuccess ? 0 : -(int)e;
 }
 
-__global__ void sa_pool_fin_kernel(const double* __restrict__ sums, int B, int n,
-                                   const float* __restrict__ noise, float eps, float* pooled,
-                                   float* mean, float* stdraw) {
-  const int i = blockIdx.x * blockDim.x + threadIdx.x;
-  if (i >= B * 128) return;
-  const int b = i / 128, j = i % 128;
-  const double S = sums[2 * i], Q = sums[2 * i + 1];
+__device__ __forceinline__ void sa_pool_finish(double S, double Q, int b, int j, int n, bool has_noise, float nz,
+                                               float eps, float* pooled, float* mean, float* stdraw) {
+  const int i = b * 128 + j;
   const double m = S / n;
   double var = (Q - S * m) / (n - 1);
   if (var < 0.0) var = 0.0;
   const float sd = (float)sqrt(var);
   mean[i] = (float)m; stdraw[i] = sd;
   float mo = (float)m;
-  if (noise) mo += eps * ((1.0f - 9.0f) * noise[i] + 9.0f);
+  if (has_noise) mo += eps * ((1.0f - 9.0f) * nz + 9.0f);
   pooled[(size_t)b * 256 + j] = mo;
   pooled[(size_t)b * 256 + 128 + j] = sd + eps;
+}
+
+__global__ void sa_pool_fin_kernel(const double* __restrict__ sums, int B, int n,
+                                   const float* __restrict__ noise, float eps, float* pooled,
+                                   float* mean, float* stdraw) {
+  const int i = blockIdx.x * blockDim.x + threadIdx.x;
+  if (i >= B * 128) return;
+  sa_pool_finish(sums[2 * i], sums[2 * i + 1], i / 128, i % 128, n, noise != nullptr, noise ? noise[i] : 0.0f, eps,
+                 pooled, mean, stdraw);
+}
+
+__global__ __launch_bounds__(1024) void sa_pool_gather_fin_kernel(const float* __restrict__ part, int nseg, int L,
+                                                                  int B, const float* __restrict__ noise, int raw,
+                                                                  float eps, float* pooled, float* mean,
+                                                                  float* stdraw) {
+  __shared__ double grp[7][128][2];
+  __shared__ float wmin[16], wmax[16];
+  const int tid = threadIdx.x, b = blockIdx.x, j = tid & 127, h = tid >> 7, Lm = L % 128;
+  float gmin = 0.0f, gmax = 0.0f;
+  if (noise && raw) {
+    float lo = INFINITY, hi = -INFINITY;
+    for (int i = tid; i < B * 128; i += 1024) { const float g = noise[i]; lo = fminf(lo, g); hi = fmaxf(hi, g); }
+#pragma unroll
+    for (int o = 32; o > 0; o >>= 1) { lo = fminf(lo, __shfl_xor(lo, o)); hi = fmaxf(hi, __shfl_xor(hi, o)); }
+    if ((tid & 63) == 0) { wmin[tid >> 6] = lo; wmax[tid >> 6] = hi; }
+  }
+  double s = 0.0, q = 0.0;
+  for (int seg = 0; seg < nseg; ++seg) {
+    const float2* p = reinterpret_cast<const float2*>(part) + ((size_t)b * nseg + seg) * 128 * 128;
+#pragma unroll 16
+    for (int c = h * 16; c < h * 16 + 16; ++c) {
+      const float2 v = p[(size_t)c * 128 + ((j - c * Lm) & 127)];
+      s += v.x; q += v.y;
+    }
+  }
+  if (h > 0) { grp[h - 1][j][0] = s; grp[h - 1][j][1] = q; }
+  __syncthreads();
+  if (h == 0) {
+#pragma unroll
+    for (int g = 0; g < 7; ++g) { s += grp[g][j][0]; q += grp[g][j][1]; }
+    float nz = 0.0f;
+    if (noise) {
+      nz = noise[b * 128 + j];
+      if (raw) {
+        gmin = wmin[0]; gmax = wmax[0];
+#pragma unroll
+        for (int w = 1; w < 16; ++w) { gmin = fminf(gmin, wmin[w]); gmax = fmaxf(gmax, wmax[w]); }
+        nz = __fdiv_rn(__fsub_rn(nz, gmin), __fsub_rn(gmax, gmin));
+      }
+    }
+    sa_pool_finish(s, q, b, j, L, noise != nullptr, nz, eps, pooled, mean, stdraw);
+  }
 }
 
 extern "C" int sa_pool_fin(const double* sums, int B, int n, const float* noise, float eps,
@@ -122,6 +170,15 @@
   hipLaunchKernelGGL(sa_pool_fin_kernel, dim3(sa_div_up(B * 128, 256)), dim3(256), 0,
                      reinterpret_cast<hipStream_t>(stream), sums, B, n, noise, eps, pooled, mean,
                      stdraw);
+  hipError_t e = hipGetLastError();
+  return e == hipSuccess ? 0 : -(int)e;
+}
+
+extern "C" int sa_pool_gather_fin(const float* part, int B, int nseg, int L, const float* noise, int raw,
+                                  float eps, float* pooled, float* mean, float* stdraw, void* stream) {
+  if (!part || !pooled || !mean || !stdraw || B <= 0 || nseg < 1 || L < 2) return -22;
+  hipLaunchKernelGGL(sa_pool_gather_fin_kernel, dim3(B), dim3(1024), 0, reinterpret_cast<hipStream_t>(stream),
+                     part, nseg, L, B, noise, raw, eps, pooled, mean, stdraw);
   hipError_t e = hipGetLastError();
   return e == hipSuccess ? 0 : -(int)e;
 }
@@ -390,10 +447,11 @@
   return e == hipSuccess ? 0 : -(int)e;
 }
 
+template <bool SCALED>
 __global__ __launch_bounds__(256) void sa_recon_loss_kernel(const float* __restrict__ a,
                                                             const float* __restrict__ b, size_t n,
                                                             int kind, float* __restrict__ grad,
-                                                            double* __restrict__ part) {
+                                                            double* __restrict__ part, float gscale) {
   __shared__ double wsum[4];
   const float inv = 1.0f / (float)n;
   double s = 0.0;
@@ -405,14 +463,18 @@
     for (int j = 0; j < 4; ++j) {
       if (kind == 0) { s += fabsf(d[j]); g[j] = d[j] > 0.f ? inv : (d[j] < 0.f ? -inv : 0.f); }
       else { s += (double)d[j] * d[j]; g[j] = 2.0f * d[j] * inv; }
+      if (SCALED) g[j] = __fmul_rn(g[j], gscale);
     }
     if (grad) reinterpret_cast<float4*>(grad)[i] = make_float4(g[0], g[1], g[2], g[3]);
   }
   if (blockIdx.x == 0 && threadIdx.x == 0)
     for (size_t i = n4 * 4; i < n; ++i) {
       const float d = a[i] - b[i];
-      if (kind == 0) { s += fabsf(d); if (grad) grad[i] = d > 0.f ? inv : (d < 0.f ? -inv : 0.f); }
-      else { s += (double)d * d; if (grad) grad[i] = 2.0f * d * inv; }
+      float g;
+      if (kind == 0) { s += fabsf(d); g = d > 0.f ? inv : (d < 0.f ? -inv : 0.f); }
+      else { s += (double)d * d; g = 2.0f * d * inv; }
+      if (SCALED) g = __fmul_rn(g, gscale);
+      if (grad) grad[i] = g;
     }
   s = sa_wave_sum_d(s);
   if ((threadIdx.x & 63) == 0) wsum[threadIdx.x >> 6] = s;
@@ -434,19 +496,33 @@
 }
 #define SA_LOSS_BLOCKS 512
 extern "C" int sa_loss_workspace_bytes() { return SA_LOSS_BLOCKS * (int)sizeof(double); }
+static int sa_loss_nblocks(long long n) {
+  long long nb = (n / 4 + 255) / 256;
+  return nb < 1 ? 1 : (nb > SA_LOSS_BLOCKS ? SA_LOSS_BLOCKS : (int)nb);
+}
 extern "C" int sa_recon_loss(const float* a, const float* b, long long n, int kind, float* grad,
                              float* loss, void* workspace, void* stream) {
   if (!a || !b || !loss || !workspace || n <= 0) return -22;
   if ((reinterpret_cast<uintptr_t>(a) | reinterpret_cast<uintptr_t>(b) |
        reinterpret_cast<uintptr_t>(grad)) & 15) return -22;
   hipStream_t st = reinterpret_cast<hipStream_t>(stream);
-  int nb = (int)((n / 4 + 255) / 256);
-  if (nb < 1) nb = 1;
-  if (nb > SA_LOSS_BLOCKS) nb = SA_LOSS_BLOCKS;
-  hipLaunchKernelGGL(sa_recon_loss_kernel, dim3(nb), dim3(256), 0, st, a, b, (size_t)n, kind, grad,
-                     reinterpret_cast<double*>(workspace));
+  const int nb = sa_loss_nblocks(n);
+  hipLaunchKernelGGL(sa_recon_loss_kernel<false>, dim3(nb), dim3(256), 0, st, a, b, (size_t)n, kind, grad,
+                     reinterpret_cast<double*>(workspace), 1.0f);
   hipLaunchKernelGGL(sa_recon_loss_fin_kernel, dim3(1), dim3(64), 0, st,
                      reinterpret_cast<const double*>(workspace), nb, (double)n, loss);
+  hipError_t e = hipGetLastError();
+  return e == hipSuccess ? 0 : -(int)e;
+}
+
+extern "C" int sa_recon_loss_part(const float* a, const float* b, long long n, int kind, float* grad,
+                                  float gscale, void* workspace, void* stream) {
+  if (!a || !b || !workspace || n <= 0) return -22;
+  if ((reinterpret_cast<uintptr_t>(a) | reinterpret_cast<uintptr_t>(b) |
+       reinterpret_cast<uintptr_t>(grad)) & 15) return -22;
+  hipLaunchKernelGGL(sa_recon_loss_kernel<true>, dim3(sa_loss_nblocks(n)), dim3(256), 0,
+                     reinterpret_cast<hipStream_t>(stream), a, b, (size_t)n, kind, grad,
+                     reinterpret_cast<double*>(workspace), gscale);
   hipError_t e = hipGetLastError();
   return e == hipSuccess ? 0 : -(int)e;
 }
@@ -481,6 +557,55 @@
   if (!logp || !label || !out) return -22;
   hipLaunchKernelGGL(sa_cls_losses_kernel, dim3(1), dim3(64), 0,
                      reinterpret_cast<hipStream_t>(stream), logp, label, B, NC, out, dnll, dconf);
+  hipError_t e = hipGetLastError();
+  return e == hipSuccess ? 0 : -(int)e;
+}
+
+__device__ __forceinline__ float sa_weighted_total(float wr, float recon, float ws, float sex) {
+#pragma clang fp contract(off)
+  const float a = wr * recon;
+  const float b = ws * sex;
+  const float s = a + b;
+  return s + 0.0f;
+}
+__global__ __launch_bounds__(64) void sa_step_loss_kernel(const double* __restrict__ part, int nb, double n,
+                                                          const float* __restrict__ logp,
+                                                          const long long* __restrict__ label, int B, int NC,
+                                                          float wr, float ws, float* __restrict__ out,
+                                                          float* __restrict__ dlogp, int* nonfinite) {
+  __shared__ double lane_sum[64], pn[64];
+  const int t = threadIdx.x;
+  double s = 0.0;
+#pragma unroll 8
+  for (int i = t; i < nb; i += 64) s += part[i];
+  const float gs = __fmul_rn(1.0f, ws);
+  double nll = 0.0;
+  for (int e = t; e < B * NC; e += 64) {
+    const int b = e / NC, c = e % NC;
+    const float lp = logp[e];
+    const bool hit = (long long)c == label[b];
+    if (hit) nll -= lp;
+    if (dlogp) dlogp[e] = __fmul_rn(hit ? -1.0f / (float)B : 0.0f, gs);
+  }
+  lane_sum[t] = s; pn[t] = nll;
+  __syncthreads();
+  if (t == 0) {
+    double r = 0.0, a = 0.0;
+    for (int i = 0; i < 64; ++i) r += lane_sum[i];
+    for (int i = 0; i < 64; ++i) a += pn[i];
+    const float recon = (float)(r / n), sex = (float)(a / B);
+    const float total = sa_weighted_total(wr, recon, ws, sex);
+    out[0] = recon; out[1] = sex; out[2] = total;
+    if (nonfinite && !isfinite(total)) *nonfinite += 1;
+  }
+}
+extern "C" int sa_step_loss(const void* workspace, long long n, const float* logp, const long long* label,
+                            int B, int NC, float w_recon, float w_sex, float* out, float* dlogp,
+                            int* nonfinite, void* stream) {
+  if (!workspace || !logp || !label || !out || n <= 0 || B <= 0 || NC <= 0) return -22;
+  hipLaunchKernelGGL(sa_step_loss_kernel, dim3(1), dim3(64), 0, reinterpret_cast<hipStream_t>(stream),
+                     reinterpret_cast<const double*>(workspace), sa_loss_nblocks(n), (double)n, logp, label, B, NC,
+                     w_recon, w_sex, out, dlogp, nonfinite);
   hipError_t e = hipGetLastError();
   return e == hipSuccess ? 0 : -(int)e;
 }
diff --git a/speech-anonymization_amd/csrc/sa_head_fused.hip b/speech-anonymization_amd/csrc/sa_head_fused.hip
--- a/speech-anonymization_amd/csrc/sa_head_fused.hip
+++ b/speech-anonymization_amd/csrc/sa_head_fused.hip
@@ -320,4 +320,132 @@
   return e == hipSuccess ? 0 : -(int)e;
 }
 
+#define SA_HEAD_BWD_WG 16
+constexpr int HB_KS = K0 / SA_HEAD_BWD_WG;
+
+__global__ __launch_bounds__(1024) void sa_head_bwd_wide_kernel(SaHeadBwdArgs a) {
+  extern __shared__ __attribute__((aligned(16))) unsigned char smem[];
+  const int M = a.M, tid = threadIdx.x, wg = blockIdx.x, kbase = wg * HB_KS;
+  const bool first = wg == 0;
+  float* H1 = reinterpret_cast<float*>(smem);
+  float* H2 = H1 + M * N1;
+  float* D1 = H2 + M * N2;
+  float* D2 = D1 + M * N1;
+  float* DL = D2 + M * N2;
+  float* Ws = DL + SA_HEAD_MAXB * NC;
+  float* Xs = Ws + N1 * HB_KS;
+  constexpr int Q = HB_KS / 4;
+  float4 stage = make_float4(0.0f, 0.0f, 0.0f, 0.0f);
+  const int sw = tid, sx = tid - N1 * Q;
+  if (sw < N1 * Q) stage = *reinterpret_cast<const float4*>(a.w1 + (size_t)(sw / Q) * K0 + kbase + 4 * (sw % Q));
+  else if (sx < M * Q) stage = *reinterpret_cast<const float4*>(a.pooled + (size_t)(sx / Q) * K0 + kbase + 4 * (sx % Q));
+  for (int i = tid; i < M * N1 / 4; i += 1024) reinterpret_cast<float4*>(H1)[i] = reinterpret_cast<const float4*>(a.h1)[i];
+  for (int i = tid; i < M * N2 / 4; i += 1024) reinterpret_cast<float4*>(H2)[i] = reinterpret_cast<const float4*>(a.h2)[i];
+  if (tid < M) {
+    const float d0 = a.dlogp[tid * NC], d1 = a.dlogp[tid * NC + 1], s = d0 + d1;
+    DL[tid * NC] = d0 - expf(a.logp[tid * NC]) * s;
+    DL[tid * NC + 1] = d1 - expf(a.logp[tid * NC + 1]) * s;
+  }
+  __syncthreads();
+  const float* s2 = a.f2 + 2 * N2; const float* t2 = a.f2 + 3 * N2;
+  const float* s1 = a.f1 + 2 * N1; const float* t1 = a.f1 + 3 * N1;
+  if (first) {
+    if (tid < NC * N2) {
+      const int c = tid / N2, k = tid % N2;
+      float acc = 0.0f;
+      for (int m = 0; m < M; ++m) acc = fmaf(DL[m * NC + c], fmaf(H2[m * N2 + k], s2[k], t2[k]), acc);
+      if (a.dw3) a.dw3[tid] = acc;
+    } else if (tid < NC * N2 + NC) {
+      const int c = tid - NC * N2;
+      float acc = 0.0f;
+      for (int m = 0; m < M; ++m) acc += DL[m * NC + c];
+      if (a.db3) a.db3[c] = acc;
+    }
+  }
+  for (int i = tid; i < M * N2; i += 1024) {
+    const int m = i / N2, k = i % N2;
+    D2[i] = fmaf(DL[m * NC], a.w3[k], DL[m * NC + 1] * a.w3[N2 + k]);
+  }
+  __syncthreads();
+  if (tid < N2) head_bn_bwd(D2, H2, M, N2, tid, a.f2, a.g2, first ? a.dg2 : nullptr, first ? a.dbe2 : nullptr);
+  __syncthreads();
+  if (a.dw2) {
+    constexpr int PER = N2 * N1 / SA_HEAD_BWD_WG;
+    for (int j = tid; j < PER; j += 1024) {
+      const int i = wg * PER + j, n = i / N1, k = i % N1;
+      float acc = 0.0f;
+      const float sk = s1[k], tk = t1[k];
+      for (int m = 0; m < M; ++m) acc = fmaf(D2[m * N2 + n], fmaf(H1[m * N1 + k], sk, tk), acc);
+      a.dw2[i] = acc;
+    }
+  }
+  if (first && tid < N2 && a.db2) {
+    float acc = 0.0f;
+    for (int m = 0; m < M; ++m) acc += D2[m * N2 + tid];
+    a.db2[tid] = acc;
+  }
+  for (int i = tid; i < M * N1; i += 1024) {
+    const int m = i / N1, k = i % N1;
+    float acc = 0.0f;
+#pragma unroll 8
+    for (int n = 0; n < N2; ++n) acc = fmaf(D2[m * N2 + n], a.w2[n * N1 + k], acc);
+    D1[i] = acc;
+  }
+  if (sw < N1 * Q) *reinterpret_cast<float4*>(Ws + 4 * sw) = stage;
+  else if (sx < M * Q) *reinterpret_cast<float4*>(Xs + 4 * sx) = stage;
+  __syncthreads();
+  if (tid < N1) head_bn_bwd(D1, H1, M, N1, tid, a.f1, a.g1, first ? a.dg1 : nullptr, first ? a.dbe1 : nullptr);
+  __syncthreads();
+  if (a.dw1 && tid < N1 * Q) {
+    const int n = tid / Q, kq = tid % Q;
+    float a0 = 0.0f, a1 = 0.0f, a2 = 0.0f, a3 = 0.0f;
+    for (int m = 0; m < M; ++m) {
+      const float4 x = *reinterpret_cast<const float4*>(Xs + m * HB_KS + 4 * kq);
+      const float d = D1[m * N1 + n];
+      a0 = fmaf(d, x.x, a0); a1 = fmaf(d, x.y, a1); a2 = fmaf(d, x.z, a2); a3 = fmaf(d, x.w, a3);
+    }
+    *reinterpret_cast<float4*>(a.dw1 + (size_t)n * K0 + kbase + 4 * kq) = make_float4(a0, a1, a2, a3);
+  }
+  if (first && tid >= 512 && tid < 512 + N1 && a.db1) {
+    const int n = tid - 512;
+    float acc = 0.0f;
+    for (int m = 0; m < M; ++m) acc += D1[m * N1 + n];
+    a.db1[n] = acc;
+  }
+  if (a.dpooled) {
+    const int kk = tid % HB_KS, m = tid / HB_KS;
+    if (m < M) {
+      float acc = 0.0f;
+#pragma unroll 8
+      for (int n = 0; n < N1; ++n) acc = fmaf(D1[m * N1 + n], Ws[n * HB_KS + kk], acc);
+      a.dpooled[(size_t)m * K0 + kbase + kk] = acc;
+    }
+  }
+}
+
+extern "C" int sa_head_bwd_wide(const float* dlogp, const float* logp, const float* pooled, const float* h1,
+                                const float* f1, const float* h2, const float* f2, const float* w1, const float* g1,
+                                const float* w2, const float* g2, const float* w3, float* dw1, float* db1,
+                                float* dg1, float* dbe1, float* dw2, float* db2, float* dg2, float* dbe2,
+                                float* dw3, float* db3, float* dpooled, int M, void* stream) {
+  if (!dlogp || !logp || !pooled || !h1 || !f1 || !h2 || !f2 || !w1 || !g1 || !w2 || !g2 || !w3 || M < 1 ||
+      M > SA_HEAD_MAXB)
+    return -22;
+  SaHeadBwdArgs a{dlogp, logp, pooled, h1, f1, h2, f2, w1, g1, w2, g2, w3,
+                  dw1, db1, dg1, dbe1, dw2, db2, dg2, dbe2, dw3, db3, dpooled, M};
+  static_assert(1024 / HB_KS >= SA_HEAD_MAXB && (N1 + SA_HEAD_MAXB) * HB_KS / 4 <= 1024, "slice geometry");
+  const size_t lds = ((size_t)M * (2 * N1 + 2 * N2 + HB_KS) + SA_HEAD_MAXB * NC + N1 * HB_KS) * sizeof(float);
+  static bool attr_set = false;
+  if (!attr_set) {
+    hipError_t e = hipFuncSetAttribute(reinterpret_cast<const void*>(sa_head_bwd_wide_kernel),
+                                       hipFuncAttributeMaxDynamicSharedMemorySize, 160 * 1024);
+    if (e != hipSuccess) return -(int)e;
+    attr_set = true;
+  }
+  hipLaunchKernelGGL(sa_head_bwd_wide_kernel, dim3(SA_HEAD_BWD_WG), dim3(1024), lds,
+                     reinterpret_cast<hipStream_t>(stream), a);
+  hipError_t e = hipGetLastError();
+  return e == hipSuccess ? 0 : -(int)e;
+}
+
 extern "C" int sa_head_max_rows(void) { return SA_HEAD_MAXB; }
diff --git a/speech-anonymization_amd/ops.py b/speech-anonymization_amd/ops.py
--- a/speech-anonymization_amd/ops.py
+++ b/speech-anonymization_amd/ops.py
@@ -474,18 +474,32 @@
     return (g / g.max()).contiguous()
 
 
-def pool_fwd(r, scale, shift, noise=None, eps=1e-5):
+def pooling_noise_raw(setting, B, Cc, device):
+    if setting is True:
+        return torch.randn(B, Cc, device=device), True
+    return pooling_noise(setting, B, Cc, device), False
+
+
+def pool_fwd(r, scale, shift, noise=None, eps=1e-5, fused=False, raw=False):
     lib = L.load()
     B, Ln, _ = r.shape
     nseg = lib.sa_pool_nseg(B)
     part = torch.empty(B, nseg, 128, 128, 2, dtype=torch.float32, device=r.device)
     L.check(lib.sa_pool_fwd(L.dt_code(r.dtype), _f(r), _f(scale), _f(shift), _f(part), B, Ln, nseg,
                             L.stream()), "sa_pool_fwd")
-    sums = torch.empty(B, 128, 2, dtype=torch.float64, device=r.device)
-    L.check(lib.sa_pool_gather(_f(part), B, nseg, Ln, _f(sums), L.stream()), "sa_pool_gather")
     pooled = torch.empty(B, 256, dtype=torch.float32, device=r.device)
     mean = torch.empty(B, 128, dtype=torch.float32, device=r.device)
     sd = torch.empty(B, 128, dtype=torch.float32, device=r.device)
+    if fused:
+        if noise is not None and (noise.numel() != B * 128 or noise.dtype != torch.float32):
+            raise L.SaHipError(f"pooling noise must be fp32 [{B}, 128], got {noise.dtype} {tuple(noise.shape)}")
+        L.check(lib.sa_pool_gather_fin(_f(part), B, nseg, Ln, _f(noise), int(bool(raw)), C.c_float(eps), _f(pooled),
+                                       _f(mean), _f(sd), L.stream()), "sa_pool_gather_fin")
+        return pooled, mean, sd
+    if raw:
+        raise L.SaHipError("raw pooling noise needs fused=True")
+    sums = torch.empty(B, 128, 2, dtype=torch.float64, device=r.device)
+    L.check(lib.sa_pool_gather(_f(part), B, nseg, Ln, _f(sums), L.stream()), "sa_pool_gather")
     L.check(lib.sa_pool_fin(_f(sums), B, Ln, _f(noise), C.c_float(eps), _f(pooled), _f(mean), _f(sd),
                             L.stream()), "sa_pool_fin")
     return pooled, mean, sd
@@ -561,15 +575,17 @@
     return H1, tuple(f1[i] for i in range(4)), H2, tuple(f2[i] for i in range(4)), logp
 
 
-def head_bwd(dlogp, logp, pooled, H1, f1, H2, f2, P, grads):
+def head_bwd(dlogp, logp, pooled, H1, f1, H2, f2, P, grads, wide=False):
     M = pooled.shape[0]
     dpooled = torch.empty(M, 256, dtype=torch.float32, device=pooled.device)
     g = lambda k: _f(grads.get(k))
-    L.check(L.load().sa_head_bwd(_f(dlogp), _f(logp), _f(pooled), _f(H1), _f(f1[0]), _f(H2), _f(f2[0]),
-                                 _f(P["0.weight"]), _f(P["2.weight"]), _f(P["3.weight"]), _f(P["5.weight"]),
-                                 _f(P["6.weight"]), g("0.weight"), g("0.bias"), g("2.weight"), g("2.bias"),
-                                 g("3.weight"), g("3.bias"), g("5.weight"), g("5.bias"), g("6.weight"), g("6.bias"),
-                                 _f(dpooled), M, L.stream()), "sa_head_bwd")
+    lib = L.load()
+    entry, name = (lib.sa_head_bwd_wide, "sa_head_bwd_wide") if wide else (lib.sa_head_bwd, "sa_head_bwd")
+    L.check(entry(_f(dlogp), _f(logp), _f(pooled), _f(H1), _f(f1[0]), _f(H2), _f(f2[0]),
+                  _f(P["0.weight"]), _f(P["2.weight"]), _f(P["3.weight"]), _f(P["5.weight"]),
+                  _f(P["6.weight"]), g("0.weight"), g("0.bias"), g("2.weight"), g("2.bias"),
+                  g("3.weight"), g("3.bias"), g("5.weight"), g("5.bias"), g("6.weight"), g("6.bias"),
+                  _f(dpooled), M, L.stream()), name)
     return dpooled
 
 
@@ -610,6 +626,26 @@
     L.check(lib.sa_cls_losses(_f(logp), _f(label), B, NC, _f(out), _f(dn), _f(dc), L.stream()),
             "sa_cls_losses")
     return out, dn, dc
+
+
+def step_loss(pred, target, kind, logp, label, w_recon, w_sex, nonfinite=None):
+    lib = L.load()
+    n = pred.numel()
+    if pred.data_ptr() % 16:
+        pred = pred.clone()
+    if target.data_ptr() % 16:
+        target = target.clone()
+    B, NC = logp.shape
+    dev = pred.device
+    ws = torch.empty(lib.sa_loss_workspace_bytes() // 8, dtype=torch.float64, device=dev)
+    d_pred = torch.empty_like(pred)
+    d_logp = torch.empty_like(logp)
+    out = torch.empty(3, dtype=torch.float32, device=dev)
+    L.check(lib.sa_recon_loss_part(_f(pred), _f(target), C.c_longlong(n), 0 if kind == "l1" else 1, _f(d_pred),
+                                   C.c_float(w_recon), _f(ws), L.stream()), "sa_recon_loss_part")
+    L.check(lib.sa_step_loss(_f(ws), C.c_longlong(n), _f(logp), _f(label), B, NC, C.c_float(w_recon),
+                             C.c_float(w_sex), _f(out), _f(d_logp), _f(nonfinite), L.stream()), "sa_step_loss")
+    return out, d_pred, d_logp
 
 
 def cosine_loss(x1, x2, want_grad=False):
```

After: 4.042 million frames/s (median of 6 runs). 1.01x the previous value.
